# ayutaz/F5-TTS

Hardware: AMD Instinct MI355X
Metric: mel-frames/s (RTF alongside), F5TTS_v1_Base NFE=16 CFM.sample (higher is better)
Workload: dtype bf16; 1 GPU; C2: F5TTS_v1_Base CFM.sample, NFE 16 EPSS + sway -1, CFG 2.0, 1 utterance per GPU, 938 prompt + 938 generated frames (1876), 300 tokens; batch_per_gpu=1, frames=1876, gen_frames_per_gpu=938, nfe=16, parallelism=dp1

## Files before the change

f5-tts_amd/csrc/attention.hip:

```cpp
#include "common.h"
#include "kernels.h"

#include <cstdlib>
#include <cstring>

namespace f5h {

template <int OFF>
F5H_DEV u32x4 lds_b128(uint32_t addr) {
  u32x4 r;
  asm volatile("ds_read_b128 %0, %1 offset:%2" : "=v"(r) : "v"(addr), "i"(OFF));
  return r;
}
template <int OFF>
F5H_DEV uint2 lds_tr_b64(uint32_t addr) {
  uint2 r;
  asm volatile("ds_read_b64_tr_b16 %0, %1 offset:%2" : "=v"(r) : "v"(addr), "i"(OFF));
  return r;
}

F5H_DEV float xor32(float x) {
  const unsigned u = __float_as_uint(x);
  auto r = __builtin_amdgcn_permlane32_swap(u, u, false, false);
  const int hi = (__lane_id() >= 32);
  return __uint_as_float(hi ? r[0] : r[1]);
}

F5H_DEV void attn_block(int& qb, int& bh) {
  const int nqb = gridDim.x, nwg = gridDim.x * gridDim.y;
  const int w = blockIdx.x + nqb * blockIdx.y;
  const int xq = nwg >> 3, xr = nwg & 7, xcd = w & 7;
  const int id = (xcd < xr ? xcd * (xq + 1) : xr * (xq + 1) + (xcd - xr) * xq) + (w >> 3);
  qb = id % nqb;
  bh = id / nqb;
}

template <typename T, bool PRESCALED, int NW, bool RSM>
__global__ __launch_bounds__(64 * NW, 8 / NW) void attn16_kernel(AttnArgs a) {
  typedef Op16<T> OP;
  typedef typename OP::v8 v8;
  typedef typename OP::v4 v4;
  const ProbeT probe_t = probe_enter(a.probe);
  constexpr int TILE_B = 2 * 64 * 128;
  constexpr int NS = 4;
  constexpr int CPW = 512 / (64 * NW);
  constexpr float THR = 8.f;
  static_assert(CPW * 64 * NW == 512, "whole DMA rounds");
  __shared__ __attribute__((aligned(16))) uint4 lds[NS * TILE_B / 16];
  const int tid = threadIdx.x, lane = tid & 63, wid = tid >> 6;
  const int h = lane >> 5;
  int qb, bh;
  attn_block(qb, bh);
  if (a.q_len) bh = spread8(bh, gridDim.y);
  const int s_idx = bh / a.H, head = bh - s_idx * a.H;
  const int L = a.L;
  if (a.q_len && qb * (32 * NW) >= a.q_len[s_idx]) {
    probe_exit(a.probe, probe_t);
    return;
  }
  const int64_t base = (int64_t)bh * L * 64;
  const T* Q = reinterpret_cast<const T*>(a.q) + base;
  const T* K = reinterpret_cast<const T*>(a.k) + base;
  const T* V = reinterpret_cast<const T*>(a.v) + base;
  int klen = L;
  if (a.kv_len) klen = min(klen, a.kv_len[s_idx]);
  const int ntile = (klen + 63) / 64;

  const int qrow = qb * (32 * NW) + wid * 32 + (lane & 31);

  const int wid_s = __builtin_amdgcn_readfirstlane(wid);
  uint32_t dvoff[CPW];
#pragma unroll
  for (int r = 0; r < CPW; ++r) {
    const int p = (r * NW + wid) * 64 + lane, row = p >> 3, slot = p & 7;
    dvoff[r] = (uint32_t)(row * 128 + swz128(row, slot) * 16);
  }
  auto dma = [&](int buf, int kt, bool live = false) {
    uint4* Ks = lds + buf * (TILE_B / 16);
    uint4* Vs = Ks + 512;
    const int rows = live ? min(64, L - kt * 64) : max(0, min(64, L - kt * 64));
    const uint32_t ext = (uint32_t)__builtin_amdgcn_readfirstlane(rows * 128);
    const __amdgpu_buffer_rsrc_t krs = rsrc_of(K + (int64_t)kt * 4096, ext);
    const __amdgpu_buffer_rsrc_t vrs = rsrc_of(V + (int64_t)kt * 4096, ext);
#pragma unroll
    for (int r = 0; r < CPW; ++r) {
      dma16(krs, (LDS_PTR(void))(Ks + (r * NW + wid_s) * 64), dvoff[r], 0);
      dma16(vrs, (LDS_PTR(void))(Vs + (r * NW + wid_s) * 64), dvoff[r], 0);
    }
  };

  const uint32_t lds0 = (uint32_t)(uintptr_t)(LDS_PTR(void))lds;
  uint32_t kaddr[4];
#pragma unroll
  for (int ks = 0; ks < 4; ++ks) {
    const int row = lane & 31;
    kaddr[ks] = lds0 + row * 128 + swz128(row, ks * 2 + h) * 16;
  }
  const int G = lane >> 4, q4 = (lane & 15) >> 2, p4 = lane & 3;
  uint32_t vaddr[2][2];
#pragma unroll
  for (int u = 0; u < 2; ++u)
#pragma unroll
    for (int g8 = 0; g8 < 2; ++g8) {
      const int r1 = 4 * (G >> 1) + q4 + 8 * g8;
      const int dh = 32 * u + 16 * (G & 1) + 4 * p4;
      vaddr[u][g8] = lds0 + 64 * 128 + r1 * 128 + swz128(r1, dh >> 3) * 16 + ((dh >> 2) & 1) * 8;
    }

  typedef float f2 __attribute__((ext_vector_type(2)));
  float m_run = 0.f;
  f32x16 oacc[2], minit;
  f2 lrow = {0.f, 0.f};
  f32x16 lacc;
#pragma unroll
  for (int r = 0; r < 16; ++r) lacc[r] = 0.f;
  v8 ones;
#pragma unroll
  for (int j = 0; j < 8; ++j) ones[j] = from_f32<T>(1.f);
#pragma unroll
  for (int r = 0; r < 16; ++r) {
// ... 156 lines not shown
        for (int sx = 0; sx < 2; ++sx) {
          asm volatile("" : "+v"(vf[u][t][sx][0]));
          asm volatile("" : "+v"(vf[u][t][sx][1]));
        }
    __builtin_amdgcn_sched_barrier(0);
    static_for<0, 3>([&](auto C) {
      mma_chunk(C);
      exp_chunk(std::integral_constant<int, decltype(C)::value + 1>{});
      __builtin_amdgcn_sched_group_barrier(0x008, 1, 0);
      __builtin_amdgcn_sched_group_barrier(0x400, 4, 0);
      __builtin_amdgcn_sched_group_barrier(0x002, 4, 0);
      __builtin_amdgcn_sched_group_barrier(0x008, 1, 0);
      __builtin_amdgcn_sched_group_barrier(0x400, 4, 0);
      __builtin_amdgcn_sched_group_barrier(0x002, 4, 0);
      __builtin_amdgcn_sched_barrier(0);
    });
    mma_chunk(std::integral_constant<int, 3>{});
  };
  using IF = std::false_type;
  using IT = std::true_type;
  auto tile = [&](auto SLOT, auto FIRST_, auto SAFE_, const int kt) __attribute__((always_inline)) {
    tile_wait(kt);
    tile_qk(SLOT, FIRST_, SAFE_, kt);
    tile_pv(SLOT);
  };
  auto pass = [&](auto SAFE_) __attribute__((always_inline)) {
    if (wave_dead) {
      for (int kt = 0; kt < ntile; ++kt) {
        if (kt + 2 < ntile)
          asm volatile("s_waitcnt vmcnt(%0)" ::"i"(4 * CPW) : "memory");
        else if (kt + 1 < ntile)
          asm volatile("s_waitcnt vmcnt(%0)" ::"i"(2 * CPW) : "memory");
        else
          asm volatile("s_waitcnt vmcnt(0)" ::: "memory");
        __builtin_amdgcn_s_barrier();
        if (kt + 3 < ntile) dma((kt + 3) % NS, kt + 3, true);
      }
    } else {
      if (ntile > 0) tile(std::integral_constant<int, 0>{}, IT{}, SAFE_, 0);
      for (int kt0 = 0; kt0 < ntile; kt0 += NS) {
        static_for<0, NS>([&](auto S) {
          const int kt = kt0 + decltype(S)::value;
          if (kt >= 1 && kt < ntile) tile(S, IF{}, SAFE_, kt);
        });
      }
    }
    asm volatile("s_waitcnt vmcnt(0)" ::: "memory");
  };
  if (__builtin_amdgcn_readfirstlane(threadIdx.x) >= 256) __builtin_amdgcn_s_setprio(1);
  pass(IF{});
  auto row_sum = [&]() -> float {
    if constexpr (RSM) return lacc[0];
    float l = lrow.x + lrow.y;
    return l + xor32(l);
  };
  float l_tot = row_sum();
  {
    const bool bad = !(l_tot <= LMAX);
    const unsigned vote = __builtin_amdgcn_ballot_w64(bad) != 0ull ? 1u : 0u;
    __builtin_amdgcn_s_barrier();
    uint32_t* flags = reinterpret_cast<uint32_t*>(lds);
    if (lane == 0) flags[wid] = vote;
    __syncthreads();
    unsigned any = 0;
#pragma unroll
    for (int w = 0; w < NW; ++w) any |= flags[w];
    if (__builtin_amdgcn_readfirstlane(any) || a.force_safe) {
      __syncthreads();
      m_run = 0.f;
      lrow = f2{0.f, 0.f};
#pragma unroll
      for (int r = 0; r < 16; ++r) lacc[r] = 0.f;
#pragma unroll
      for (int r = 0; r < 16; ++r) {
        oacc[0][r] = 0.f;
        oacc[1][r] = 0.f;
        minit[r] = 0.f;
      }
      dma(0, 0);
      dma(1, 1);
      dma(2, 2);
      pass(IT{});
      l_tot = row_sum();
    }
  }
  probe_mark(a.probe, probe_t, 2);
  const float inv = l_tot > 0.f ? 1.f / l_tot : 0.f;
  if (!wave_dead) {
    T* O = reinterpret_cast<T*>(a.o) + (((int64_t)s_idx * L + min(qrow, L - 1)) * a.H + head) * 64;
#pragma unroll
    for (int u = 0; u < 2; ++u)
#pragma unroll
      for (int r4 = 0; r4 < 4; r4 += 2) {
        v4 w0 = {from_f32<T>(oacc[u][4 * r4 + 0] * inv), from_f32<T>(oacc[u][4 * r4 + 1] * inv),
                 from_f32<T>(oacc[u][4 * r4 + 2] * inv), from_f32<T>(oacc[u][4 * r4 + 3] * inv)};
        v4 w1 = {from_f32<T>(oacc[u][4 * r4 + 4] * inv), from_f32<T>(oacc[u][4 * r4 + 5] * inv),
                 from_f32<T>(oacc[u][4 * r4 + 6] * inv), from_f32<T>(oacc[u][4 * r4 + 7] * inv)};
        uint2 a2 = __builtin_bit_cast(uint2, w0), b2 = __builtin_bit_cast(uint2, w1);
        auto sx = __builtin_amdgcn_permlane32_swap(a2.x, b2.x, false, false);
        auto sy = __builtin_amdgcn_permlane32_swap(a2.y, b2.y, false, false);
        const uint4 out = make_uint4(sx[0], sy[0], sx[1], sy[1]);
        if (qrow < L) *reinterpret_cast<uint4*>(O + 32 * u + 8 * r4 + 8 * h) = out;
      }
  }
  probe_exit(a.probe, probe_t);
}

__global__ __launch_bounds__(64) void attn_f32_kernel(AttnArgs a) {
  const ProbeT probe_t = probe_enter(a.probe);
  __shared__ float Ks[32][65];
  __shared__ float Vs[32][64];
  const int lane = threadIdx.x;
  const int bh = blockIdx.y;
  const int s_idx = bh / a.H, head = bh - s_idx * a.H;
  const int L = a.L;
  const int64_t base = (int64_t)bh * L * 64;
  const float* Q = reinterpret_cast<const float*>(a.q) + base;
  const float* K = reinterpret_cast<const float*>(a.k) + base;
  const float* V = reinterpret_cast<const float*>(a.v) + base;
  int klen = L;
  if (a.kv_len) klen = min(klen, a.kv_len[s_idx]);
  if (a.q_len && (int)blockIdx.x * 64 >= a.q_len[s_idx]) {
    probe_exit(a.probe, probe_t);
    return;
  }
  const int qrow = blockIdx.x * 64 + lane;
  float q[64], o[64];
#pragma unroll
  for (int d = 0; d < 64; ++d) {
    q[d] = qrow < L ? Q[(int64_t)qrow * 64 + d] : 0.f;
    o[d] = 0.f;
  }
  float m_run = -INFINITY, l_run = 0.f;
  for (int k0 = 0; k0 < klen; k0 += 32) {
    __syncthreads();
    for (int i = lane; i < 32 * 64; i += 64) {
      int r = i >> 6, d = i & 63, key = k0 + r;
      Ks[r][d] = key < klen ? K[(int64_t)key * 64 + d] : 0.f;
      Vs[r][d] = key < klen ? V[(int64_t)key * 64 + d] : 0.f;
    }
    __syncthreads();
    float sc[32];
    float mx = m_run;
#pragma unroll
    for (int r = 0; r < 32; ++r) {
      float acc = 0.f;
#pragma unroll
      for (int d = 0; d < 64; ++d) acc = fmaf(q[d], Ks[r][d], acc);
      sc[r] = (k0 + r < klen) ? (a.prescaled ? acc : acc * a.scale) : -INFINITY;
      mx = fmaxf(mx, sc[r]);
    }
    const float alpha = a.prescaled ? exp2f(m_run - mx) : expf(m_run - mx);
    m_run = mx;
    l_run *= alpha;
#pragma unroll
    for (int d = 0; d < 64; ++d) o[d] *= alpha;
#pragma unroll
    for (int r = 0; r < 32; ++r) {
      float p = a.prescaled ? exp2f(sc[r] - mx) : expf(sc[r] - mx);
      l_run += p;
#pragma unroll
      for (int d = 0; d < 64; ++d) o[d] = fmaf(p, Vs[r][d], o[d]);
    }
  }
  if (qrow < L) {
    float* O = reinterpret_cast<float*>(a.o) + (((int64_t)s_idx * L + qrow) * a.H + head) * 64;
    const float inv = 1.f / l_run;
#pragma unroll
    for (int d = 0; d < 64; ++d) O[d] = o[d] * inv;
  }
  probe_exit(a.probe, probe_t);
}

template <typename T>
static void launch16(const AttnArgs& a, hipStream_t st) {
  constexpr int NW = 8;
  dim3 grid((a.L + 32 * NW - 1) / (32 * NW), a.S * a.H);
  static const bool rsm = [] {
    const char* v = getenv("F5H_ATTN_ROWSUM");
    return v && !strcmp(v, "mfma");
  }();
  if (a.prescaled) {
    if (rsm)
      hipLaunchKernelGGL((attn16_kernel<T, true, NW, true>), grid, dim3(64 * NW), 0, st, a);
    else
      hipLaunchKernelGGL((attn16_kernel<T, true, NW, false>), grid, dim3(64 * NW), 0, st, a);
  } else {
    hipLaunchKernelGGL((attn16_kernel<T, false, NW, false>), grid, dim3(64 * NW), 0, st, a);
  }
}

static int g_force_safe = 0;
void attention_force_safe(int on) { g_force_safe = on ? 1 : 0; }

hipError_t attention(int compute, const AttnArgs& a0, hipStream_t st) {
  if (a0.S <= 0 || a0.H <= 0 || a0.L <= 0) return hipErrorInvalidValue;
  AttnArgs a = a0;
  a.force_safe = g_force_safe;
  switch (compute) {
    case F5H_C_BF16: launch16<bf16>(a, st); break;
    case F5H_C_FP16: launch16<f16>(a, st); break;
    default: {
      dim3 grid((a.L + 63) / 64, a.S * a.H);
      hipLaunchKernelGGL(attn_f32_kernel, grid, dim3(64), 0, st, a);
    }
  }
  return hipGetLastError();
}

}
```

f5-tts_amd/csrc/chain.h:

```cpp
#pragma once
#include "common.h"
#include "kernels.h"

namespace f5h {

constexpr int kAuxWT = 16;
constexpr unsigned kChainSpinLimit = 1u << 18;
constexpr int kChainSleep = 2;

F5H_DEV void chain_wait(const ChainDep& d, int M, int r0, int nrows) {
  if (!d.wait) return;
  if (__builtin_amdgcn_readfirstlane(threadIdx.x >> 6) == 0) {
    const int g0 = r0 / kChainRows, g1 = (min(r0 + nrows, M) - 1) / kChainRows;
    for (int gi = g0; gi <= g1; ++gi) {
      const int rows = min(kChainRows, M - gi * kChainRows);
      const unsigned need = (unsigned)(d.wait_mult * ((rows + d.wait_unit - 1) / d.wait_unit));
      for (unsigned spins = 0;; ++spins) {
        const unsigned v =
            __builtin_amdgcn_readfirstlane(__hip_atomic_load(d.wait + gi, __ATOMIC_RELAXED, __HIP_MEMORY_SCOPE_AGENT));
        if (v >= need) break;
        if (spins >= d.spin_limit) {
          __hip_atomic_store(d.err, 1u, __ATOMIC_RELAXED, __HIP_MEMORY_SCOPE_AGENT);
          break;
        }
        __builtin_amdgcn_s_sleep(kChainSleep);
      }
    }
    __builtin_amdgcn_fence(__ATOMIC_ACQUIRE, "agent");
    asm volatile("s_waitcnt vmcnt(0)" ::: "memory");
    if (d.tl && threadIdx.x == 0) d.tl[1] = wall_clock64();
  }
  __syncthreads();
}

F5H_DEV void chain_publish(const ChainDep& d, int M, int r0, int nrows) {
  asm volatile("s_waitcnt vmcnt(0)" ::: "memory");
  __syncthreads();
  if (d.tl && threadIdx.x == 0) d.tl[2] = wall_clock64();
  if (threadIdx.x == 0) {
    const int g0 = r0 / kChainRows, g1 = (min(r0 + nrows, M) - 1) / kChainRows;
    for (int gi = g0; gi <= g1; ++gi) __hip_atomic_fetch_add(d.pub + gi, 1u, __ATOMIC_RELAXED, __HIP_MEMORY_SCOPE_AGENT);
  }
}

}
```

f5-tts_amd/csrc/common.h:

```cpp
#pragma once
#include <hip/hip_runtime.h>
#include <stdint.h>

#include <type_traits>

#include "kernels.h"

typedef __bf16 bf16;
typedef __bf16 bf16x8 __attribute__((ext_vector_type(8)));
typedef __bf16 bf16x4 __attribute__((ext_vector_type(4)));
typedef _Float16 f16;
typedef _Float16 f16x8 __attribute__((ext_vector_type(8)));
typedef _Float16 f16x4 __attribute__((ext_vector_type(4)));
typedef short s16x4 __attribute__((ext_vector_type(4)));
typedef float f32x4 __attribute__((ext_vector_type(4)));
typedef float f32x16 __attribute__((ext_vector_type(16)));
typedef unsigned int u32x4 __attribute__((ext_vector_type(4)));

#define F5H_DEV __device__ __forceinline__
#define LDS_PTR(T) __attribute__((address_space(3))) T*

F5H_DEV bf16 f2bf(float x) { return (bf16)x; }
F5H_DEV float bf2f(bf16 x) { return (float)x; }

// ... 122 lines not shown
F5H_DEV float wave_max(float v) {
#pragma unroll
  for (int o = 32; o > 0; o >>= 1) v = fmaxf(v, __shfl_xor(v, o, 64));
  return v;
}

F5H_DEV int swz128(int row, int chunk) {
  return chunk ^ ((((row >> 1) & 1) << 2) | ((row >> 2) & 3));
}
F5H_DEV int swz256(int row, int chunk) { return chunk ^ (row & 15); }

template <typename T> struct Slab;
template <> struct Slab<bf16> {
  typedef bf16x8 frag;
  static F5H_DEV f32x4 mma(const frag& a, const frag& b, f32x4 c) {
    return __builtin_amdgcn_mfma_f32_16x16x32_bf16(a, b, c, 0, 0, 0);
  }
};
template <> struct Slab<f16> {
  typedef f16x8 frag;
  static F5H_DEV f32x4 mma(const frag& a, const frag& b, f32x4 c) {
    return __builtin_amdgcn_mfma_f32_16x16x32_f16(a, b, c, 0, 0, 0);
  }
};
template <> struct Slab<float> {
  typedef f32x4 frag;
  static F5H_DEV f32x4 mma(const frag& a, const frag& b, f32x4 c) {
    c = __builtin_amdgcn_mfma_f32_16x16x4f32(a[0], b[0], c, 0, 0, 0);
    c = __builtin_amdgcn_mfma_f32_16x16x4f32(a[1], b[1], c, 0, 0, 0);
    c = __builtin_amdgcn_mfma_f32_16x16x4f32(a[2], b[2], c, 0, 0, 0);
    c = __builtin_amdgcn_mfma_f32_16x16x4f32(a[3], b[3], c, 0, 0, 0);
    return c;
  }
};

template <typename T, typename S> struct Load16;
template <> struct Load16<bf16, bf16> {
  static F5H_DEV uint4 ld(const bf16* p, bool ok) {
    return ok ? *reinterpret_cast<const uint4*>(p) : make_uint4(0, 0, 0, 0);
  }
};
template <> struct Load16<float, float> {
  static F5H_DEV uint4 ld(const float* p, bool ok) {
    return ok ? *reinterpret_cast<const uint4*>(p) : make_uint4(0, 0, 0, 0);
  }
};
template <> struct Load16<f16, f16> {
  static F5H_DEV uint4 ld(const f16* p, bool ok) {
    return ok ? *reinterpret_cast<const uint4*>(p) : make_uint4(0, 0, 0, 0);
  }
};
template <> struct Load16<f16, float> {
  static F5H_DEV uint4 ld(const float* p, bool ok) {
    if (!ok) return make_uint4(0, 0, 0, 0);
    float4 a = *reinterpret_cast<const float4*>(p);
    float4 b = *reinterpret_cast<const float4*>(p + 4);
    f16x8 v = {(f16)a.x, (f16)a.y, (f16)a.z, (f16)a.w, (f16)b.x, (f16)b.y, (f16)b.z, (f16)b.w};
    return __builtin_bit_cast(uint4, v);
  }
};
template <> struct Load16<bf16, float> {
  static F5H_DEV uint4 ld(const float* p, bool ok) {
    if (!ok) return make_uint4(0, 0, 0, 0);
    float4 a = *reinterpret_cast<const float4*>(p);
    float4 b = *reinterpret_cast<const float4*>(p + 4);
    bf16x8 v = {f2bf(a.x), f2bf(a.y), f2bf(a.z), f2bf(a.w), f2bf(b.x), f2bf(b.y), f2bf(b.z), f2bf(b.w)};
    return __builtin_bit_cast(uint4, v);
  }
};

template <typename T> F5H_DEV constexpr int elems16() { return 16 / (int)sizeof(T); }

F5H_DEV int spread8(int r, int n) {
  const int q = n >> 3, rem = n & 7;
  if (q == 0) return r;
  const int big = rem * (q + 1);
  const int c = r < big ? r / (q + 1) : rem + (r - big) / q;
  const int i = r < big ? r - c * (q + 1) : (r - big) - (c - rem) * q;
  return i * 8 + c;
}

F5H_DEV __amdgpu_buffer_rsrc_t rsrc_of(const void* p, uint64_t bytes) {
  return __builtin_amdgcn_make_buffer_rsrc(const_cast<void*>(p), 0, (int)(uint32_t)bytes, 0x00020000);
}
F5H_DEV void dma16(__amdgpu_buffer_rsrc_t r, LDS_PTR(void) dst, uint32_t voff, uint32_t soff) {
  __builtin_amdgcn_raw_ptr_buffer_load_lds(r, dst, 16, voff, soff, 0, 0);
}

template <int B, int E, typename F>
F5H_DEV void static_for(F&& f) {
  if constexpr (B < E) {
    f(std::integral_constant<int, B>{});
    static_for<B + 1, E>(f);
  }
}

#define F5H_OP_DISPATCH(compute, T, ...)  \
  do {                                     \
    switch (compute) {                     \
      case f5h::F5H_C_BF16: {              \
        typedef bf16 T;                    \
        __VA_ARGS__;                       \
      } break;                             \
      case f5h::F5H_C_FP16: {              \
        typedef f16 T;                     \
        __VA_ARGS__;                       \
      } break;                             \
      default: {                           \
        typedef float T;                   \
        __VA_ARGS__;                       \
      }                                    \
    }                                      \
  } while (0)
```

f5-tts_amd/csrc/engine.cpp:

```cpp
#include <hip/hip_runtime.h>

#include <cmath>
#include <cstring>
#include <algorithm>
#include <atomic>
#include <chrono>
#include <cstdio>
#include <memory>
#include <functional>
#include <mutex>
#include <string>
#include <unordered_map>
#include <vector>

#include "../../include/f5h.h"
#include "kernels.h"
#include "reaper.h"

using namespace f5h;

static thread_local std::string g_err;
static int fail(int code, const std::string& msg) {
  g_err = msg;
  return code;
}
int f5h_internal_fail(int code, const std::string& msg) { return fail(code, msg); }
#define HIPCK(x)                                                                               \
  do {                                                                                         \
    hipError_t _e = (x);                                                                       \
    if (_e != hipSuccess) return fail(F5H_EHIP, std::string(#x) + ": " + hipGetErrorString(_e)); \
  } while (0)

#define RC(x)              \
  do {                     \
    int _r = (x);          \
    if (_r) return _r;     \
  } while (0)

struct Lin {
  void* w = nullptr;
  float* b = nullptr;
  int N = 0, K = 0, Npad = 0;
};

struct CNX {
  float *dw_w = nullptr, *dw_b = nullptr, *ln_w = nullptr, *ln_b = nullptr, *gamma = nullptr, *beta = nullptr;
  Lin pw1, pw2;
};

struct Layer {
  Lin qkv, out, ff1, ff2, skip;
  float *g_attn = nullptr, *g_ff = nullptr;
  Lin qkv_g, ff1_g;
};

struct GraphKey {
  const void* ws;
  int kind;
  int B, N, nt, nfe, use_cfg, batch_mask, probe, split, pad_skip, chain, lnfold;
  int method;
  uint64_t kernel_epoch;
  uint32_t cfg_bits;
  bool operator==(const GraphKey& o) const {
    return ws == o.ws && kind == o.kind && B == o.B && N == o.N && nt == o.nt && nfe == o.nfe && kernel_epoch == o.kernel_epoch &&
           use_cfg == o.use_cfg && batch_mask == o.batch_mask && probe == o.probe && cfg_bits == o.cfg_bits &&
           split == o.split && pad_skip == o.pad_skip && chain == o.chain && lnfold == o.lnfold && method == o.method;
  }
};

struct f5h_engine {
  f5h_arch a{};
  int dev = 0;
  int bf = 0;
  size_t esz = 4;
  int tdp = 0;
  std::vector<void*> allocs;
  hipStream_t mstream = nullptr;
  Lin t1, t2, ada, in_x, in_ct, proj_out;
  float* text_table = nullptr;
  float* freqs = nullptr;
  std::vector<CNX> cnx;
  void* conv_w[2] = {nullptr, nullptr};
  float* conv_b[2] = {nullptr, nullptr};
  std::vector<Layer> layers;
  float* norm_out_g = nullptr;
  std::mutex gm;
  std::vector<std::shared_ptr<struct GraphEntry>> graphs;
  std::vector<std::shared_ptr<struct GraphEntry>> graveyard;
  std::vector<hipEvent_t> ev_pool;
  std::vector<struct GraphKey> pro_seen;
  int64_t n_evicted = 0, n_reaped = 0;
  std::mutex hm;
  double last_host[8] = {};
  hipStream_t cap = nullptr;
  hipStream_t cap2 = nullptr;
  hipEvent_t ev_fork = nullptr, ev_join = nullptr;
  int graph_mode = 1;
  int split_cfg = 2;
  int pad_skip = 1;
  int chain = 0;
  int lnfold = 1;
  bool lnf_ok = false, rmsf_ok = false;
  const void** lnf_w = nullptr;
  int64_t ada_row = 0;
  std::atomic<int64_t> n_lnfold{0};
  unsigned* chain_fault = nullptr;
  volatile unsigned* fault_host = nullptr;
  int fault_slot = -1;
  std::atomic<int64_t> n_chain{0};
  uint64_t use_ctr = 0;
  int64_t n_captures = 0, n_replays = 0;
  std::mutex pm;
  int probe_class = -1;
  unsigned long long* pstamp = nullptr;
  unsigned long long* pslots = nullptr;
  unsigned long long* ptl = nullptr;
  int* ptick = nullptr;
  double wall_khz = 0.0;
  UseLog uses;
};
static constexpr size_t kGraphCache = 16;
static constexpr size_t kProbeBytes = (64 + 2 * (size_t)kProbeEnd) * sizeof(unsigned long long);

static std::atomic<uint64_t> g_kernel_epoch{0};

struct GraphEntry {
  GraphKey key{};
  hipGraphExec_t exec = nullptr;
  uint64_t stamp = 0;
  std::vector<hipEvent_t> inflight;
  ~GraphEntry() {
    if (exec) (void)hipGraphExecDestroy(exec);
    for (hipEvent_t ev : inflight) (void)hipEventDestroy(ev);
  }
};

struct WView {
  const void* p;
  int dt;
  int64_t numel;
};
struct WMap {
  std::unordered_map<std::string, WView> m;
  const WView* get(const std::string& n, int64_t numel, std::string* err) const {
    auto it = m.find(n);
    if (it == m.end()) {
      *err = "missing weight " + n;
      return nullptr;
    }
    if (it->second.numel != numel) {
      *err = "weight " + n + " has " + std::to_string(it->second.numel) + " elements, expected " +
             std::to_string(numel);
      return nullptr;
    }
    return &it->second;
  }
};

static int ealloc(f5h_engine* e, size_t bytes, void** out) {
  void* p = dev_alloc(e->dev, bytes, e->mstream);
  if (!p) return fail(F5H_EHIP, "device allocation of " + std::to_string(bytes) + " bytes");
  e->allocs.push_back(p);
  *out = p;
  return 0;
}

template <typename T>
static int upload(f5h_engine* e, const std::vector<T>& h, T** out) {
  void* p = nullptr;
  RC(ealloc(e, h.size() * sizeof(T) + 16, &p));
  HIPCK(hipMemcpyAsync(p, h.data(), h.size() * sizeof(T), hipMemcpyHostToDevice, e->mstream));
  HIPCK(hipStreamSynchronize(e->mstream));
  *out = reinterpret_cast<T*>(p);
  return 0;
}

static int dalloc(f5h_engine* e, size_t bytes, void** out) {
  void* p = nullptr;
  RC(ealloc(e, bytes + 16, &p));
  HIPCK(hipMemsetAsync(p, 0, bytes + 16, e->mstream));
  *out = p;
  return 0;
}

static int op_dt(const f5h_engine* e) { return e->bf; }

static int pack_rows(const WView& v, int rows, int64_t ld_src, int col0, int ncols, void* dst, int ddt,
                     int64_t ld_dst, int dst_row0, int dst_col, hipStream_t st) {
// ... 233 lines not shown
  uint8_t* rowkeep;
  int32_t* kvlen;
  float* lnp;
  unsigned* chain;
  int chain_g4;
  float *ada_cur, *temb_cur, *tgrid;
  int* kstep;
  float* y;
  float** trajp;
  float *sgrid, *kbuf;
  std::vector<void*> xs;
  void* pp[2];
  float* in_cond;
  uint8_t* in_mask;
  int64_t* in_text;
  int32_t* in_dur;
};

static void layout(const f5h_engine* e, WS& ws, Bufs& b, int B, int N, int nfe, int use_cfg, int method = 0,
                   int steps = 0) {
  const f5h_arch& a = e->a;
  const int d = a.dim, td = a.text_dim, S = use_cfg ? 2 * B : B;
  const int L = a.backbone == F5H_DIT ? N : N + 1;
  const size_t rows = (size_t)S * L, es = e->esz;
  const int inner = a.heads * 64;
  b.tsin = ws.take<float>((size_t)nfe * 256);
  b.th = ws.take<float>((size_t)nfe * d);
  b.temb = ws.take<float>((size_t)nfe * d);
  b.tin_op = ws.take<char>((size_t)nfe * std::max(256, d) * es);
  b.ada = a.backbone == F5H_DIT ? ws.take<float>((size_t)nfe * e->ada_row) : nullptr;
  b.te = ws.take<float>((size_t)2 * B * N * td);
  b.keepfill = ws.take<uint8_t>((size_t)2 * B * N);
  if (a.conv_layers > 0) {
    b.dwln = ws.take<char>((size_t)2 * B * N * td * es);
    b.pw1o = ws.take<float>((size_t)2 * B * N * 2 * td);
    b.grno = ws.take<char>((size_t)2 * B * N * 2 * td * es);
    b.grn_scr = ws.take<float>((size_t)((N + 63) / 64 + 1) * 2 * B * 2 * td);
  } else {
    b.dwln = b.grno = nullptr;
    b.pw1o = b.grn_scr = nullptr;
  }
  b.act = ws.take<char>((size_t)S * N * (128 + e->tdp) * es);
  b.P = ws.take<float>((size_t)S * N * d);
  b.ypad = ws.take<char>((size_t)B * N * 128 * es);
  b.h0 = ws.take<float>((size_t)S * N * d);
  b.c1 = ws.take<char>((size_t)S * N * d * es);
  b.h = a.backbone == F5H_DIT ? ws.take<float>(rows * d) : nullptr;
  b.aop = ws.take<char>(rows * d * es);
  b.q = ws.take<char>(rows * inner * es);
  b.k = ws.take<char>(rows * inner * es);
  b.v = ws.take<char>(rows * inner * es);
  b.o = ws.take<char>(rows * inner * es);
  b.f = ws.take<char>(rows * a.ff_dim * es);
  b.p = ws.take<float>(rows * e->proj_out.Npad);
  b.rope = ws.take<float2>((size_t)L * 32);
  b.rowkeep = ws.take<uint8_t>(rows);
  b.kvlen = ws.take<int32_t>(S);
  b.chain_g4 = ((int)((rows + kChainRows - 1) / kChainRows) + 3) / 4 * 4;
  b.chain = a.backbone == F5H_DIT ? ws.take<unsigned>((size_t)a.depth * 5 * b.chain_g4) : nullptr;
  b.ada_cur = a.backbone == F5H_DIT ? ws.take<float>((size_t)e->ada_row) : nullptr;
  b.lnp = (e->lnf_ok || e->rmsf_ok) ? ws.take<float>(rows * (size_t)(d / 64) * 2) : nullptr;
  b.temb_cur = ws.take<float>((size_t)d);
  b.tgrid = ws.take<float>((size_t)nfe);
  b.kstep = ws.take<int>(64);
  b.y = ws.take<float>((size_t)B * N * e->a.mel_dim);
  b.trajp = ws.take<float*>(8);
  b.in_cond = ws.take<float>((size_t)B * N * a.mel_dim);
  b.in_mask = ws.take<uint8_t>((size_t)B * N);
  b.in_text = ws.take<int64_t>((size_t)B * N);
  b.in_dur = ws.take<int32_t>((size_t)B);
  b.xs.clear();
  b.pp[0] = b.pp[1] = nullptr;
  if (a.backbone == F5H_UNETT) {
    for (int i = 0; i <= a.depth / 2; ++i) b.xs.push_back(ws.take<char>(rows * d * es));
    b.pp[0] = ws.take<char>(rows * d * es);
    b.pp[1] = ws.take<char>(rows * d * es);
  }
  b.sgrid = method ? ws.take<float>((size_t)steps + 1) : nullptr;
  const int kept = ode_kept_slopes(method);
  b.kbuf = kept ? ws.take<float>((size_t)kept * B * N * a.mel_dim) : nullptr;
}

enum { KC_FFN1 = 0, KC_ATTN = 1, KC_QKV = 2, KC_FFN2 = 3, KC_CONV = 4, KC_OUT = 5, KC_NORM = 6, KC_CHAIN = 7 };
struct ProbeScope {
  f5h_engine* e;
  hipStream_t st;
  bool on;
  bool self = false;
  unsigned long long* slots = nullptr;
  ProbeScope(f5h_engine* e_, int kc, hipStream_t s, int* site, DevProbe* kp = nullptr)
      : e(e_), st(s), on(e_->probe_class == kc && e_->pslots && *site < kProbeSites) {
    if (!on) return;
    const int s0 = (*site)++;
    slots = e->pslots + (size_t)s0 * kProbeRow;
    if (kp) {
      self = true;
      kp->slots = slots;
      kp->tick = e->ptick;
      kp->tl = s0 == 0 ? e->ptl : nullptr;
    } else {
      (void)stamp_begin(slots, e->ptick, st);
    }
  }
  ~ProbeScope() {
    if (on && !self) (void)stamp_end(slots, e->ptick, st);
  }
};

struct Ctx {
  f5h_engine* e;
  hipStream_t st;
  Bufs b;
  int B, N, nt, S, L, nfe, use_cfg, batch_mask;
  int method, steps;
  int drop_audio, drop_text;
  hipStream_t st2;
  int site;
  int chain;
  int lnfold;
  double* hp;
};
enum { HP_TOTAL = 0, HP_PROLOGUE, HP_LOCK, HP_REAP, HP_CAPTURE, HP_INSTANTIATE, HP_LAUNCH, HP_FINAL, kHostPhases };
static double host_ms() {
  return std::chrono::duration<double, std::milli>(std::chrono::steady_clock::now().time_since_epoch()).count();
}

static GemmArgs gargs(const void* A, int64_t lda, const Lin& W, int M, void* C, int64_t ldc) {
  GemmArgs g{};
  g.A = A;
  g.lda = lda;
  g.W = W.w;
  g.ldw = W.K;
  g.M = M;
  g.N = W.N;
  g.K = W.K;
  g.bias = W.b;
  g.C = C;
  g.ldc = ldc;
  return g;
}

#define KCK(x)                                                                                  \
  do {                                                                                          \
    hipError_t _e = (x);                                                                        \
    if (_e != hipSuccess) return fail(F5H_EHIP, std::string(#x) + ": " + hipGetErrorString(_e)); \
  } while (0)

static int prologue(Ctx& c, const float* t_host, int nt_vals, const float* cond, const uint8_t* cond_mask,
                    const int64_t* text, const int32_t* duration, bool text_cached = false) {
  f5h_engine* e = c.e;
  const f5h_arch& a = e->a;
  const int d = a.dim, td = a.text_dim, bf = e->bf;
  Bufs& b = c.b;
  hipStream_t st = c.st;
  KCK(rope_table(c.L, b.rope, st));
  const int off = a.backbone == F5H_DIT ? 0 : 1;
  if (c.batch_mask) {
    KCK(build_rowkeep(duration, c.B, c.S, c.L, off, b.rowkeep, st));
    KCK(build_kvlen(duration, c.B, c.S, off, b.kvlen, st));
  }
  {
    if (t_host)
      KCK(time_sinus(t_host, nt_vals, b.tsin, st));
    else
      KCK(time_sinus_dev(b.tgrid, nt_vals, b.tsin, st));
    KCK(f32_to_op(bf, b.tsin, (int64_t)nt_vals * 256, b.tin_op, st));
    GemmArgs g = gargs(b.tin_op, 256, e->t1, nt_vals, b.th, d);
    KCK(gemm(bf, EPI_SILU, g, st));
    KCK(f32_to_op(bf, b.th, (int64_t)nt_vals * d, b.tin_op, st));
    g = gargs(b.tin_op, d, e->t2, nt_vals, b.temb, d);
    KCK(gemm(bf, EPI_STORE, g, st));
    if (a.backbone == F5H_DIT) {
      KCK(silu_to_op(bf, b.temb, b.tin_op, (int64_t)nt_vals * d, st));
      g = gargs(b.tin_op, d, e->ada, nt_vals, b.ada, e->ada_row);
      KCK(gemm(bf, EPI_STORE, g, st));
      if (c.lnfold) {
        LnFoldArgs la{};
        la.table = b.ada;
        la.stride = e->ada_row;
        la.out_off = e->ada.Npad;
        la.nfe = nt_vals;
        la.depth = a.depth;
        la.d = d;
        la.F = a.ff_dim;
        la.w1 = e->lnf_w;
        la.wqkv = e->lnf_w + a.depth;
        KCK(lnfold_uv(bf, la, st));
      }
    }
  }
  if (!text_cached) {
    TextEmbArgs t{};
    t.text = text;
    t.B = c.B;
    t.nt = c.nt;
    t.N = c.N;
    t.td = td;
    t.seq_len = (a.backbone == F5H_DIT && c.batch_mask) ? duration : nullptr;
    t.table = e->text_table;
    t.freqs = a.conv_layers > 0 ? e->freqs : nullptr;
    t.mask_padding = a.text_mask_padding;
    t.out_c = b.te;
// ... 79 lines not shown
    cv.x = b.h0 + no * d;
    cv.x_f32 = 1;
    cv.w = e->conv_w[0];
    cv.bias = e->conv_b[0];
    cv.mode = 0;
    cv.y = op(b.c1, no, d);
    {
      ProbeScope ps(e, KC_CONV, st, &c.site);
      KCK(conv_pos(bf, cv, st));
    }
    cv.x = op(b.c1, no, d);
    cv.x_f32 = bf ? 0 : 1;
    cv.w = e->conv_w[1];
    cv.bias = e->conv_b[1];
    cv.mode = r16 ? 2 : 1;
    cv.y = bh;
    cv.y_seq_stride = c.L;
    cv.y_row_off = dit ? 0 : 1;
    cv.resid = b.h0 + no * d;
    KCK(conv_pos(bf, cv, st));
  }
  if (!dit) KCK(write_time_token(bf, r16, b.temb_cur, ns, c.L, d, bh, st));

  const float* ada_k = dit ? b.ada_cur : nullptr;
  const int epi_resid = r16 ? EPI_RESID16 : EPI_RESID;
  void* h = bh;
  const void* h_in = nullptr;
  auto qkv_args = [&](const Layer& Lq) {
    GemmArgs g = gargs(aop, d, Lq.qkv, rows, nullptr, 0);
    g.rope = b.rope;
    g.seq_len = c.L;
    g.heads = H;
    g.rope_heads = a.pe_attn_head > 0 ? a.pe_attn_head : H;
    g.q = q;
    g.k = k;
    g.v = v;
    g.q_scale = 0.125f * 1.4426950408889634f;
    return g;
  };
  const bool chain_on = c.chain && dit && r16 && do_ln && !keep && d == 1024 && b.chain && s0 == 0 && ns == c.S &&
                        (e->probe_class < 0 || e->probe_class == KC_ATTN || e->probe_class == KC_CONV ||
                         e->probe_class == KC_CHAIN);
  static const bool zero_memset = [] {
    const char* v = getenv("F5H_CHAIN_ZERO");
    return v && !strcmp(v, "memset");
  }();
  if (chain_on) {
    if (zero_memset)
      KCK(hipMemsetAsync(b.chain, 0, (size_t)a.depth * 5 * b.chain_g4 * sizeof(unsigned), st));
    else
      KCK(zero_words(b.chain, (int64_t)a.depth * 5 * b.chain_g4, st));
  }
  bool qkv_done = false;
  bool final_done = false;
  const bool fold_on = c.lnfold && dit && r16 && do_ln && !keep && !chain_on && b.lnp && e->lnf_ok;
  const bool rms_on = c.lnfold && !dit && r16 && b.lnp && e->rmsf_ok;
  const int64_t lnf_lw = 2 * (int64_t)a.ff_dim + 6 * (int64_t)d;
  auto lnf = [&](int l) { return ada_k + e->ada.Npad + (int64_t)l * lnf_lw; };
  auto fold_consumer = [&](GemmArgs& g, const float* u, const float* v) {
    g.ln_part_in = b.lnp + ro * (size_t)(d / 64) * 2;
    g.ln_nparts = d / 64;
    g.ln_u = u;
    g.ln_v = v;
    g.ln_eps = 1e-6f;
  };
  auto rms_consumer = [&](GemmArgs& g) {
    g.ln_part_in = b.lnp + ro * (size_t)(d / 64) * 2;
    g.ln_nparts = d / 64;
    g.ln_rms = 1;
    g.ln_eps = 1e-30f;
  };
  auto rms_producer = [&](GemmArgs& g) {
    g.ln_part = b.lnp + ro * (size_t)(d / 64) * 2;
    g.ln_nparts = d / 64;
    g.ln_rms = 1;
  };
  auto fold_producer = [&](GemmArgs& g, const float* scale) {
    g.hs = aop;
    g.hs_scale = scale;
    g.ln_part = b.lnp + ro * (size_t)(d / 64) * 2;
    g.ln_nparts = d / 64;
  };
  if (fold_on || rms_on) e->n_lnfold.fetch_add(1, std::memory_order_relaxed);
  for (int l = 0; l < a.depth; ++l) {
    Layer& Ly = e->layers[l];
    const float* ad = ada_k ? ada_k + (size_t)l * 6 * d : nullptr;
    if (!dit) {
      const int half = a.depth / 2;
      if (l < half) {
        h_in = res(b.xs[l]);
        h = res(b.xs[l + 1]);
        if (!(rms_on && l > 0)) KCK(rms_norm_g(bf, h_in, r16, rows, d, Ly.g_attn, aop, st));
      } else {
        void* x_prev = h;
        h = res(b.pp[(l - half) & 1]);
        h_in = nullptr;
        GemmArgs g = gargs(x_prev, d, Ly.skip, rows, h, d);
        g.A2 = res(b.xs[a.depth - 1 - l]);
        g.k_split = d;
        KCK(gemm(bf, r16 ? EPI_STORE16 : EPI_STORE, g, st));
        KCK(rms_norm_g(bf, h, r16, rows, d, Ly.g_attn, aop, st));
      }
    } else {
      if (do_ln && !qkv_done && !(fold_on && l > 0))
        KCK(ln_modulate(bf, h, r16, rows, d, ad , ad + d , aop, st));
    }
    if (!qkv_done) {
      GemmArgs g = qkv_args(Ly);
      if (fold_on && l > 0) fold_consumer(g, lnf(l) + 2 * a.ff_dim, lnf(l) + 2 * a.ff_dim + 3 * d);
      if (rms_on && l > 0 && l < a.depth / 2) {
        g.A = h_in;
        g.W = Ly.qkv_g.w;
        rms_consumer(g);
      }
      ProbeScope ps(e, KC_QKV, st, &c.site, &g.probe);
      KCK(gemm(bf, EPI_QKV, g, st));
    }
    qkv_done = false;
    {
      AttnArgs at{};
      at.q = q;
      at.k = k;
      at.v = v;
      at.o = o;
      at.S = ns;
      at.H = H;
      at.L = c.L;
      at.kv_len = (a.attn_mask_enabled && c.batch_mask) ? b.kvlen + s0 : nullptr;
      at.q_len = (c.batch_mask && e->pad_skip) ? b.kvlen + s0 : nullptr;
      at.scale = 0.125f;
      at.prescaled = 1;
      ProbeScope ps(e, KC_ATTN, st, &c.site, &at.probe);
      KCK(attention(bf, at, st));
    }
    if (chain_on) {
      ChainArgs ca{};
      ca.out = gargs(o, inner, Ly.out, rows, h, d);
      ca.out.gate = ad + 2 * d;
      ca.ln1 = LnArgs{h, aop, ad + 3 * d , ad + 4 * d };
      ca.ff1 = gargs(aop, d, Ly.ff1, rows, f, a.ff_dim);
      ca.ff2 = gargs(f, a.ff_dim, Ly.ff2, rows, h, d);
      ca.ff2.gate = ad + 5 * d;
      if (l + 1 < a.depth) {
        const float* an = ada_k + (size_t)(l + 1) * 6 * d;
        ca.ln2 = LnArgs{h, aop, an , an + d };
        ca.qkv = qkv_args(e->layers[l + 1]);
      } else {
        const float* fin = ada_k + (size_t)a.depth * 6 * d;
        ca.ln2 = LnArgs{h, aop, fin + d, fin};
      }
      ca.cnt = b.chain + (size_t)l * 5 * b.chain_g4;
      ca.groups = (rows + kChainRows - 1) / kChainRows;
      ca.fault = e->chain_fault;
      ProbeScope ps(e, KC_CHAIN, st, &c.site, &ca.probe);
      const hipError_t ce = chain_launch(bf, ca, st);
      if (ce == hipSuccess) {
        e->n_chain.fetch_add(1, std::memory_order_relaxed);
        qkv_done = l + 1 < a.depth;
        final_done = l + 1 == a.depth;
        continue;
      }
      if (ce != hipErrorInvalidValue) KCK(ce);
    }
    {
      GemmArgs g = gargs(o, inner, Ly.out, rows, h, d);
      g.resid = h_in;
      g.gate = ad ? ad + 2 * d : nullptr;
      g.rowkeep = keep;
      if (keep && !h_in && e->pad_skip && !rms_on) {
        g.live_len = b.kvlen + s0;
        g.live_seq = c.L;
      }
      if (fold_on) fold_producer(g, ad + 4 * d );
      if (rms_on) rms_producer(g);
      ProbeScope ps(e, KC_OUT, st, &c.site, &g.probe);
      KCK(gemm(bf, epi_resid, g, st));
    }
    if (!fold_on && !rms_on) {
      ProbeScope ps(e, KC_NORM, st, &c.site);
      if (dit) {
        if (do_ln) KCK(ln_modulate(bf, h, r16, rows, d, ad + 3 * d , ad + 4 * d , aop, st));
      }
      else
        KCK(rms_norm_g(bf, h, r16, rows, d, Ly.g_ff, aop, st));
    }
    {
      GemmArgs g = gargs(aop, d, Ly.ff1, rows, f, a.ff_dim);
      if (fold_on) fold_consumer(g, lnf(l), lnf(l) + a.ff_dim);
      if (rms_on) {
        g.A = h;
        g.W = Ly.ff1_g.w;
        rms_consumer(g);
      }
      ProbeScope ps(e, KC_FFN1, st, &c.site, &g.probe);
      KCK(gemm(bf, EPI_GELU_TANH, g, st));
    }
    {
      GemmArgs g = gargs(f, a.ff_dim, Ly.ff2, rows, h, d);
      g.gate = ad ? ad + 5 * d : nullptr;
      if (fold_on && l + 1 < a.depth) fold_producer(g, ada_k + (size_t)(l + 1) * 6 * d + d);
      if (rms_on && l + 1 < a.depth / 2) rms_producer(g);
      ProbeScope ps(e, KC_FFN2, st, &c.site, &g.probe);
      KCK(gemm(bf, epi_resid, g, st));
    }
  }
  if (dit) {
    const float* fin = ada_k + (size_t)a.depth * 6 * d;
    if (!final_done) KCK(ln_modulate(bf, h, r16, rows, d, fin + d, fin, aop, st));
  } else {
    KCK(rms_norm_g(bf, h, r16, rows, d, e->norm_out_g, aop, st));
  }
  const int pld = e->proj_out.Npad;
  GemmArgs g = gargs(aop, d, e->proj_out, rows, b.p + ro * pld, pld);
  g.N = pld;
  KCK(gemm(bf, EPI_STORE, g, st));
  return 0;
}

static int backbone_step(Ctx& c) {
  if (!c.st2 || !c.use_cfg) return backbone_part(c, 0, c.S, c.st);
  f5h_engine* e = c.e;
  KCK(hipEventRecord(e->ev_fork, c.st));
  KCK(hipStreamWaitEvent(c.st2, e->ev_fork, 0));
  RC(backbone_part(c, 0, c.B, c.st));
  RC(backbone_part(c, c.B, c.B, c.st2));
  KCK(hipEventRecord(e->ev_join, c.st2));
  KCK(hipStreamWaitEvent(c.st, e->ev_join, 0));
  return 0;
}

static std::mutex g_slot_m;
static unsigned* g_slots = nullptr;
static std::vector<int> g_free_slots;
static constexpr int kFaultSlots = 4096;
static int fault_slot_take(volatile unsigned** host) {
  std::lock_guard<std::mutex> lk(g_slot_m);
  if (!g_slots) {
    void* p = nullptr;
    if (hipHostMalloc(&p, kFaultSlots * 64, hipHostMallocDefault) != hipSuccess) return -1;
    g_slots = static_cast<unsigned*>(p);
    for (int i = kFaultSlots - 1; i >= 0; --i) g_free_slots.push_back(i);
  }
  if (g_free_slots.empty()) return -1;
  const int i = g_free_slots.back();
  g_free_slots.pop_back();
  *host = g_slots + (size_t)i * 16;
  **host = 0u;
  return i;
}
static void fault_slot_give(int i) {
  if (i < 0) return;
  std::lock_guard<std::mutex> lk(g_slot_m);
  g_free_slots.push_back(i);
}

struct ChainGate {
  std::mutex m;
  hipStream_t owner = nullptr;
  bool owned = false;
  int enqueuing = 0;
  hipEvent_t done = nullptr;
  bool pending = false;
};
static ChainGate g_gate[64];
static std::atomic<int64_t> g_gate_refused{0};

static bool chain_admit(int dev, hipStream_t st) {
  ChainGate& g = g_gate[dev & 63];
  std::lock_guard<std::mutex> lk(g.m);
  if (g.owned && g.owner != st) {
    bool busy = g.enqueuing > 0;
    if (!busy && g.pending) {
      busy = hipEventQuery(g.done) == hipErrorNotReady;
      (void)hipGetLastError();
      if (!busy) g.pending = false;
    }
    if (busy) {
      g_gate_refused.fetch_add(1, std::memory_order_relaxed);
      return false;
    }
  }
  g.owner = st;
  g.owned = true;
  ++g.enqueuing;
// ... 207 lines not shown
  *out = e;
  return 0;
}

int f5h_engine_create(const f5h_arch* arch, const f5h_weight* weights, int32_t n_weights, int32_t device,
                      f5h_engine** out) {
  if (n_weights < 0 || (n_weights > 0 && !weights)) return fail(F5H_EINVAL, "null weights");
  std::vector<f5h_tensor_view> v((size_t)n_weights);
  for (int i = 0; i < n_weights; ++i)
    v[i] = f5h_tensor_view{weights[i].name, weights[i].data, F5H_DT_F32, 0, weights[i].numel};
  return f5h_engine_create_views(arch, v.data(), n_weights, device, out);
}

void f5h_engine_destroy(f5h_engine* e) {
  if (!e) return;
  retire(e->dev, [e] {
    for (hipEvent_t ev : e->uses.take()) {
      (void)hipEventSynchronize(ev);
      (void)hipEventDestroy(ev);
    }
    {
      std::lock_guard<std::mutex> g(e->gm);
      for (auto* v : {&e->graphs, &e->graveyard})
        for (auto& x : *v)
          for (hipEvent_t ev : x->inflight) (void)hipEventSynchronize(ev);
    }
    e->graphs.clear();
    e->graveyard.clear();
    for (hipEvent_t ev : e->ev_pool) (void)hipEventDestroy(ev);
    e->ev_pool.clear();
    if (e->cap) (void)hipStreamDestroy(e->cap);
    if (e->cap2) (void)hipStreamDestroy(e->cap2);
    if (e->ev_fork) (void)hipEventDestroy(e->ev_fork);
    if (e->ev_join) (void)hipEventDestroy(e->ev_join);
    for (void* p : e->allocs) dev_free(p, e->mstream);
    if (e->mstream) (void)hipStreamDestroy(e->mstream);
    fault_slot_give(e->fault_slot);
    delete e;
  });
}

size_t f5h_workspace_size_ode(const f5h_engine* e, int32_t B, int32_t N, int32_t nt, int32_t steps, int32_t use_cfg,
                             int32_t method) {
  (void)nt;
  if (!e || B <= 0 || N <= 0 || steps <= 0 || method < 0 || method >= kOdeMethods) return 0;
  WS ws;
  Bufs b;
  layout(e, ws, b, B, N, steps * ode_tableau(method).stages + 1, use_cfg, method, steps);
  return ws.off;
}
size_t f5h_workspace_size(const f5h_engine* e, int32_t B, int32_t N, int32_t nt, int32_t nfe, int32_t use_cfg) {
  return f5h_workspace_size_ode(e, B, N, nt, nfe, use_cfg, F5H_EULER);
}

static int check_ws(f5h_engine* e, int B, int N, int nfe, int use_cfg, void* w, size_t bytes, Ctx& c, int method = 0,
                    int steps = 0) {
  WS ws;
  layout(e, ws, c.b, B, N, nfe + 1, use_cfg, method, steps);
  if (bytes < ws.off)
    return fail(F5H_ENOMEM, "workspace too small: need " + std::to_string(ws.off) + " have " + std::to_string(bytes));
  ws.off = 0;
  ws.base = reinterpret_cast<char*>(w);
  layout(e, ws, c.b, B, N, nfe + 1, use_cfg, method, steps);
  return 0;
}

static int run_steps(Ctx& c, const f5h_sample_args* a, const void* ws);
static int graph_get(Ctx& c, const GraphKey& key, bool split, const std::function<int(Ctx&)>& body,
                     std::shared_ptr<GraphEntry>& hold, int64_t replays);
static int note_replays(f5h_engine* e, GraphEntry* g, hipStream_t st);
static bool prologue_repeats(f5h_engine* e, const GraphKey& key);

static GraphKey prologue_key(const Ctx& c, const void* ws) {
  GraphKey key{};
  key.ws = ws;
  key.kind = 1;
  key.B = c.B;
  key.N = c.N;
  key.nt = c.nt;
  key.nfe = c.nfe;
  key.use_cfg = c.use_cfg;
  key.batch_mask = c.batch_mask;
  key.lnfold = c.lnfold;
  key.method = c.method;
  key.kernel_epoch = g_kernel_epoch.load();
  return key;
}
static int prologue_graph(Ctx& c, const f5h_sample_args* a, const GraphKey& key) {
  f5h_engine* e = c.e;
  const size_t bn = (size_t)c.B * c.N;
  HIPCK(hipMemcpyAsync(c.b.in_cond, a->cond, bn * e->a.mel_dim * sizeof(float), hipMemcpyDeviceToDevice, c.st));
  HIPCK(hipMemcpyAsync(c.b.in_mask, a->cond_mask, bn, hipMemcpyDeviceToDevice, c.st));
  if (c.nt > 0)
    HIPCK(hipMemcpyAsync(c.b.in_text, a->text, (size_t)c.B * c.nt * sizeof(int64_t), hipMemcpyDeviceToDevice, c.st));
  HIPCK(hipMemcpyAsync(c.b.in_dur, a->duration, (size_t)c.B * sizeof(int32_t), hipMemcpyDeviceToDevice, c.st));
  const Bufs& b = c.b;
  std::shared_ptr<GraphEntry> hold;
  RC(graph_get(c, key, false,
               [&](Ctx& cc) { return prologue(cc, nullptr, cc.nfe, b.in_cond, b.in_mask, b.in_text, b.in_dur); },
               hold, 1));
  HIPCK(hipGraphLaunch(hold->exec, c.st));
  return note_replays(e, hold.get(), c.st);
}

static float round_to(int compute, float x) {
  if (compute == F5H_FP16) return (float)(_Float16)x;
  if (compute != F5H_BF16 || x != x) return x;
  uint32_t u;
  std::memcpy(&u, &x, 4);
  u = (u + 0x7fffu + ((u >> 16) & 1u)) & 0xffff0000u;
  std::memcpy(&x, &u, 4);
  return x;
}
static void ode_eval_times(int method, int compute, const float* t, int steps, float* out) {
#pragma clang fp contract(off)
  const OdeTableau T = ode_tableau(method);
  for (int i = 0; i <= steps; ++i)
    if (round_to(compute, t[i]) != t[i]) compute = F5H_FP32;
  for (int k = 0; k < steps; ++k) {
    const float t0 = t[k], t1 = t[k + 1];
    const float dt = round_to(compute, t1 - t0);
    for (int s = 0; s < T.stages; ++s) {
      float v = t0;
      if (s > 0) v = T.c[s] == 1.f ? t1 : round_to(compute, t0 + round_to(compute, dt * T.c[s]));
      out[k * T.stages + s] = v;
    }
  }
}

int f5h_debug_ode_tableau(int32_t method, int32_t* stages, float* c, float* a, float* b) {
  if (method < 0 || method >= kOdeMethods) return fail(F5H_EINVAL, "ode method must be 0 (euler), 1 (midpoint) or 2 (rk4)");
  const OdeTableau T = ode_tableau(method);
  if (stages) *stages = T.stages;
  if (c) std::memcpy(c, T.c, sizeof(T.c));
  if (a) std::memcpy(a, T.a, sizeof(T.a));
  if (b) std::memcpy(b, T.b, sizeof(T.b));
  return 0;
}
int f5h_debug_ode_eval_times(int32_t method, int32_t compute, const float* t_grid, int32_t steps, float* out) {
  if (method < 0 || method >= kOdeMethods || compute < F5H_FP32 || compute > F5H_FP16 || !t_grid || steps <= 0 || !out)
    return fail(F5H_EINVAL, "bad ode_eval_times argument");
  ode_eval_times(method, compute, t_grid, steps, out);
  return 0;
}

static int sample_impl(f5h_engine* e, void* stream, const f5h_sample_args* a, int method, void* workspace,
                       size_t workspace_bytes);
int f5h_sample(f5h_engine* e, void* stream, const f5h_sample_args* a, void* workspace, size_t workspace_bytes) {
  return sample_impl(e, stream, a, F5H_EULER, workspace, workspace_bytes);
}
int f5h_sample_ode(f5h_engine* e, void* stream, const f5h_sample_args* a, int32_t method, void* workspace,
                   size_t workspace_bytes) {
  if (method < 0 || method >= kOdeMethods) return fail(F5H_EINVAL, "ode method must be 0 (euler), 1 (midpoint) or 2 (rk4)");
  return sample_impl(e, stream, a, method, workspace, workspace_bytes);
}

static int sample_impl(f5h_engine* e, void* stream, const f5h_sample_args* a, int method, void* workspace,
                       size_t workspace_bytes) {
  if (!e || !a) return fail(F5H_EINVAL, "null engine/args");
  if (a->B <= 0 || a->N <= 0 || a->nt < 0 || a->nfe <= 0 || a->nfe > 512)
    return fail(F5H_EINVAL, "bad B/N/nt/nfe");
  const int stages = ode_tableau(method).stages;
  if (a->nfe * stages > 512)
    return fail(F5H_EINVAL, std::to_string(a->nfe) + " steps x " + std::to_string(stages) + " stages = " +
                                std::to_string(a->nfe * stages) +
                                " backbone evaluations exceed the 512 rows of the per-call time tables");
  if (!a->cond || !a->cond_mask || !a->duration || !a->y0 || !a->t_grid || !a->out || (a->nt > 0 && !a->text))
    return fail(F5H_EINVAL, "null tensor argument");
  if (e->a.backbone == F5H_DIT && a->N > 8192) return fail(F5H_EINVAL, "N exceeds the text position table (8192)");
  HIPCK(hipSetDevice(e->dev));
  UseNote used{e->uses, reinterpret_cast<hipStream_t>(stream)};
  Ctx c{};
  c.e = e;
  c.st = reinterpret_cast<hipStream_t>(stream);
  c.B = a->B;
  c.N = a->N;
  c.nt = a->nt;
  c.method = method;
  c.steps = a->nfe;
  c.nfe = a->nfe * stages;
  c.use_cfg = a->cfg_strength >= 1e-5f;
  c.S = c.use_cfg ? 2 * c.B : c.B;
  c.L = e->a.backbone == F5H_DIT ? c.N : c.N + 1;
  c.batch_mask = a->use_batch_mask ? 1 : 0;
  RC(check_ws(e, c.B, c.N, c.nfe, c.use_cfg, workspace, workspace_bytes, c, method, c.steps));
  RC(chain_fault_check(e, c.st));
  ChainTicket ticket;
  c.chain = chain_for_call(e, c, ticket);
  c.lnfold = e->lnfold && !c.chain && ((e->lnf_ok && !c.batch_mask) || e->rmsf_ok);
  double hp[kHostPhases] = {};
  c.hp = hp;
  const double h0 = host_ms();
  static const bool pro_graph = [] {
    const char* v = getenv("F5H_PROLOGUE_GRAPH");
    return !(v && *v == '0');
  }();
  std::vector<float> evt;
  const float* t_rows = a->t_grid;
  if (method == F5H_EULER) {
    HIPCK(grid_upload(a->t_grid, c.nfe + 1, c.b.tgrid, c.st));
  } else {
    evt.resize(c.nfe);
    ode_eval_times(method, e->bf, a->t_grid, c.steps, evt.data());
    t_rows = evt.data();
    HIPCK(grid_upload(t_rows, c.nfe, c.b.tgrid, c.st));
    HIPCK(grid_upload(a->t_grid, c.steps + 1, c.b.sgrid, c.st));
  }
  const GraphKey pkey = prologue_key(c, workspace);
  if (pro_graph && e->graph_mode && c.nt <= c.N && prologue_repeats(e, pkey))
    RC(prologue_graph(c, a, pkey));
  else
    RC(prologue(c, t_rows, c.nfe, a->cond, a->cond_mask, a->text, a->duration));
  const double h1 = host_ms();
  const size_t ysz = (size_t)c.B * c.N * e->a.mel_dim;
  HIPCK(hipMemcpyAsync(c.b.y, a->y0, ysz * sizeof(float), hipMemcpyDeviceToDevice, c.st));
  if (a->trajectory)
    HIPCK(hipMemcpyAsync(a->trajectory, a->y0, ysz * sizeof(float), hipMemcpyDeviceToDevice, c.st));
  HIPCK(pack_y(e->bf, c.b.y, c.B * c.N, e->a.mel_dim, c.b.ypad, c.st));
  HIPCK(ptr_upload(a->trajectory, c.b.trajp, c.st));
  HIPCK(hipMemsetAsync(c.b.kstep, 0, 64 * sizeof(int), c.st));
  RC(step_prep(c));
  const double h2 = host_ms();
  const double g2 = hp[HP_LOCK] + hp[HP_REAP] + hp[HP_CAPTURE] + hp[HP_INSTANTIATE];
  RC(run_steps(c, a, workspace));
  const double h3 = host_ms();
  HIPCK(final_where_out(a->cond, a->cond_mask, c.b.y, a->out, c.B, c.N, e->a.mel_dim,
                        c.chain ? e->chain_fault : nullptr, c.st));
  if (c.chain) RC(chain_fault_note(e, c.st));
  const double h4 = host_ms();
  hp[HP_TOTAL] = h4 - h0;
  hp[HP_PROLOGUE] = h1 - h0;
  hp[HP_LAUNCH] = (h3 - h2) - (hp[HP_LOCK] + hp[HP_REAP] + hp[HP_CAPTURE] + hp[HP_INSTANTIATE] - g2);
  hp[HP_FINAL] = h4 - h3;
  {
    std::lock_guard<std::mutex> g(e->hm);
    std::memcpy(e->last_host, hp, sizeof(hp));
  }
  return 0;
}

static int enqueue_step(Ctx& c, const f5h_sample_args* a) {
  f5h_engine* e = c.e;
  {
    c.site = 0;
    RC(backbone_step(c));
    const bool dit = e->a.backbone == F5H_DIT;
    if (c.method != F5H_EULER) {
      RkArgs r{};
      r.y = c.b.y;
      r.B = c.B;
      r.N = c.N;
      r.mel = e->a.mel_dim;
      r.p = c.b.p;
      r.p_seq_stride = (int64_t)c.L * e->proj_out.Npad;
      r.p_row_off = dit ? 0 : 1;
      r.p_ld = e->proj_out.Npad;
      r.use_cfg = c.use_cfg;
      r.cfg = a->cfg_strength;
      r.ypad = c.b.ypad;
      r.compute = e->bf;
      r.method = c.method;
      r.kbuf = c.b.kbuf;
      r.keval = c.b.kstep;
      r.sgrid = c.b.sgrid;
      r.trajp = c.b.trajp;
      r.next_src = dit ? c.b.ada : c.b.temb;
      r.next_stride = dit ? e->ada_row : e->a.dim;
      r.next_n = dit ? (int)e->ada_row : e->a.dim;
      r.next_dst = dit ? c.b.ada_cur : c.b.temb_cur;
      r.neval = c.nfe;
      r.arrive = reinterpret_cast<unsigned*>(c.b.kstep + kArrive);
      r.tick = e->ptick;
      KCK(cfg_rk(r, c.st));
      return 0;
    }
    EulerArgs u{};
    u.y = c.b.y;
    u.B = c.B;
    u.N = c.N;
    u.mel = e->a.mel_dim;
    u.p = c.b.p;
    u.p_seq_stride = (int64_t)c.L * e->proj_out.Npad;
    u.p_row_off = e->a.backbone == F5H_DIT ? 0 : 1;
    u.p_ld = e->proj_out.Npad;
    u.use_cfg = c.use_cfg;
    u.cfg = a->cfg_strength;
    u.dt = 0.f;
    u.kstep = c.b.kstep;
    u.tgrid = c.b.tgrid;
    u.ypad = c.b.ypad;
    u.compute = e->bf;
    u.traj = nullptr;
    u.trajp = c.b.trajp;
    u.next_src = dit ? c.b.ada : c.b.temb;
    u.next_stride = dit ? e->ada_row : e->a.dim;
    u.next_n = dit ? (int)e->ada_row : e->a.dim;
    u.next_dst = dit ? c.b.ada_cur : c.b.temb_cur;
    u.nfe = c.nfe;
    u.arrive = reinterpret_cast<unsigned*>(c.b.kstep + kArrive);
    u.tick = e->ptick;
    KCK(cfg_euler(u, c.st));
  }
  return 0;
}

static int run_steps(Ctx& c, const f5h_sample_args* a, const void* ws) {
  f5h_engine* e = c.e;
  if (!e->graph_mode) {
    for (int k = 0; k < c.nfe; ++k) RC(enqueue_step(c, a));
    return 0;
  }
  GraphKey key{};
  key.ws = ws;
  key.B = c.B;
  key.N = c.N;
  key.nfe = c.nfe;
  key.use_cfg = c.use_cfg;
  key.batch_mask = c.batch_mask;
  key.probe = e->probe_class;
  const bool split = e->split_cfg == 1;
  key.split = split;
  key.pad_skip = e->pad_skip;
  key.chain = c.chain;
  key.lnfold = c.lnfold;
  key.method = c.method;
  key.kernel_epoch = g_kernel_epoch.load();
  std::memcpy(&key.cfg_bits, &a->cfg_strength, 4);
  std::shared_ptr<GraphEntry> hold;
  RC(graph_get(c, key, split, [&](Ctx& cc) { return enqueue_step(cc, a); }, hold, c.nfe));
  int rc = 0, k = 0;
  for (; k < c.nfe; ++k) {
    const hipError_t le = hipGraphLaunch(hold->exec, c.st);
    if (le != hipSuccess) {
      rc = fail(F5H_EHIP, std::string("hipGraphLaunch: ") + hipGetErrorString(le));
      break;
    }
  }
  if (k > 0) {
    const int r2 = note_replays(e, hold.get(), c.st);
    if (!rc) rc = r2;
  }
  return rc;
}

static bool host_trace() {
  static const bool on = [] {
    const char* v = getenv("F5H_HOST_TRACE");
    return v && *v == '1';
  }();
  return on;
}
static void reap_graphs(f5h_engine* e) {
  auto done = [e](GraphEntry& g) {
    size_t k = 0;
    for (hipEvent_t ev : g.inflight) {
      if (hipEventQuery(ev) == hipSuccess)
        e->ev_pool.push_back(ev);
      else
        g.inflight[k++] = ev;
    }
    (void)hipGetLastError();
    g.inflight.resize(k);
    return k == 0;
  };
  for (auto& g : e->graphs)
    if (g->inflight.size() > 4) done(*g);
  size_t k = 0;
  for (size_t i = 0; i < e->graveyard.size(); ++i) {
    auto& g = e->graveyard[i];
    if (done(*g) && g.use_count() == 1) {
      ++e->n_reaped;
      continue;
    }
    if (k != i) std::swap(e->graveyard[k], e->graveyard[i]);
    ++k;
  }
  e->graveyard.resize(k);
}

static int note_replays(f5h_engine* e, GraphEntry* g, hipStream_t st) {
  hipEvent_t ev = nullptr;
  {
    std::lock_guard<std::mutex> lk(e->gm);
    if (!e->ev_pool.empty()) {
      ev = e->ev_pool.back();
      e->ev_pool.pop_back();
    }
  }
  if (!ev) HIPCK(hipEventCreateWithFlags(&ev, hipEventDisableTiming));
  HIPCK(hipEventRecord(ev, st));
  std::lock_guard<std::mutex> lk(e->gm);
  g->inflight.push_back(ev);
  return 0;
}

static int graph_get(Ctx& c, const GraphKey& key, bool split, const std::function<int(Ctx&)>& body,
                     std::shared_ptr<GraphEntry>& hold, int64_t replays) {
  f5h_engine* e = c.e;
  const double t0 = host_ms();
  std::lock_guard<std::mutex> g(e->gm);
  const double t1 = host_ms();
  const int64_t reaped0 = e->n_reaped;
  reap_graphs(e);
  const double t2 = host_ms();
  if (c.hp) {
    c.hp[HP_LOCK] += t1 - t0;
    c.hp[HP_REAP] += t2 - t1;
// ... 14 lines not shown
    ne->key = key;
    Ctx cc = c;
    cc.st = e->cap;
    cc.st2 = split ? e->cap2 : nullptr;
    const double c0 = host_ms();
    hipError_t be = hipStreamBeginCapture(e->cap, hipStreamCaptureModeThreadLocal);
    if (be != hipSuccess) return fail(F5H_EHIP, std::string("hipStreamBeginCapture: ") + hipGetErrorString(be));
    const int rc = body(cc);
    hipGraph_t graph = nullptr;
    const hipError_t ce = hipStreamEndCapture(e->cap, &graph);
    if (rc || ce != hipSuccess) {
      if (graph) (void)hipGraphDestroy(graph);
      if (rc) return rc;
      return fail(F5H_EHIP, std::string("hipStreamEndCapture: ") + hipGetErrorString(ce));
    }
    const double c1 = host_ms();
    const hipError_t ie = hipGraphInstantiate(&ne->exec, graph, nullptr, nullptr, 0);
    (void)hipGraphDestroy(graph);
    if (c.hp) {
      c.hp[HP_CAPTURE] += c1 - c0;
      c.hp[HP_INSTANTIATE] += host_ms() - c1;
    }
    if (host_trace())
      std::fprintf(stderr, "[f5h host] capture %.3f ms, instantiate %.3f ms\n", c1 - c0, host_ms() - c1);
    if (ie != hipSuccess) {
      ne->exec = nullptr;
      return fail(F5H_EHIP, std::string("hipGraphInstantiate: ") + hipGetErrorString(ie));
    }
    if (e->graphs.size() >= kGraphCache) {
      size_t lru = 0;
      for (size_t i = 1; i < e->graphs.size(); ++i)
        if (e->graphs[i]->stamp < e->graphs[lru]->stamp) lru = i;
      e->graveyard.push_back(std::move(e->graphs[lru]));
      e->graphs.erase(e->graphs.begin() + lru);
      ++e->n_evicted;
    }
    e->graphs.push_back(ne);
    e->n_captures++;
    hold = ne;
  }
  hold->stamp = ++e->use_ctr;
  e->n_replays += replays;
  return 0;
}

static bool prologue_repeats(f5h_engine* e, const GraphKey& key) {
  std::lock_guard<std::mutex> g(e->gm);
  for (const auto& x : e->graphs)
    if (x->key == key) return true;
  for (const auto& k : e->pro_seen)
    if (k == key) return true;
  if (e->pro_seen.size() >= 64) e->pro_seen.erase(e->pro_seen.begin());
  e->pro_seen.push_back(key);
  return false;
}

int f5h_forward(f5h_engine* e, void* stream, const f5h_forward_args* a, void* workspace, size_t workspace_bytes) {
  if (!e || !a) return fail(F5H_EINVAL, "null engine/args");
  if (a->B <= 0 || a->N <= 0 || a->nt < 0) return fail(F5H_EINVAL, "bad B/N/nt");
  if (!a->x || !a->cond || !a->cond_mask || !a->duration || !a->pred || (a->nt > 0 && !a->text))
    return fail(F5H_EINVAL, "null tensor argument");
  HIPCK(hipSetDevice(e->dev));
  UseNote used{e->uses, reinterpret_cast<hipStream_t>(stream)};
  Ctx c{};
  c.e = e;
  c.st = reinterpret_cast<hipStream_t>(stream);
  c.B = a->B;
  c.N = a->N;
  c.nt = a->nt;
  c.nfe = 1;
  c.use_cfg = a->cfg_infer ? 1 : 0;
  c.S = c.use_cfg ? 2 * c.B : c.B;
  c.drop_audio = (!c.use_cfg && a->drop_audio_cond) ? 1 : 0;
  c.drop_text = (!c.use_cfg && a->drop_text) ? 1 : 0;
  c.L = e->a.backbone == F5H_DIT ? c.N : c.N + 1;
  c.batch_mask = a->use_batch_mask ? 1 : 0;
  if (e->a.backbone == F5H_DIT && a->N > 8192) return fail(F5H_EINVAL, "N exceeds the text position table (8192)");
  if (a->text_cache < 0 || a->text_cache > 2) return fail(F5H_EINVAL, "text_cache must be 0, 1 or 2");
  RC(check_ws(e, c.B, c.N, 1, c.use_cfg, workspace, workspace_bytes, c));
  RC(chain_fault_check(e, c.st));
  ChainTicket ticket;
  c.chain = chain_for_call(e, c, ticket);
  c.lnfold = e->lnfold && !c.chain && ((e->lnf_ok && !c.batch_mask) || e->rmsf_ok);
  const bool cached = a->text_cache == 2;
  if (a->t_dev) {
    HIPCK(hipMemcpyAsync(c.b.tgrid, a->t_dev, sizeof(float), hipMemcpyDeviceToDevice, c.st));
    RC(prologue(c, nullptr, 1, a->cond, a->cond_mask, a->text, a->duration, cached));
  } else {
    float tg[2] = {a->t, a->t};
    RC(prologue(c, tg, 1, a->cond, a->cond_mask, a->text, a->duration, cached));
  }
  HIPCK(pack_y(e->bf, a->x, c.B * c.N, e->a.mel_dim, c.b.ypad, c.st));
  HIPCK(hipMemsetAsync(c.b.kstep, 0, sizeof(int), c.st));
  auto body = [](Ctx& cc) -> int {
    cc.site = 0;
    RC(step_prep(cc));
    RC(backbone_step(cc));
    KCK(step_advance(cc.b.kstep, cc.e->ptick, cc.st));
    return 0;
  };
  if (e->graph_mode && a->text_cache != 0) {
    GraphKey key{};
    key.ws = workspace;
    key.kind = 2;
    key.B = c.B;
    key.N = c.N;
    key.nt = c.nt;
    key.nfe = 1;
    key.use_cfg = c.use_cfg;
    key.batch_mask = c.batch_mask;
    key.probe = e->probe_class;
    key.pad_skip = e->pad_skip;
    key.chain = c.chain;
    key.lnfold = c.lnfold;
    key.kernel_epoch = g_kernel_epoch.load();
    std::shared_ptr<GraphEntry> hold;
    RC(graph_get(c, key, false, body, hold, 1));
    HIPCK(hipGraphLaunch(hold->exec, c.st));
    RC(note_replays(e, hold.get(), c.st));
  } else {
    RC(body(c));
  }
  HIPCK(copy_pred(c.b.p, c.S, c.L, e->a.backbone == F5H_DIT ? 0 : 1, e->a.mel_dim, e->proj_out.Npad, a->pred,
                  c.chain ? e->chain_fault : nullptr, c.st));
  if (c.chain) RC(chain_fault_note(e, c.st));
  return 0;
}

int f5h_probe_enable(f5h_engine* e, int32_t kclass, int32_t enable) {
  if (!e) return fail(F5H_EINVAL, "null engine");
  std::lock_guard<std::mutex> g(e->pm);
  e->probe_class = enable ? kclass : -1;
  if (e->pstamp) {
    HIPCK(hipSetDevice(e->dev));
    HIPCK(hipDeviceSynchronize());
    HIPCK(hipMemset(e->pstamp, 0, 64 * sizeof(unsigned long long)));
    HIPCK(hipMemset(e->pslots, 0xff, (size_t)kProbeEnd * sizeof(unsigned long long)));
    HIPCK(hipMemset(e->pslots + kProbeEnd, 0, (size_t)kProbeEnd * sizeof(unsigned long long)));
    HIPCK(hipMemset(e->ptl, 0, (size_t)kTimelineWG * 4 * sizeof(unsigned long long)));
    HIPCK(hipDeviceSynchronize());
  }
  return 0;
}

int f5h_probe_timeline(f5h_engine* e, uint64_t* stamps, int32_t max_wg, int32_t* n_wg, double* tick_khz) {
  if (!e || !stamps || max_wg <= 0) return fail(F5H_EINVAL, "null engine / buffer");
  std::lock_guard<std::mutex> g(e->pm);
  HIPCK(hipSetDevice(e->dev));
  HIPCK(hipDeviceSynchronize());
  const int n = std::min<int>(max_wg, kTimelineWG);
  HIPCK(hipMemcpy(stamps, e->ptl, (size_t)n * 4 * sizeof(unsigned long long), hipMemcpyDeviceToHost));
  int last = 0;
  for (int i = 0; i < n; ++i)
    if (stamps[4 * i]) last = i + 1;
  if (n_wg) *n_wg = last;
  if (tick_khz) *tick_khz = e->wall_khz;
  return 0;
}

int f5h_probe_read(f5h_engine* e, int64_t* launches, double* total_ms) {
  if (!e) return fail(F5H_EINVAL, "null engine");
  std::lock_guard<std::mutex> g(e->pm);
  double ms = 0.0;
  int64_t n = 0;
  if (e->pstamp && e->wall_khz > 0.0) {
    HIPCK(hipSetDevice(e->dev));
    HIPCK(hipDeviceSynchronize());
    std::vector<unsigned long long> h(2 * (size_t)kProbeEnd);
    HIPCK(hipMemcpy(h.data(), e->pslots, h.size() * sizeof(unsigned long long), hipMemcpyDeviceToHost));
    unsigned long long ticks = 0;
    for (int64_t i = 0; i < kProbeEnd; i += (int64_t)kProbeLanes * kProbeStride) {
      unsigned long long t0 = ~0ull, t1 = 0;
      for (int l = 0; l < kProbeLanes; ++l) {
        t0 = std::min(t0, h[i + l * kProbeStride]);
        t1 = std::max(t1, h[kProbeEnd + i + l * kProbeStride]);
      }
      if (t1 == 0 || t0 == ~0ull || t1 < t0) continue;
      ticks += t1 - t0;
      ++n;
    }
    ms = (double)ticks / e->wall_khz;
  }
  if (launches) *launches = n;
  if (total_ms) *total_ms = ms;
  return 0;
}

int f5h_set_graph_mode(f5h_engine* e, int32_t mode) {
  if (!e) return fail(F5H_EINVAL, "null engine");
  if (mode != 0 && mode != 1) return fail(F5H_EINVAL, "graph mode must be 0 (eager) or 1 (step graph)");
  std::lock_guard<std::mutex> g(e->gm);
  e->graph_mode = mode;
  return 0;
}

int f5h_set_cfg_streams(f5h_engine* e, int32_t n) {
  if (!e) return fail(F5H_EINVAL, "null engine");
  if (n < 0 || n > 2) return fail(F5H_EINVAL, "cfg streams must be 0 (auto), 1 or 2");
  std::lock_guard<std::mutex> g(e->gm);
  e->split_cfg = n == 0 ? 2 : (n == 2 ? 1 : 0);
  return 0;
}

int f5h_set_pad_skip(f5h_engine* e, int32_t enable) {
  if (!e) return fail(F5H_EINVAL, "null engine");
  if (enable != 0 && enable != 1) return fail(F5H_EINVAL, "pad skip must be 0 or 1");
  std::lock_guard<std::mutex> g(e->gm);
  e->pad_skip = enable;
  return 0;
}

int f5h_set_chain(f5h_engine* e, int32_t enable) {
  if (!e) return fail(F5H_EINVAL, "null engine");
  if (enable != 0 && enable != 1) return fail(F5H_EINVAL, "chain must be 0 or 1");
  std::lock_guard<std::mutex> g(e->gm);
  e->chain = enable;
  return 0;
}

int f5h_chain_stats(f5h_engine* e, int64_t* launches, int32_t* fault, int64_t* refused) {
  if (!e) return fail(F5H_EINVAL, "null engine");
  if (launches) *launches = e->n_chain.load(std::memory_order_relaxed);
  if (refused) *refused = g_gate_refused.load(std::memory_order_relaxed);
  if (fault) {
    *fault = 0;
    if (e->chain_fault) {
      unsigned v = 0;
      HIPCK(hipSetDevice(e->dev));
      HIPCK(hipMemcpyAsync(&v, e->chain_fault, sizeof(v), hipMemcpyDeviceToHost, e->mstream));
      HIPCK(hipStreamSynchronize(e->mstream));
      *fault = v ? 1 : 0;
    }
  }
  return 0;
}

int f5h_set_ln_fold(f5h_engine* e, int32_t enable) {
  if (!e) return fail(F5H_EINVAL, "null engine");
  if (enable != 0 && enable != 1) return fail(F5H_EINVAL, "ln fold must be 0 or 1");
  std::lock_guard<std::mutex> g(e->gm);
  e->lnfold = enable;
  return 0;
}

int f5h_ln_fold_stats(f5h_engine* e, int32_t* supported, int64_t* passes) {
  if (!e) return fail(F5H_EINVAL, "null engine");
  if (supported) *supported = (e->lnf_ok || e->rmsf_ok) ? 1 : 0;
  if (passes) *passes = e->n_lnfold.load(std::memory_order_relaxed);
  return 0;
}

int f5h_last_call_host_ms(f5h_engine* e, double* ms, int32_t n) {
  if (!e || !ms || n <= 0) return fail(F5H_EINVAL, "null engine / buffer");
  std::lock_guard<std::mutex> g(e->hm);
  for (int i = 0; i < n; ++i) ms[i] = i < kHostPhases ? e->last_host[i] : 0.0;
  return 0;
}

int f5h_chain_debug_spin_limit(int64_t limit) {
  chain_set_spin_limit(limit);
  g_kernel_epoch.fetch_add(1);
  return 0;
}

int f5h_graph_stats(f5h_engine* e, int64_t* captures, int64_t* replays, int32_t* cached) {
  if (!e) return fail(F5H_EINVAL, "null engine");
  std::lock_guard<std::mutex> g(e->gm);
  if (captures) *captures = e->n_captures;
  if (replays) *replays = e->n_replays;
  if (cached) *cached = (int32_t)e->graphs.size();
  return 0;
}

int f5h_op_linear(void* stream, int32_t compute, int32_t M, int32_t N, int32_t K, const float* A, const float* W,
                  const float* bias, float* C, void* workspace, size_t workspace_bytes) {
  if (M <= 0 || N <= 0 || K <= 0 || K % 64) return fail(F5H_EINVAL, "op_linear needs K % 64 == 0");
  if (compute < F5H_FP32 || compute > F5H_FP16) return fail(F5H_EINVAL, "bad compute mode");
  const int Npad = (N + 127) / 128 * 128;
  const size_t es = compute ? 2 : 4;
  const size_t need = (size_t)Npad * K * es;
  if (workspace_bytes < (need + 255) / 256 * 256 + (size_t)M * K * es)
    return fail(F5H_ENOMEM, "workspace too small for op_linear");
  hipStream_t st = reinterpret_cast<hipStream_t>(stream);
  HIPCK(hipMemsetAsync(workspace, 0, need, st));
  HIPCK(f32_to_op(compute, W, (int64_t)N * K, workspace, st));
  const void* Aop = A;
  if (compute) {
    char* ab = reinterpret_cast<char*>(workspace) + (need + 255) / 256 * 256;
    HIPCK(f32_to_op(compute, A, (int64_t)M * K, ab, st));
    Aop = ab;
  }
  GemmArgs g{};
  g.A = Aop;
  g.lda = K;
  g.W = workspace;
  g.ldw = K;
  g.M = M;
  g.N = N;
  g.K = K;
  g.bias = bias;
  g.C = C;
  g.ldc = N;
  HIPCK(gemm(compute, EPI_STORE, g, st));
  return 0;
}

int f5h_gemm_force_config(int32_t cfg) {
  if (cfg != -1 && cfg != 0 && cfg != 1 && cfg != 5 && cfg != 11 && cfg != 12 && cfg != 13)
    return fail(F5H_EINVAL, "gemm config must be -1, 0, 1, 5, 11, 12 or 13");
  gemm_force_config(cfg);
  g_kernel_epoch.fetch_add(1);
  return 0;
}

int f5h_attn_force_safe(int32_t on) {
  attention_force_safe(on);
  g_kernel_epoch.fetch_add(1);
  return 0;
}

int f5h_debug_tile_live(const int32_t* live_len, int32_t live_seq, int32_t M, int32_t m0, int32_t BM) {
  if (live_seq <= 0 || M <= 0 || BM <= 0 || m0 < 0 || m0 >= M) return fail(F5H_EINVAL, "bad tile");
  return tile_live_rows(live_len, live_seq, M, m0, BM) ? 1 : 0;
}

static int op_attention_impl(void* stream, int32_t compute, int32_t S, int32_t H, int32_t N, const float* Q,
                             const float* K, const float* V, const int32_t* kv_len, const int32_t* q_len,
                             int32_t q_prescaled, float* O, void* workspace, size_t workspace_bytes) {
  if (S <= 0 || H <= 0 || N <= 0) return fail(F5H_EINVAL, "bad attention shape");
  if (compute < F5H_FP32 || compute > F5H_FP16) return fail(F5H_EINVAL, "bad compute mode");
  hipStream_t st = reinterpret_cast<hipStream_t>(stream);
// ... 414 lines not shown
```

f5-tts_amd/csrc/gemm.hip:

```cpp
#include "gemm_impl.h"

namespace f5h {

static int g_force_cfg = -1;
static int gemm_env_cfg() {
  static int v = [] {
    const char* e = getenv("F5H_GEMM_CFG");
    return e ? atoi(e) : -1;
  }();
  return v;
}


static int large_cfg() {
  static const int v = [] {
    const char* e = getenv("F5H_LARGE_CFG");
    const int c = e ? atoi(e) : 11;
    return (c == 12 || c == 13) ? c : 11;
  }();
  return v;
}

int gemm_group_m() {
  static const int v = [] {
    const char* e = getenv("F5H_GEMM_GROUP_M");
    const int g = e ? atoi(e) : 1;
    return g > 1 && g <= 64 ? g : 1;
  }();
  return v;
}

int gemm_num_cus() {
  static int cus[64] = {0};
  int dev = 0;
  if (hipGetDevice(&dev) != hipSuccess || dev < 0 || dev >= 64) return 256;
  if (!cus[dev]) {
    int n = 0;
    if (hipDeviceGetAttribute(&n, hipDeviceAttributeMultiprocessorCount, dev) != hipSuccess || n <= 0) n = 256;
    cus[dev] = n;
  }
  return cus[dev];
}

static int pick_cfg(const GemmArgs& a) {
  if (a.K % 64 == 0 && (int64_t)((a.M + 255) / 256) * ((a.N + 255) / 256) >= 1024) return large_cfg();
  struct Opt { int cfg, bm, bn; float eff; };
  constexpr Opt opts[3] = {{5, 192, 128, 0.86f}, {1, 128, 128, 0.74f}, {0, 64, 128, 0.57f}};
  int best = 0;
  double tbest = 1e300;
  for (const Opt& o : opts) {
    const int64_t tiles = (int64_t)((a.M + o.bm - 1) / o.bm) * ((a.N + o.bn - 1) / o.bn);
    const double t = (double)((tiles + 511) / 512) * o.bm * o.bn / o.eff;
    if (t < tbest * 0.999) tbest = t, best = o.cfg;
  }
  return best;
}

static int gemm_map_cfg(int N, int K) {
  struct E { int n, k, c; };
  static std::vector<E> m = [] {
    std::vector<E> v;
    const char* e = getenv("F5H_GEMM_MAP");
    while (e && *e) {
      int n, k, c, used = 0;
      if (sscanf(e, "%d:%d:%d%n", &n, &k, &c, &used) != 3) break;
      v.push_back({n, k, c});
      e += used;
      if (*e == ',') ++e;
    }
    return v;
  }();
  for (const E& x : m)
    if (x.n == N && x.k == K) return x.c;
  return -1;
}


int gemm_select_cfg(const GemmArgs& a) {
  int cfg = g_force_cfg >= 0 ? g_force_cfg : gemm_env_cfg();
  if (cfg < 0) cfg = gemm_map_cfg(a.N, a.K);
  if (cfg < 0) cfg = pick_cfg(a);
  return cfg;
}

hipError_t gemm_launch_bf16_a(int epi, const GemmArgs& a, hipStream_t st);
hipError_t gemm_launch_bf16_b(int epi, const GemmArgs& a, hipStream_t st);
hipError_t gemm_launch_f16_a(int epi, const GemmArgs& a, hipStream_t st);
hipError_t gemm_launch_f16_b(int epi, const GemmArgs& a, hipStream_t st);
hipError_t gemm_launch_f32(int epi, const GemmArgs& a, hipStream_t st);

static bool hot_epi(int epi) {
  return epi == EPI_QKV || epi == EPI_RESID || epi == EPI_RESID16 || epi == EPI_GELU_TANH || epi == EPI_GELU_ERF_OP;
}

void gemm_force_config(int cfg) { g_force_cfg = cfg; }

hipError_t gemm(int compute, int epi, const GemmArgs& a, hipStream_t st) {
  const int bke = compute ? 64 : 32;
  if (a.K % bke != 0 || a.M < 0 || a.N <= 0 || a.lda % 8 || a.ldw % 8) return hipErrorInvalidValue;
  if (epi == EPI_INPROJ && (a.ldc % 8 || a.ld_add % 8 || a.N % 8)) return hipErrorInvalidValue;
  if (epi == EPI_QKV && (a.N % 64)) return hipErrorInvalidValue;
  if (a.A2 && (a.k_split <= 0 || a.k_split % 64 || a.k_split >= a.K)) return hipErrorInvalidValue;
  if (a.resid && epi != EPI_RESID && epi != EPI_RESID16) return hipErrorInvalidValue;
  switch (compute) {
    case F5H_C_BF16: return hot_epi(epi) ? gemm_launch_bf16_a(epi, a, st) : gemm_launch_bf16_b(epi, a, st);
    case F5H_C_FP16: return hot_epi(epi) ? gemm_launch_f16_a(epi, a, st) : gemm_launch_f16_b(epi, a, st);
    default: return gemm_launch_f32(epi, a, st);
  }
}

}
```

f5-tts_amd/csrc/gemm_impl.h:

```cpp
#pragma once
#include "common.h"
#include "kernels.h"
#include "chain.h"

#include <cstdio>
#include <cstdlib>
#include <vector>

namespace f5h {

int gemm_select_cfg(const GemmArgs& a);


template <int BM, int BN, int WGM, int WGN, int NS, int KB = 128>
struct GemmCfg {
  static constexpr int NW = WGM * WGN, THREADS = 64 * NW;
  static constexpr int WM = BM / WGM, WN = BN / WGN, MT = WM / 16, NT = WN / 16;
  static constexpr int CPR = KB / 16;
  static constexpr int stage_bytes = (BM + BN) * KB;
  static constexpr int main_bytes = NS * stage_bytes;
  static constexpr int EPAD = WN + 4;
  static constexpr int epi_bytes = NW * 16 * EPAD * 4;
  static constexpr int bytes = main_bytes > epi_bytes ? main_bytes : epi_bytes;
  static_assert(KB == 128 || KB == 64, "stage row bytes");
// ... 420 lines not shown
      const float* src = Cs + rr * EPAD + cc * 8;
      const float4 a0 = *reinterpret_cast<const float4*>(src), a1 = *reinterpret_cast<const float4*>(src + 4);
      V8 x{{a0.x, a0.y, a0.z, a0.w, a1.x, a1.y, a1.z, a1.w}};
      const RowIn& ri = rbuf[i % RB][t];
      if constexpr (LNCONS) {
        float m, rstd;
        if constexpr (LNF == 3) {
          const float2 ms = *reinterpret_cast<const float2*>(ln_rows + 2 * (i * 16 + rr));
          m = ms.x;
          rstd = ms.y;
        } else {
        const float m0 = __uint_as_float(ri.s0.x), m1 = __uint_as_float(ri.s1.x);
        m = mul_nc(sum8(add_nc(ln_w0 * m0, ln_w1 * m1)), ln_inv_np);
        const float e0 = ln_m2_term(__uint_as_float(ri.s0.y), m0, m), e1 = ln_m2_term(__uint_as_float(ri.s1.y), m1, m);
        rstd = ln_rstd(sum8(add_nc(ln_w0 * e0, ln_w1 * e1)), ln_inv_np, g.ln_eps);
        }
#pragma unroll
        for (int e = 0; e < 8; e += 2) {
          const f32x2 t = f32x2{x.v[e], x.v[e + 1]} - f32x2{m, m} * f32x2{lnA.v[e], lnA.v[e + 1]};
          const f32x2 y = f32x2{rstd, rstd} * t + f32x2{lnB.v[e], lnB.v[e + 1]};
          x.v[e] = y.x;
          x.v[e + 1] = y.y;
        }
      }
      if constexpr (BIAS && !LNCONS) {
#pragma unroll
        for (int e = 0; e < 8; ++e) x.v[e] = add_nc(x.v[e], bias8.v[e]);
      }
      if constexpr (EPI == EPI_QKV) {
        const V8 cs = as_v8(ri);
#pragma unroll
        for (int p = 0; p < 4; ++p) {
          const float c = cs.v[2 * p], sn = cs.v[2 * p + 1];
          const f32x2 ab = {x.v[2 * p], x.v[2 * p + 1]};
          f32x2 r;
          {
#pragma clang fp contract(off)
            const f32x2 pc = ab * c, ps = f32x2{ab.y, ab.x} * sn;
            r = pc + f32x2{-ps.x, ps.y};
            r = (rope_on ? r : ab) * qsc;
          }
          x.v[2 * p] = r.x;
          x.v[2 * p + 1] = r.y;
        }
        (void)row;
        store8_rs<TC, AUX>(dst, (uint32_t)(((ps_sq[t] * g.heads + head) * g.seq_len + ps_pos[t]) * 64 + dh), x);
        advance(ps_sq[t], ps_pos[t]);
      } else if constexpr (EPI == EPI_RESID || EPI == EPI_RESID16) {
        V8 c;
        if constexpr (PREF)
          c = pre[PREF ? i : 0][PREF ? t : 0];
        else
          c = as_v8(ri);
        const bool keep = !masked || ri.kb;
        V8 o;
#pragma unroll
        for (int e = 0; e < 8; ++e) o.v[e] = resid_add(c.v[e], gate8.v[e], x.v[e], keep);
        store8_rs<ResT<TC, EPI>, AUX>(dst, (uint32_t)((int64_t)row * g.ldc + col), o);
        if constexpr (LNF == 1 || LNF == 4) {
          V8 hr, hv;
          f32x2 s2 = {0.f, 0.f};
#pragma unroll
          for (int e = 0; e < 8; e += 2) {
            const f32x2 h2 = {to_f32(from_f32<TC>(o.v[e])), to_f32(from_f32<TC>(o.v[e + 1]))};
            hr.v[e] = h2.x;
            hr.v[e + 1] = h2.y;
            if constexpr (LNF == 1) {
              const f32x2 v2 = h2 * f32x2{lnA.v[e], lnA.v[e + 1]};
              hv.v[e] = v2.x;
              hv.v[e + 1] = v2.y;
              s2 += h2;
            }
          }
          if constexpr (LNF == 1) store8_rs<TC, AUX>(ln_dst, (uint32_t)((int64_t)row * g.ldc + col), hv);
          const float mean = LNF == 4 ? 0.f : sum8(s2.x + s2.y) * (1.f / 64.f);
          f32x2 q2 = {0.f, 0.f};
#pragma unroll
          for (int e = 0; e < 8; e += 2) {
            const f32x2 dv = f32x2{hr.v[e], hr.v[e + 1]} - f32x2{mean, mean};
            q2 += dv * dv;
          }
          const float m2 = sum8(q2.x + q2.y);
          __builtin_amdgcn_raw_buffer_store_b64(u32x2_t{__float_as_uint(mean), __float_as_uint(m2)}, ln_st,
                                                (uint32_t)((row * ln_np + ln_p) * 8), 0, AUX);
        }
      } else if constexpr (EPI == EPI_GELU_TANH || EPI == EPI_GELU_ERF_OP) {
        if constexpr (EPI == EPI_GELU_TANH && is16<TC>()) {
#pragma unroll
          for (int e = 0; e < 8; e += 2) {
            const f32x2 gv = gelu_tanh_fast2(f32x2{x.v[e], x.v[e + 1]});
            x.v[e] = gv.x;
            x.v[e + 1] = gv.y;
          }
        } else {
#pragma unroll
          for (int e = 0; e < 8; ++e) x.v[e] = EPI == EPI_GELU_ERF_OP ? gelu_erf(x.v[e]) : gelu_tanh(x.v[e]);
        }
        store8_rs<TC, AUX>(dst, (uint32_t)((int64_t)row * g.ldc + col), x);
      } else if constexpr (EPI == EPI_STORE16) {
        store8_rs<TC, AUX>(dst, (uint32_t)((int64_t)row * g.ldc + col), x);
      } else if constexpr (EPI == EPI_INPROJ) {
        V8 o0, o1;
#pragma unroll
        for (int e = 0; e < 4; ++e) {
          o0.v[e] = x.v[e] + __uint_as_float(ri.d0[e]);
          o0.v[e + 4] = x.v[e + 4] + __uint_as_float(ri.d1[e]);
          o1.v[e] = x.v[e] + __uint_as_float(ri.e0[e]);
          o1.v[e + 4] = x.v[e + 4] + __uint_as_float(ri.e1[e]);
        }
        constexpr uint32_t kPast = 0xF0000000u / 4;
        store8_rs<float, AUX>(dst, row < g.M ? (uint32_t)((int64_t)row * g.ldc + col) : kPast, o0);
        if (g.dual_rows)
          store8_rs<float, AUX>(dst, row < g.M ? (uint32_t)((int64_t)(row + g.dual_rows) * g.ldc + col) : kPast, o1);
      } else {
        store8_rs<float, AUX>(dst, (uint32_t)((int64_t)row * g.ldc + col), x);
      }
    }
    __builtin_amdgcn_fence(__ATOMIC_RELEASE, "wavefront");
    __builtin_amdgcn_wave_barrier();
    __builtin_amdgcn_fence(__ATOMIC_ACQUIRE, "wavefront");
  });
}
template <typename TC, int EPI, int MT, int NT, int WN, int EPAD, bool PREF, int AUX = 0, int PD = 1, int PM, int PT>
F5H_DEV void epilogue_fast(const GemmArgs& g, const f32x4 (&acc)[MT][NT], float* Cs, int rbase, int cbase,
                           int lane, const V8 (&pre)[PM][PT], const float* ln_rows = nullptr) {
  if constexpr (WN == 64 && is16<TC>() && AUX == 0) {
    if constexpr (EPI == EPI_RESID16) {
      if (g.ln_part && g.ln_rms) {
        if (g.bias)
          epilogue_fast_t<TC, EPI, MT, NT, WN, EPAD, PREF, true, PM, PT, AUX, PD, 4>(g, acc, Cs, rbase, cbase, lane, pre);
        else
          epilogue_fast_t<TC, EPI, MT, NT, WN, EPAD, PREF, false, PM, PT, AUX, PD, 4>(g, acc, Cs, rbase, cbase, lane, pre);
        return;
      }
      if (g.ln_part) {
        if (g.bias)
          epilogue_fast_t<TC, EPI, MT, NT, WN, EPAD, PREF, true, PM, PT, AUX, PD, 1>(g, acc, Cs, rbase, cbase, lane, pre);
        else
          epilogue_fast_t<TC, EPI, MT, NT, WN, EPAD, PREF, false, PM, PT, AUX, PD, 1>(g, acc, Cs, rbase, cbase, lane, pre);
        return;
      }
    } else if constexpr (EPI == EPI_GELU_TANH || EPI == EPI_QKV) {
      if (g.ln_part_in && ln_rows) {
        if (g.bias)
          epilogue_fast_t<TC, EPI, MT, NT, WN, EPAD, PREF, true, PM, PT, AUX, PD, 3>(g, acc, Cs, rbase, cbase, lane, pre,
                                                                                   ln_rows);
        else
          epilogue_fast_t<TC, EPI, MT, NT, WN, EPAD, PREF, false, PM, PT, AUX, PD, 3>(g, acc, Cs, rbase, cbase, lane, pre,
                                                                                    ln_rows);
        return;
      }
      if (g.ln_part_in) {
        if (g.bias)
          epilogue_fast_t<TC, EPI, MT, NT, WN, EPAD, PREF, true, PM, PT, AUX, PD, 2>(g, acc, Cs, rbase, cbase, lane, pre);
        else
          epilogue_fast_t<TC, EPI, MT, NT, WN, EPAD, PREF, false, PM, PT, AUX, PD, 2>(g, acc, Cs, rbase, cbase, lane, pre);
        return;
      }
    }
  }
  if (g.bias)
    epilogue_fast_t<TC, EPI, MT, NT, WN, EPAD, PREF, true, PM, PT, AUX, PD>(g, acc, Cs, rbase, cbase, lane, pre);
  else
    epilogue_fast_t<TC, EPI, MT, NT, WN, EPAD, PREF, false, PM, PT, AUX, PD>(g, acc, Cs, rbase, cbase, lane, pre);
}

template <typename TC, int EPI, int MT, int NT, bool PREF, bool BIAS, int PM, int PT, int AUX = 0>
F5H_DEV void epilogue_direct_t(const GemmArgs& g, const f32x4 (&acc)[MT][NT], int rbase, int cbase, int lane,
                               const V8 (&pre)[PM][PT]) {
  static_assert(NT % 2 == 0, "column blocks in pairs");
  constexpr int NP = NT / 2;
  const int fr = lane & 15, q = lane >> 4;
  const int coff = 16 * (q & 1) + 8 * (q >> 1);
  V8 bias8[NP], gate8[NP];
  int colp[NP];
#pragma unroll
  for (int jp = 0; jp < NP; ++jp) {
    colp[jp] = cbase + 32 * jp + coff;
    bias8[jp] = V8{};
    if constexpr (BIAS) bias8[jp] = load8(g.bias + colp[jp]);
    gate8[jp] = V8{{1.f, 1.f, 1.f, 1.f, 1.f, 1.f, 1.f, 1.f}};
    if constexpr (EPI == EPI_RESID || EPI == EPI_RESID16)
      if (g.gate) gate8[jp] = load8(g.gate + colp[jp]);
  }
  int which = 0, head = 0, dh[NP];
  bool rope_on = false;
  float qsc = 1.f;
  __amdgpu_buffer_rsrc_t dst;
  if constexpr (EPI == EPI_QKV) {
    const int inner = g.heads * 64;
    which = __builtin_amdgcn_readfirstlane(fdiv(cbase, inner));
    head = __builtin_amdgcn_readfirstlane((cbase - which * inner) >> 6);
#pragma unroll
    for (int jp = 0; jp < NP; ++jp) dh[jp] = (colp[jp] - which * inner) & 63;
    rope_on = which < 2 && head < g.rope_heads;
    qsc = (which == 0 && g.q_scale != 0.f) ? g.q_scale : 1.f;
    dst = rsrc_of(which == 0 ? g.q : (which == 1 ? g.k : g.v), (uint64_t)g.M * inner * sizeof(TC));
  } else {
    constexpr int OES = (EPI == EPI_STORE || EPI == EPI_RESID || EPI == EPI_INPROJ) ? 4 : (int)sizeof(TC);
    dst = rsrc_of(g.C, (uint64_t)(g.M + (EPI == EPI_INPROJ ? g.dual_rows : 0)) * g.ldc * OES);
  }
  struct RowIn {
    u32x4 d0, d1;
    u32x4 e0, e1;
  };
  const __amdgpu_buffer_rsrc_t rk = rsrc_of(g.rowkeep, g.rowkeep ? (uint64_t)g.M : 0);
  const bool masked = g.rowkeep != nullptr;
  int pf_sq = 0, pf_pos = 0, ps_sq = 0, ps_pos = 0;
  if constexpr (EPI == EPI_QKV) {
// ... 65 lines not shown
        x.v[r + 4] = __uint_as_float(sw[1]);
      }
      const int col = colp[jp];
      if constexpr (BIAS) {
#pragma unroll
        for (int e = 0; e < 8; ++e) x.v[e] = add_nc(x.v[e], bias8[jp].v[e]);
      }
      const RowIn& ri = rbuf[i & 1][jp];
      if constexpr (EPI == EPI_QKV) {
        const V8 cs = as_v8(ri);
#pragma unroll
        for (int p = 0; p < 4; ++p) {
          const float c = cs.v[2 * p], sn = cs.v[2 * p + 1];
          const f32x2 ab = {x.v[2 * p], x.v[2 * p + 1]};
          f32x2 rr;
          {
#pragma clang fp contract(off)
            const f32x2 pc = ab * c, ps = f32x2{ab.y, ab.x} * sn;
            rr = pc + f32x2{-ps.x, ps.y};
            rr = (rope_on ? rr : ab) * qsc;
          }
          x.v[2 * p] = rr.x;
          x.v[2 * p + 1] = rr.y;
        }
        (void)row;
        store8_rs<TC, AUX>(dst, (uint32_t)(((ps_sq * g.heads + head) * g.seq_len + ps_pos) * 64 + dh[jp]), x);
      } else if constexpr (EPI == EPI_RESID || EPI == EPI_RESID16) {
        V8 c;
        if constexpr (PREF)
          c = pre[PREF ? i : 0][PREF ? jp : 0];
        else
          c = as_v8(ri);
        const bool keep = !masked || kb[i & 1];
        V8 o;
#pragma unroll
        for (int e = 0; e < 8; ++e) o.v[e] = resid_add(c.v[e], gate8[jp].v[e], x.v[e], keep);
        store8_rs<ResT<TC, EPI>, AUX>(dst, (uint32_t)((int64_t)row * g.ldc + col), o);
      } else if constexpr (EPI == EPI_GELU_TANH || EPI == EPI_GELU_ERF_OP) {
        if constexpr (EPI == EPI_GELU_TANH && is16<TC>()) {
#pragma unroll
          for (int e = 0; e < 8; e += 2) {
            const f32x2 gv = gelu_tanh_fast2(f32x2{x.v[e], x.v[e + 1]});
            x.v[e] = gv.x;
            x.v[e + 1] = gv.y;
          }
        } else {
#pragma unroll
          for (int e = 0; e < 8; ++e) x.v[e] = EPI == EPI_GELU_ERF_OP ? gelu_erf(x.v[e]) : gelu_tanh(x.v[e]);
        }
        store8_rs<TC, AUX>(dst, (uint32_t)((int64_t)row * g.ldc + col), x);
      } else if constexpr (EPI == EPI_STORE16) {
        store8_rs<TC, AUX>(dst, (uint32_t)((int64_t)row * g.ldc + col), x);
      } else if constexpr (EPI == EPI_INPROJ) {
        V8 o0, o1;
#pragma unroll
        for (int e = 0; e < 4; ++e) {
          o0.v[e] = x.v[e] + __uint_as_float(ri.d0[e]);
          o0.v[e + 4] = x.v[e + 4] + __uint_as_float(ri.d1[e]);
          o1.v[e] = x.v[e] + __uint_as_float(ri.e0[e]);
          o1.v[e + 4] = x.v[e + 4] + __uint_as_float(ri.e1[e]);
        }
        constexpr uint32_t kPast = 0xF0000000u / 4;
        store8_rs<float, AUX>(dst, row < g.M ? (uint32_t)((int64_t)row * g.ldc + col) : kPast, o0);
        if (g.dual_rows)
          store8_rs<float, AUX>(dst, row < g.M ? (uint32_t)((int64_t)(row + g.dual_rows) * g.ldc + col) : kPast, o1);
      } else {
        store8_rs<float, AUX>(dst, (uint32_t)((int64_t)row * g.ldc + col), x);
      }
    }
    if constexpr (EPI == EPI_QKV) advance(ps_sq, ps_pos);
  });
}
template <typename TC, int EPI, int MT, int NT, bool PREF, int AUX = 0, int PM, int PT>
F5H_DEV void epilogue_direct(const GemmArgs& g, const f32x4 (&acc)[MT][NT], int rbase, int cbase, int lane,
                             const V8 (&pre)[PM][PT]) {
  if (g.bias)
    epilogue_direct_t<TC, EPI, MT, NT, PREF, true, PM, PT, AUX>(g, acc, rbase, cbase, lane, pre);
  else
    epilogue_direct_t<TC, EPI, MT, NT, PREF, false, PM, PT, AUX>(g, acc, rbase, cbase, lane, pre);
}


template <typename TC, int EPI, int BM, int BN, int WGM, int WGN, int NS, bool FAST, int KB, bool PUB = false,
          bool CHAIN = false>
F5H_DEV void gemm_body(const GemmArgs& g, const int b, const int nwg, uint4* lds, const ChainDep& dep) {
  const ProbeT probe_t = probe_enter(g.probe);
  typedef GemmCfg<BM, BN, WGM, WGN, NS, KB> C;
  constexpr int E = elems16<TC>();
  constexpr int CPR = C::CPR, SLABS = KB / 64;
  constexpr int BKE = CPR * E;
  constexpr int NW = C::NW, WM = C::WM, WN = C::WN, MT = C::MT, NT = C::NT;
  constexpr int AR = BM * CPR / C::THREADS, BR = BN * CPR / C::THREADS;
  constexpr int DPS = AR + BR;
  static_assert(NS >= 2 && NS <= 6 && (NS - 1) * DPS <= 63, "LDS stages");
  typedef typename Slab<TC>::frag frag;
  auto swz = [](int row, int chunk) { return KB == 128 ? swz128g(row, chunk) : swz64(row, chunk); };

  constexpr int stage_u4 = C::stage_bytes / 16;
  const int tid = threadIdx.x, lane = tid & 63, wid = tid >> 6;
  const int wm = wid / WGN, wn = wid % WGN;
  const int ntn = (g.N + BN - 1) / BN;
  const int xq = nwg >> 3, xr = nwg & 7, xcd = b & 7;
  const int bid = (xcd < xr ? xcd * (xq + 1) : xr * (xq + 1) + (xcd - xr) * xq) + (b >> 3);
  if constexpr (CHAIN) {
    if (bid >= ((g.M + BM - 1) / BM) * ntn) return;
  }
  const int mrow = g.live_len ? spread8(bid / ntn, (g.M + BM - 1) / BM) : bid / ntn;
  const int m0 = mrow * BM, n0 = (bid % ntn) * BN;
  if constexpr (EPI == EPI_RESID || EPI == EPI_RESID16) {
    if (!tile_live(g, m0, BM)) {
      probe_exit(g.probe, probe_t);
      return;
    }
  }
  const TC* A = reinterpret_cast<const TC*>(g.A);
  const TC* W = reinterpret_cast<const TC*>(g.W);

  const int wid_s = __builtin_amdgcn_readfirstlane(wid);
  constexpr int ESZ = (int)sizeof(TC);
  const uint32_t abytes = (uint32_t)(min(BM, g.M - m0) * g.lda * ESZ);
  const uint32_t wbytes = (uint32_t)(min(BN, g.N - n0) * g.ldw * ESZ);
  uint32_t aoff[AR], boff[BR];
  static_for<0, AR>([&](auto I) {
    constexpr int i = decltype(I)::value;
    const int p = (i * NW + wid) * 64 + lane, row = p / CPR, slot = p % CPR;
    aoff[i] = (uint32_t)((row * g.lda + swz(row, slot) * E) * ESZ);
  });
  static_for<0, BR>([&](auto I) {
    constexpr int i = decltype(I)::value;
    const int p = (i * NW + wid) * 64 + lane, row = p / CPR, slot = p % CPR;
    boff[i] = (uint32_t)((row * g.ldw + swz(row, slot) * E) * ESZ);
  });
  const TC* A2 = reinterpret_cast<const TC*>(g.A2);
  const __amdgpu_buffer_rsrc_t wrs =
      rsrc_of(W + (int64_t)n0 * g.ldw, wbytes);
  auto stage_a = [&](int buf, int k0) {
    uint4* As = lds + buf * stage_u4;
    const bool second = A2 && k0 >= g.k_split;
    const TC* Ab = second ? A2 : A;
    const int ka = second ? k0 - g.k_split : k0;
    const __amdgpu_buffer_rsrc_t ars =
        rsrc_of(Ab + (int64_t)m0 * g.lda, abytes);
    static_for<0, AR>([&](auto I) {
      constexpr int i = decltype(I)::value;
      dma16(ars, (LDS_PTR(void))(As + (i * NW + wid_s) * 64), aoff[i], ka * ESZ);
    });
  };
  auto stage_w = [&](int buf, int k0) {
    uint4* Bs = lds + buf * stage_u4 + BM * CPR;
    static_for<0, BR>([&](auto I) {
      constexpr int i = decltype(I)::value;
      dma16(wrs, (LDS_PTR(void))(Bs + (i * NW + wid_s) * 64), boff[i], k0 * ESZ);
    });
  };
  auto stage = [&](int buf, int k0) {
    stage_a(buf, k0);
    stage_w(buf, k0);
  };

  const uint32_t lds0 = (uint32_t)(uintptr_t)(LDS_PTR(void))lds;
  const int fr = lane & 15, q = lane >> 4;
  uint32_t abase[SLABS], bbase[SLABS];
#pragma unroll
  for (int s = 0; s < SLABS; ++s) {
    abase[s] = lds0 + (wm * WM + fr) * KB + swz(fr, s * 4 + q) * 16;
    bbase[s] = lds0 + BM * KB + (wn * WN + fr) * KB + swz(fr, s * 4 + q) * 16;
  }
// ... 38 lines not shown
  for (int kt = 0; kt < nk; ++kt) {
    if (kt == 0) {
      if constexpr (CHAIN)
        wait_stages<AR, NPRE>(min(NS - 2, nk - 1));
      else
        wait_stages<DPS, NPRE>(min(NS - 2, nk - 1));
    } else {
      wait_stages<DPS>(min(NS - 2, nk - 1 - kt));
    }
    __builtin_amdgcn_s_barrier();
    if (kt == 0) probe_mark(g.probe, probe_t, 1);
    const uint32_t soff = (uint32_t)((kt % NS) * C::stage_bytes);
    u32x4 ar[SLABS][MT], br[SLABS][NT];
#pragma unroll
    for (int s = 0; s < SLABS; ++s) {
      static_for<0, MT>([&](auto I) {
        constexpr int i = decltype(I)::value;
        ar[s][i] = lds_read_b128<i * 16 * KB>(abase[s] + soff);
      });
      static_for<0, NT>([&](auto J) {
        constexpr int j = decltype(J)::value;
        br[s][j] = lds_read_b128<j * 16 * KB>(bbase[s] + soff);
      });
    }
    if (kt + NS - 1 < nk) stage((kt + NS - 1) % NS, (kt + NS - 1) * BKE);
    if constexpr (SLABS == 1) {
      asm volatile("s_waitcnt lgkmcnt(0)" ::: "memory");
#pragma unroll
      for (int i = 0; i < MT; ++i) asm volatile("" : "+v"(ar[0][i]));
#pragma unroll
      for (int j = 0; j < NT; ++j) asm volatile("" : "+v"(br[0][j]));
      __builtin_amdgcn_sched_barrier(0);
#pragma unroll
      for (int i = 0; i < MT; ++i)
#pragma unroll
        for (int j = 0; j < NT; ++j)
          acc[i][j] = Slab<TC>::mma(__builtin_bit_cast(frag, br[0][j]), __builtin_bit_cast(frag, ar[0][i]), acc[i][j]);
      continue;
    } else {
    asm volatile("s_waitcnt lgkmcnt(%0)" ::"i"(MT + NT) : "memory");
#pragma unroll
    for (int i = 0; i < MT; ++i) asm volatile("" : "+v"(ar[0][i]));
#pragma unroll
    for (int j = 0; j < NT; ++j) asm volatile("" : "+v"(br[0][j]));
    __builtin_amdgcn_sched_barrier(0);
#pragma unroll
    for (int i = 0; i < MT; ++i)
#pragma unroll
      for (int j = 0; j < NT; ++j)
        acc[i][j] = Slab<TC>::mma(__builtin_bit_cast(frag, br[0][j]), __builtin_bit_cast(frag, ar[0][i]), acc[i][j]);
    __builtin_amdgcn_sched_barrier(0);
    asm volatile("s_waitcnt lgkmcnt(0)" ::: "memory");
#pragma unroll
    for (int i = 0; i < MT; ++i) asm volatile("" : "+v"(ar[1][i]));
#pragma unroll
    for (int j = 0; j < NT; ++j) asm volatile("" : "+v"(br[1][j]));
    __builtin_amdgcn_sched_barrier(0);
#pragma unroll
    for (int i = 0; i < MT; ++i)
#pragma unroll
      for (int j = 0; j < NT; ++j)
        acc[i][j] = Slab<TC>::mma(__builtin_bit_cast(frag, br[SLABS - 1][j]), __builtin_bit_cast(frag, ar[SLABS - 1][i]),
                                  acc[i][j]);
    }
  }
  __builtin_amdgcn_s_waitcnt(0x0F70);
  __syncthreads();
  probe_mark(g.probe, probe_t, 2);
  float* const ln_rows = reinterpret_cast<float*>(lds) + NW * 16 * C::EPAD;
  if constexpr (LNC) {
    static_assert(C::bytes >= (NW * 16 * C::EPAD + 2 * BM) * 4, "LDS for the fold's row statistics");
    if (g.ln_part_in) {
      if (tid < BM) ln_row_stats(g, lnraw, ln_rows + 2 * tid);
      __syncthreads();
    }
  }

  float* Cs = reinterpret_cast<float*>(lds) + wid * 16 * C::EPAD;
  constexpr int CH = WN / 8;
  constexpr int TPC = 16 * CH / 64;
  constexpr bool FAST_EPI = FAST && NT % 2 == 0;
  static_assert(FAST_EPI || !PUB, "the chain publishes after the fast (LDS-strip) epilogue");
  if constexpr (FAST_EPI) {
    epilogue_fast<TC, EPI, MT, NT, WN, C::EPAD, PREF, PUB ? kAuxWT : 0>(g, acc, Cs, m0 + wm * WM, n0 + wn * WN, lane,
                                                                         pre, LNC ? ln_rows + 2 * wm * WM : nullptr);
    if constexpr (PUB) chain_publish(dep, g.M, m0, BM);
  }
  if constexpr (!FAST_EPI) {
#pragma unroll
    for (int i = 0; i < MT; ++i) {
#pragma unroll
      for (int j = 0; j < NT; ++j) *reinterpret_cast<f32x4*>(Cs + fr * C::EPAD + j * 16 + 4 * q) = acc[i][j];
      __builtin_amdgcn_fence(__ATOMIC_RELEASE, "wavefront");
      __builtin_amdgcn_wave_barrier();
      __builtin_amdgcn_fence(__ATOMIC_ACQUIRE, "wavefront");
#pragma unroll
      for (int t = 0; t < TPC; ++t) {
        const int idx = t * 64 + lane, rr = idx / CH, cc = idx % CH;
        const int row = m0 + wm * WM + i * 16 + rr, col = n0 + wn * WN + cc * 8;
        const float* src = Cs + rr * C::EPAD + cc * 8;
        float4 a = *reinterpret_cast<const float4*>(src), b = *reinterpret_cast<const float4*>(src + 4);
        if (row < g.M && col < g.N)
          epi8<TC, EPI>(g, row, col, V8{{a.x, a.y, a.z, a.w, b.x, b.y, b.z, b.w}}, PREF ? &pre[PREF ? i : 0][PREF ? t : 0] : nullptr);
      }
      __builtin_amdgcn_fence(__ATOMIC_RELEASE, "wavefront");
      __builtin_amdgcn_wave_barrier();
      __builtin_amdgcn_fence(__ATOMIC_ACQUIRE, "wavefront");
    }
  }
  probe_exit(g.probe, probe_t);
}

template <typename TC, int EPI, int BM, int BN, int WGM, int WGN, int NS, bool FAST = false, int KB = 128>
__global__ __launch_bounds__(64 * WGM * WGN, 2) void gemm_kernel(GemmArgs g) {
  __shared__ __attribute__((aligned(16))) uint4 lds[GemmCfg<BM, BN, WGM, WGN, NS, KB>::bytes / 16];
  gemm_body<TC, EPI, BM, BN, WGM, WGN, NS, FAST, KB>(g, blockIdx.x, gridDim.x, lds, ChainDep{});
}

template <int BM, int BN, int WGM2, int WGN2, int KS, int D>
struct PPCfg {
  static constexpr int WM = BM / 2 / WGM2, WN = BN / WGN2, MT = WM / 16, NT = WN / 16;
  static constexpr int stage_bytes = (BM + BN) * 64;
  static constexpr int R = D + 1;
  static constexpr int ring_bytes = R * KS * stage_bytes;
  static constexpr int EPAD = WN + 4;
  static constexpr int epi_bytes = 8 * 16 * EPAD * 4;
  static constexpr int bytes = ring_bytes > epi_bytes ? ring_bytes : epi_bytes;
  static constexpr int NA = BM / 64, NB = BN / 64;
  static_assert(WGM2 * WGN2 == 4, "4 waves per group");
  static_assert(MT * 16 == WM && NT * 16 == WN, "16x16 fragments");
  static_assert(NA * 64 == BM && NB * 64 == BN, "whole DMA rounds");
  static_assert(bytes <= 160 * 1024, "LDS");
};

template <typename TC, int EPI, int BM, int BN, int WGM2, int WGN2, int KS, int D, bool FAST = false>
__global__ __launch_bounds__(512, 1) void gemm_pp_kernel(GemmArgs g) {
  const ProbeT probe_t = probe_enter(g.probe);
  typedef PPCfg<BM, BN, WGM2, WGN2, KS, D> C;
  constexpr int WM = C::WM, WN = C::WN, MT = C::MT, NT = C::NT, NA = C::NA, NB = C::NB;
  constexpr int SB = C::stage_bytes, PB = KS * SB;
  __shared__ __attribute__((aligned(16))) uint4 lds[C::bytes / 16];

  const int tid = threadIdx.x, lane = tid & 63;
  const int wid = __builtin_amdgcn_readfirstlane(tid >> 6);
  const int grp = wid >> 2, w4 = wid & 3;
  const int wm = w4 / WGN2, wn = w4 % WGN2;
  const int ntn = (g.N + BN - 1) / BN;
  const int nwg = gridDim.x, b = blockIdx.x, xq = nwg >> 3, xr = nwg & 7, xcd = b & 7;
  const int bid = (xcd < xr ? xcd * (xq + 1) : xr * (xq + 1) + (xcd - xr) * xq) + (b >> 3);
  const int mrow = g.live_len ? spread8(bid / ntn, (g.M + BM - 1) / BM) : bid / ntn;
  const int m0 = mrow * BM, n0 = (bid % ntn) * BN;
  if constexpr (EPI == EPI_RESID || EPI == EPI_RESID16) {
    if (!tile_live(g, m0, BM)) {
      probe_exit(g.probe, probe_t);
      return;
    }
  }
  const TC* A = reinterpret_cast<const TC*>(g.A);
  const TC* W = reinterpret_cast<const TC*>(g.W);

  constexpr int NI = NA > NB ? NA : NB;
  const int nI = grp == 0 ? NA : NB;
  const int ld = grp == 0 ? g.lda : g.ldw;
  const TC* pan = grp == 0 ? A + (int64_t)m0 * g.lda : W + (int64_t)n0 * g.ldw;
  const TC* pan2 = (grp == 0 && g.A2) ? reinterpret_cast<const TC*>(g.A2) + (int64_t)m0 * g.lda : pan;
  const uint32_t pbytes = (uint32_t)((grp == 0 ? min(BM, g.M - m0) : min(BN, g.N - n0)) * ld * 2);
  uint32_t voff[NI], dst_off[NI];
#pragma unroll
  for (int i = 0; i < NI; ++i) {
    const int row = (i * 4 + w4) * 16 + (lane >> 2);
    const int lc = swz64(row, lane & 3);
    voff[i] = (uint32_t)((row * ld + lc * 8) * 2);
    dst_off[i] = (uint32_t)((grp == 0 ? 0 : BM * 64) + (i * 4 + w4) * 16 * 64);
  }
  char* lds_c = reinterpret_cast<char*>(lds);
  auto dma_phase = [&](int p) {
    const int slot = p % C::R;
#pragma unroll
    for (int s = 0; s < KS; ++s) {
      const int k0 = (p * KS + s) * 32;
      const bool second = grp == 0 && g.A2 && k0 >= g.k_split;
      const __amdgpu_buffer_rsrc_t rs =
          rsrc_of(second ? pan2 : pan, pbytes);
      const int ks = second ? k0 - g.k_split : k0;
#pragma unroll
      for (int i = 0; i < NI; ++i)
        if (i < nI)
          dma16(rs, (LDS_PTR(void))(lds_c + slot * PB + s * SB + dst_off[i]), voff[i], ks * 2);
    }
  };
  auto wait_dma = [&](int need, int issued) {
    const int younger = min(max(issued - need, 0), D - 1);
    static_for<0, D>([&](auto Y) {
      constexpr int y = decltype(Y)::value;
      if (younger == y) {
        if (grp == 0)
          asm volatile("s_waitcnt vmcnt(%0)" ::"i"(y * KS * NA) : "memory");
        else
          asm volatile("s_waitcnt vmcnt(%0)" ::"i"(y * KS * NB) : "memory");
// ... 419 lines not shown
    __builtin_amdgcn_s_barrier();
    __builtin_amdgcn_sched_barrier(0);
  };
  using I0 = std::integral_constant<int, 0>;
  using I1 = std::integral_constant<int, 1>;

  const int T = g.K / KT;
  dma_half(0, 0);
  dma_half(0, 2);
  dma_half(0, 3);
  dma_half(0, 1);
  if (T > 1) {
    dma_half(1, 0);
    dma_half(1, 2);
    dma_half(1, 3);
    asm volatile("s_waitcnt vmcnt(6)" ::: "memory");
  } else {
    asm volatile("s_waitcnt vmcnt(0)" ::: "memory");
  }
  __builtin_amdgcn_s_barrier();
  probe_mark(g.probe, probe_t, 1);
  for (int t = 0; t < T; ++t) {
    const uint32_t so = (uint32_t)((t & 1) * BUF);
    const bool more1 = t + 1 < T, more2 = t + 2 < T;
    read_b(so, I0{}, bl);
    read_a(so, I0{});
    if (more1) dma_half(t + 1, 1);
    compute(I0{}, I0{}, bl);
    read_b(so, I1{}, br);
    if (more2) dma_half(t + 2, 0);
    compute(I0{}, I1{}, br);
    read_a(so, I1{});
    if (more2) dma_half(t + 2, 2);
    compute(I1{}, I1{}, br);
    if (more2) {
      dma_half(t + 2, 3);
      asm volatile("s_waitcnt vmcnt(6)" ::: "memory");
    } else {
      asm volatile("s_waitcnt vmcnt(0)" ::: "memory");
    }
    compute(I1{}, I0{}, bl);
  }
  __builtin_amdgcn_s_waitcnt(0x0F70);
  __syncthreads();
  probe_mark(g.probe, probe_t, 2);

  float* Cs = reinterpret_cast<float*>(lds) + wid * 16 * EPAD;
  static_for<0, 4>([&](auto QB) {
    constexpr int ha = decltype(QB)::value >> 1, hb = decltype(QB)::value & 1;
    const int rbase = m0 + ha * 128 + wr * 64, cbase = n0 + hb * 128 + wc * QW;
    if constexpr (FAST) {
      const V8 none[1][1] = {};
      epilogue_fast<TC, EPI, 4, 2, QW, EPAD, false>(g, acc[ha][hb], Cs, rbase, cbase, lane, none);
    } else {
      constexpr int CH = QW / 8;
#pragma unroll
      for (int i = 0; i < 4; ++i) {
#pragma unroll
        for (int j = 0; j < 2; ++j)
          *reinterpret_cast<f32x4*>(Cs + fr * EPAD + j * 16 + 4 * q) = acc[ha][hb][i][j];
        __builtin_amdgcn_fence(__ATOMIC_RELEASE, "wavefront");
        __builtin_amdgcn_wave_barrier();
        __builtin_amdgcn_fence(__ATOMIC_ACQUIRE, "wavefront");
        for (int idx = lane; idx < 16 * CH; idx += 64) {
          const int rr = idx / CH, cc = idx % CH;
          const int row = rbase + i * 16 + rr, col = cbase + cc * 8;
          const float* sp = Cs + rr * EPAD + cc * 8;
          float4 x0 = *reinterpret_cast<const float4*>(sp), x1 = *reinterpret_cast<const float4*>(sp + 4);
          if (row < g.M && col < g.N)
            epi8<TC, EPI>(g, row, col, V8{{x0.x, x0.y, x0.z, x0.w, x1.x, x1.y, x1.z, x1.w}});
        }
        __builtin_amdgcn_fence(__ATOMIC_RELEASE, "wavefront");
        __builtin_amdgcn_wave_barrier();
        __builtin_amdgcn_fence(__ATOMIC_ACQUIRE, "wavefront");
      }
    }
  });
  probe_exit(g.probe, probe_t);
}

template <typename TC, int EPI>
static void launch_8p(const GemmArgs& a, hipStream_t st);

template <int EPI>
static bool fast_epi_ok(const GemmArgs& a, int BN) {
  const uint64_t span = (uint64_t)(a.M + a.dual_rows) * (uint64_t)std::max<int64_t>(a.ldc, a.N) * 4;
  return a.N % BN == 0 && (EPI == EPI_QKV || a.ldc % 8 == 0) && (EPI != EPI_INPROJ || a.ld_add % 8 == 0) &&
         span < 0xF0000000ull;
}

template <typename TC, int EPI, int BM, int BN, int WGM2, int WGN2, int KS, int D>
static void launch_pp(const GemmArgs& a, hipStream_t st) {
  const int tiles = ((a.M + BM - 1) / BM) * ((a.N + BN - 1) / BN);
  constexpr bool HOT = EPI == EPI_QKV || EPI == EPI_RESID || EPI == EPI_RESID16 || EPI == EPI_GELU_TANH ||
                       EPI == EPI_GELU_ERF_OP || EPI == EPI_STORE || EPI == EPI_STORE16 || EPI == EPI_INPROJ;
  if constexpr (HOT) {
    if (fast_epi_ok<EPI>(a, BN)) {
      hipLaunchKernelGGL((gemm_pp_kernel<TC, EPI, BM, BN, WGM2, WGN2, KS, D, true>), dim3(tiles), dim3(512), 0, st, a);
      return;
    }
  }
  hipLaunchKernelGGL((gemm_pp_kernel<TC, EPI, BM, BN, WGM2, WGN2, KS, D>), dim3(tiles), dim3(512), 0, st, a);
}

int gemm_num_cus();
int gemm_group_m();
template <typename TC, int EPI, int BM, int BN, int WGM2, int WGN2, int KS, int D>
static void launch_ppp(const GemmArgs& a, hipStream_t st) {
  const int tiles = ((a.M + BM - 1) / BM) * ((a.N + BN - 1) / BN);
  constexpr bool HOT = EPI == EPI_QKV || EPI == EPI_RESID || EPI == EPI_RESID16 || EPI == EPI_GELU_TANH ||
                       EPI == EPI_GELU_ERF_OP || EPI == EPI_STORE || EPI == EPI_STORE16 || EPI == EPI_INPROJ;
  if constexpr (HOT) {
    if (fast_epi_ok<EPI>(a, BN) && a.K >= 32 * KS * D) {
      const int grid = std::min(tiles, gemm_num_cus());
      GemmArgs b = a;
      b.group_m = gemm_group_m();
      hipLaunchKernelGGL((gemm_ppp_kernel<TC, EPI, BM, BN, WGM2, WGN2, KS, D>), dim3(grid), dim3(512), 0, st, b);
      return;
    }
  }
  launch_pp<TC, EPI, BM, BN, WGM2, WGN2, KS, D>(a, st);
}

template <typename TC, int EPI>
static void launch_8p(const GemmArgs& a, hipStream_t st) {
  const int tiles = ((a.M + 255) / 256) * ((a.N + 255) / 256);
  constexpr bool HOT = EPI == EPI_QKV || EPI == EPI_RESID || EPI == EPI_RESID16 || EPI == EPI_GELU_TANH ||
                       EPI == EPI_GELU_ERF_OP || EPI == EPI_STORE || EPI == EPI_STORE16 || EPI == EPI_INPROJ;
  if constexpr (HOT) {
    if (fast_epi_ok<EPI>(a, 256)) {
      hipLaunchKernelGGL((gemm_8p_kernel<TC, EPI, true>), dim3(tiles), dim3(512), 0, st, a);
      return;
    }
  }
  hipLaunchKernelGGL((gemm_8p_kernel<TC, EPI>), dim3(tiles), dim3(512), 0, st, a);
}

template <typename TC, int EPI, int BM, int BN, int WGM, int WGN, int NS, int KB = 128>
static void launch_cfg(const GemmArgs& a, hipStream_t st) {
  const int tiles = ((a.M + BM - 1) / BM) * ((a.N + BN - 1) / BN);
  constexpr bool HOT = EPI == EPI_QKV || EPI == EPI_RESID || EPI == EPI_RESID16 || EPI == EPI_GELU_TANH ||
                       EPI == EPI_GELU_ERF_OP || EPI == EPI_STORE || EPI == EPI_STORE16 || EPI == EPI_INPROJ;
  if constexpr (HOT) {
    if (fast_epi_ok<EPI>(a, BN)) {
      hipLaunchKernelGGL((gemm_kernel<TC, EPI, BM, BN, WGM, WGN, NS, true, KB>), dim3(tiles), dim3(64 * WGM * WGN), 0,
                         st, a);
      return;
    }
  }
  hipLaunchKernelGGL((gemm_kernel<TC, EPI, BM, BN, WGM, WGN, NS, false, KB>), dim3(tiles), dim3(64 * WGM * WGN), 0, st,
                     a);
}

template <typename TC, int EPI>
static hipError_t launch_t(const GemmArgs& a, hipStream_t st) {
  if (a.M == 0) return hipSuccess;
  int cfg = 0;
  if constexpr (is16<TC>()) cfg = gemm_select_cfg(a);
  if ((a.ln_part || a.ln_part_in) && (cfg == 12 || cfg == 13)) cfg = 11;
  if ((a.ln_part || a.ln_part_in) && cfg == 11 && !fast_epi_ok<EPI>(a, 256)) cfg = 1;
  if (a.hs || a.ln_part || a.ln_part_in) {
    const bool prod = a.ln_part && EPI == EPI_RESID16 && (a.ln_rms ? !a.hs && !a.hs_scale : a.hs && a.hs_scale);
    const bool cons = a.ln_part_in && (EPI == EPI_GELU_TANH || EPI == EPI_QKV) &&
                      (a.ln_rms ? !a.ln_u && !a.ln_v : a.ln_u && a.ln_v);
    const int bn = cfg == 11 ? 256 : 128;
    if (!is16<TC>() || (a.ln_part && a.ln_part_in) || !(prod || cons) || a.ln_nparts <= 0 || a.ln_nparts > 16 ||
        (cfg != 0 && cfg != 1 && cfg != 5 && cfg != 11) || !fast_epi_ok<EPI>(a, bn) || (a.rowkeep && !a.ln_rms) ||
        a.live_len)
      return hipErrorInvalidValue;
  }
  switch (cfg) {
    case 0: launch_cfg<TC, EPI, 64, 128, 2, 2, 3>(a, st); break;
    case 1: launch_cfg<TC, EPI, 128, 128, 2, 2, 2>(a, st); break;
    case 5: launch_cfg<TC, EPI, 192, 128, 2, 2, 2>(a, st); break;
    default:
      if constexpr (is16<TC>()) {
        if (a.K % 64) return hipErrorInvalidValue;
        if (cfg != 11 && cfg != 12 && cfg != 13) return hipErrorInvalidValue;
        if (cfg == 11)
          launch_pp<TC, EPI, 256, 256, 1, 4, 1, 3>(a, st);
        else if (cfg == 13)
          launch_ppp<TC, EPI, 256, 256, 1, 4, 1, 3>(a, st);
        else
          launch_8p<TC, EPI>(a, st);
        break;
      }
      return hipErrorInvalidValue;
  }
  return hipGetLastError();
}

template <typename TC>
static hipError_t launch_epi(int epi, const GemmArgs& a, hipStream_t st) {
  switch (epi) {
    case EPI_STORE: return launch_t<TC, EPI_STORE>(a, st);
    case EPI_SILU: return launch_t<TC, EPI_SILU>(a, st);
    case EPI_GELU_TANH: return launch_t<TC, EPI_GELU_TANH>(a, st);
    case EPI_GELU_ERF: return launch_t<TC, EPI_GELU_ERF>(a, st);
    case EPI_RESID: return launch_t<TC, EPI_RESID>(a, st);
    case EPI_RESID16: return launch_t<TC, EPI_RESID16>(a, st);
    case EPI_RESID_FILL: return launch_t<TC, EPI_RESID_FILL>(a, st);
    case EPI_INPROJ: return launch_t<TC, EPI_INPROJ>(a, st);
    case EPI_QKV: return launch_t<TC, EPI_QKV>(a, st);
    case EPI_GELU_ERF_OP: return launch_t<TC, EPI_GELU_ERF_OP>(a, st);
    case EPI_STORE16: return launch_t<TC, EPI_STORE16>(a, st);
  }
  return hipErrorInvalidValue;
}


}
```

f5-tts_amd/csrc/kernels.h:

```cpp
#pragma once
#include <hip/hip_runtime.h>
#include <stdint.h>

namespace f5h {

enum ComputeMode { F5H_C_FP32 = 0, F5H_C_BF16 = 1, F5H_C_FP16 = 2 };

enum Epi {
  EPI_STORE = 0,
  EPI_SILU = 1,
  EPI_GELU_TANH = 2,
  EPI_GELU_ERF = 3,
  EPI_RESID = 4,
  EPI_RESID_FILL = 5,
  EPI_INPROJ = 6,
  EPI_QKV = 7,
  EPI_GELU_ERF_OP = 8,
  EPI_RESID16 = 9,
  EPI_STORE16 = 10,
};

constexpr int kProbeTicks = 512, kProbeSites = 64, kProbeLanes = 16, kProbeStride = 16, kProbeEvery = 4;
constexpr int64_t kProbeRow = (int64_t)kProbeTicks * kProbeLanes * kProbeStride;
constexpr int64_t kProbeEnd = kProbeRow * kProbeSites;
struct DevProbe {
  unsigned long long* slots;
  const int* tick;
  unsigned long long* tl;
};
constexpr int kTimelineWG = 8192;

struct GemmArgs {
  const void* A; int64_t lda;
  const void* W; int64_t ldw;
  int M, N, K;
  const float* bias;
  void* C; int64_t ldc;
  const float* gate;
  const uint8_t* rowkeep;
  const float* add; int64_t ld_add;
  int64_t dual_rows;
  const float2* rope;
  int seq_len;
  int heads, rope_heads;
  void* q; void* k; void* v;
  float q_scale;
  DevProbe probe;
  const void* resid;
  const void* A2; int k_split;
  const int32_t* live_len; int live_seq;
  int group_m;
  void* hs; const float* hs_scale; float* ln_part;
  const float* ln_part_in; int ln_nparts; const float* ln_u; const float* ln_v;
  int ln_rms; float ln_eps;
};

__host__ __device__ inline bool tile_live_rows(const int32_t* live_len, int live_seq, int M, int m0, int BM) {
  if (!live_len) return true;
  const int last = (m0 + BM < M ? m0 + BM : M) - 1;
  for (int s = m0 / live_seq; s <= last / live_seq; ++s) {
    const int r0 = s * live_seq;
    const int lo = m0 > r0 ? m0 : r0;
    const int hi_tile = last + 1, hi_live = r0 + live_len[s];
    if (lo < (hi_tile < hi_live ? hi_tile : hi_live)) return true;
  }
  return false;
}

hipError_t gemm(int compute, int epi, const GemmArgs& a, hipStream_t st);
void gemm_force_config(int cfg);

struct AttnArgs {
  const void* q; const void* k; const void* v; void* o;
  int S, H, L;
  const int32_t* kv_len;
  const int32_t* q_len;
  float scale;
  int prescaled;
  DevProbe probe;
  int force_safe;
};
hipError_t attention(int compute, const AttnArgs& a, hipStream_t st);
void attention_force_safe(int on);

struct ConvArgs {
  const void* x; int x_f32;
  const void* w;
  const float* bias;
  const uint8_t* rowkeep;
  int S, L, d;
  int mode;
  void* y; int64_t y_seq_stride; int64_t y_row_off;
  const float* resid;
};
hipError_t conv_pos(int compute, const ConvArgs& a, hipStream_t st);

hipError_t time_sinus(const float* t_host, int n, float* out, hipStream_t st);
hipError_t time_sinus_dev(const float* tg, int n, float* out, hipStream_t st);
hipError_t silu_to_op(int compute, const float* x, void* y, int64_t n, hipStream_t st);
hipError_t ln_modulate(int compute, const void* h, int h16, int M, int d, const float* shift, const float* scale,
                       void* out, hipStream_t st);
hipError_t rms_norm_g(int compute, const void* h, int h16, int M, int d, const float* g, void* out, hipStream_t st);
hipError_t scale_cols(int compute, const void* W, int64_t rows, int K, const float* g, void* out, hipStream_t st);
hipError_t rope_table(int L, float2* out, hipStream_t st);
struct TextEmbArgs {
  const int64_t* text; int B, nt, N, td;
  const int32_t* seq_len;
  const float* table;
  const float* freqs;
  int mask_padding;
  float* out_c; float* out_u;
  uint8_t* keep;
};
hipError_t text_embed(const TextEmbArgs& a, hipStream_t st);
hipError_t dwconv_ln(int compute, const float* x, int S, int L, int C, const float* dw_w, const float* dw_b,
                     const float* ln_w, const float* ln_b, void* out, hipStream_t st);
hipError_t grn(int compute, const float* x, int S, int L, int C, const float* gamma, const float* beta,
               float* scratch , void* out, hipStream_t st);
hipError_t build_ct(int compute, const float* cond, const uint8_t* cond_mask, const float* text_c,
                    const float* text_u, int B, int N, int td, int S, int drop_audio, int drop_text, void* out,
                    hipStream_t st);
hipError_t pack_y(int compute, const float* y, int rows, int mel, void* ypad, hipStream_t st);
struct EulerArgs {
  float* y; int B, N, mel;
  const float* p; int64_t p_seq_stride; int p_row_off; int64_t p_ld;
  int use_cfg; float cfg; float dt;
  void* ypad; int compute;
  float* traj;
  const int* kstep; const float* tgrid; float* const* trajp;
  const float* next_src; int64_t next_stride; int next_n; float* next_dst; int nfe;
  unsigned* arrive; int* tick;
};
hipError_t cfg_euler(const EulerArgs& a, hipStream_t st);
constexpr int kOdeMethods = 3;
struct OdeTableau {
  int stages;
  float c[4], a[16], b[4];
};
constexpr float kOneThird = (float)(1.0 / 3.0), kTwoThirds = (float)(2.0 / 3.0);
constexpr OdeTableau ode_tableau(int method) {
  return method == 1   ? OdeTableau{2, {0.f, 0.5f}, {0.f, 0.f, 0.f, 0.f, 0.5f}, {0.f, 1.f}}
         : method == 2 ? OdeTableau{4,
                                    {0.f, kOneThird, kTwoThirds, 1.f},
                                    {0.f, 0.f, 0.f, 0.f, kOneThird, 0.f, 0.f, 0.f, -kOneThird, 1.f, 0.f, 0.f, 1.f, -1.f, 1.f, 0.f},
                                    {0.125f, 0.375f, 0.375f, 0.125f}}
                       : OdeTableau{1, {0.f}, {0.f}, {1.f}};
}
constexpr int ode_kept_slopes(int method) { return method == 2 ? 3 : 0; }
struct RkArgs {
  float* y; int B, N, mel;
  const float* p; int64_t p_seq_stride; int p_row_off; int64_t p_ld;
  int use_cfg; float cfg;
  void* ypad; int compute;
  int method;
  float* kbuf;
  int* keval; const float* sgrid; float* const* trajp;
  const float* next_src; int64_t next_stride; int next_n; float* next_dst; int neval;
  unsigned* arrive; int* tick;
};
hipError_t cfg_rk(const RkArgs& a, hipStream_t st);
hipError_t grid_upload(const float* t_host, int n, float* out, hipStream_t st);
hipError_t step_begin(const int* kstep, const float* src, int64_t stride, int n, float* dst, hipStream_t st);
hipError_t stamp_begin(unsigned long long* slots, const int* tick, hipStream_t st);
hipError_t stamp_end(unsigned long long* slots, const int* tick, hipStream_t st);
hipError_t step_advance(int* kstep, int* tick, hipStream_t st);
// ... 66 lines not shown
```

f5-tts_amd/f5_tts_amd/_lib.py:

```python

from __future__ import annotations

import ctypes
import os

import torch

_HERE = os.path.dirname(os.path.abspath(__file__))
LIB_PATH = os.environ.get("F5H_LIB", os.path.join(_HERE, "lib", "libf5h.so"))

F5H_DIT, F5H_UNETT = 0, 1
F5H_FP32, F5H_BF16, F5H_FP16 = 0, 1, 2
COMPUTE = {"fp32": F5H_FP32, "bf16": F5H_BF16, "fp16": F5H_FP16}
F5H_DT_F32, F5H_DT_BF16, F5H_DT_F16 = 0, 1, 2
F5H_EULER, F5H_MIDPOINT, F5H_RK4 = 0, 1, 2
ODE_METHOD = {"euler": F5H_EULER, "midpoint": F5H_MIDPOINT, "rk4": F5H_RK4}

EXPORTS = (
    "f5h_engine_create_views",
    "f5h_engine_create",
    "f5h_engine_destroy",
    "f5h_release_pending",
    "f5h_workspace_size",
    "f5h_sample",
    "f5h_workspace_size_ode",
    "f5h_sample_ode",
    "f5h_debug_ode_tableau",
    "f5h_debug_ode_eval_times",
    "f5h_forward",
    "f5h_probe_enable",
    "f5h_probe_read",
    "f5h_probe_timeline",
    "f5h_set_graph_mode",
    "f5h_set_cfg_streams",
    "f5h_graph_stats",
    "f5h_last_call_host_ms",
    "f5h_set_pad_skip",
    "f5h_set_chain",
    "f5h_chain_stats",
    "f5h_chain_debug_spin_limit",
    "f5h_set_ln_fold",
    "f5h_ln_fold_stats",
    "f5h_op_linear",
    "f5h_op_attention",
    "f5h_op_attention_qlen",
    "f5h_op_conv_pos",
    "f5h_op_norm",
    "f5h_op_dwconv_ln",
    "f5h_op_grn",
    "f5h_op_gemm_epi",
    "f5h_op_lnfold_uv",
    "f5h_op_scale_cols",
    "f5h_gemm_force_config",
    "f5h_attn_force_safe",
    "f5h_debug_tile_live",
    "f5h_vocos_create",
    "f5h_vocos_destroy",
    "f5h_vocos_workspace_size",
    "f5h_vocos_decode",
    "f5h_mel_create",
    "f5h_mel_destroy",
    "f5h_mel_workspace_size",
    "f5h_mel_forward",
    "f5h_last_error",
    "f5h_version",
)

KCLASS = {"ffn1": 0, "attention": 1, "qkv": 2, "ffn2": 3, "conv": 4, "out": 5, "norm": 6, "chain": 7}


class Arch(ctypes.Structure):
    _fields_ = [(n, ctypes.c_int32) for n in (
        "backbone", "dim", "depth", "heads", "dim_head", "ff_dim", "text_dim", "text_num_embeds", "mel_dim",
        "conv_layers", "text_mask_padding", "pe_attn_head", "attn_mask_enabled", "compute")]


class VocosArch(ctypes.Structure):
    _fields_ = [(n, ctypes.c_int32) for n in (
        "input_channels", "dim", "intermediate_dim", "num_layers", "n_fft", "hop_length", "compute")]


class MelArch(ctypes.Structure):
    _fields_ = [(n, ctypes.c_int32) for n in ("n_fft", "hop_length", "n_mels", "sample_rate")]


class Weight(ctypes.Structure):
    _fields_ = [("name", ctypes.c_char_p), ("data", ctypes.c_void_p), ("numel", ctypes.c_int64)]


class TensorView(ctypes.Structure):
    _fields_ = [("name", ctypes.c_char_p), ("data", ctypes.c_void_p), ("dtype", ctypes.c_int32),
                ("on_device", ctypes.c_int32), ("numel", ctypes.c_int64)]


class SampleArgs(ctypes.Structure):
    _fields_ = [
        ("B", ctypes.c_int32), ("N", ctypes.c_int32), ("nt", ctypes.c_int32), ("nfe", ctypes.c_int32),
        ("cond", ctypes.c_void_p), ("cond_mask", ctypes.c_void_p), ("text", ctypes.c_void_p),
        ("duration", ctypes.c_void_p), ("y0", ctypes.c_void_p), ("t_grid", ctypes.c_void_p),
        ("cfg_strength", ctypes.c_float), ("use_batch_mask", ctypes.c_int32),
        ("out", ctypes.c_void_p), ("trajectory", ctypes.c_void_p),
    ]


class ForwardArgs(ctypes.Structure):
    _fields_ = [
        ("B", ctypes.c_int32), ("N", ctypes.c_int32), ("nt", ctypes.c_int32),
        ("x", ctypes.c_void_p), ("cond", ctypes.c_void_p), ("cond_mask", ctypes.c_void_p),
        ("text", ctypes.c_void_p), ("duration", ctypes.c_void_p), ("t", ctypes.c_float),
        ("use_batch_mask", ctypes.c_int32), ("pred", ctypes.c_void_p),
        ("cfg_infer", ctypes.c_int32), ("drop_audio_cond", ctypes.c_int32), ("drop_text", ctypes.c_int32),
        ("t_dev", ctypes.c_void_p), ("text_cache", ctypes.c_int32),
    ]


class OpGemmArgs(ctypes.Structure):
    _fields_ = [
        ("compute", ctypes.c_int32), ("epi", ctypes.c_int32), ("M", ctypes.c_int32), ("N", ctypes.c_int32),
        ("K", ctypes.c_int32), ("k_split", ctypes.c_int32),
        ("A", ctypes.c_void_p), ("A2", ctypes.c_void_p), ("W", ctypes.c_void_p), ("bias", ctypes.c_void_p),
        ("C", ctypes.c_void_p), ("resid", ctypes.c_void_p), ("gate", ctypes.c_void_p), ("rowkeep", ctypes.c_void_p),
        ("live_len", ctypes.c_void_p), ("live_seq", ctypes.c_int32),
        ("seq_len", ctypes.c_int32), ("heads", ctypes.c_int32), ("rope_heads", ctypes.c_int32),
        ("q_scale", ctypes.c_float),
        ("add", ctypes.c_void_p), ("ld_add", ctypes.c_int64), ("dual_rows", ctypes.c_int64),
# ... 24 lines not shown
        raise RuntimeError(_load_error)
    L = ctypes.CDLL(LIB_PATH)
    vp, i32, i64, sz = ctypes.c_void_p, ctypes.c_int32, ctypes.c_int64, ctypes.c_size_t
    L.f5h_engine_create.argtypes = [ctypes.POINTER(Arch), ctypes.POINTER(Weight), i32, i32, ctypes.POINTER(vp)]
    L.f5h_engine_create.restype = ctypes.c_int
    L.f5h_engine_create_views.argtypes = [ctypes.POINTER(Arch), ctypes.POINTER(TensorView), i32, i32,
                                          ctypes.POINTER(vp)]
    L.f5h_engine_create_views.restype = ctypes.c_int
    L.f5h_engine_destroy.argtypes = [vp]
    L.f5h_engine_destroy.restype = None
    L.f5h_release_pending.argtypes = [i32]
    L.f5h_release_pending.restype = ctypes.c_int
    L.f5h_workspace_size.argtypes = [vp, i32, i32, i32, i32, i32]
    L.f5h_workspace_size.restype = sz
    L.f5h_sample.argtypes = [vp, vp, ctypes.POINTER(SampleArgs), vp, sz]
    L.f5h_sample.restype = ctypes.c_int
    if hasattr(L, "f5h_sample_ode"):
        L.f5h_workspace_size_ode.argtypes = [vp, i32, i32, i32, i32, i32, i32]
        L.f5h_workspace_size_ode.restype = sz
        L.f5h_sample_ode.argtypes = [vp, vp, ctypes.POINTER(SampleArgs), i32, vp, sz]
        L.f5h_sample_ode.restype = ctypes.c_int
        fp = ctypes.POINTER(ctypes.c_float)
        L.f5h_debug_ode_tableau.argtypes = [i32, ctypes.POINTER(i32), fp, fp, fp]
        L.f5h_debug_ode_tableau.restype = ctypes.c_int
        L.f5h_debug_ode_eval_times.argtypes = [i32, i32, fp, i32, fp]
        L.f5h_debug_ode_eval_times.restype = ctypes.c_int
    L.f5h_forward.argtypes = [vp, vp, ctypes.POINTER(ForwardArgs), vp, sz]
    L.f5h_forward.restype = ctypes.c_int
    L.f5h_probe_enable.argtypes = [vp, i32, i32]
    L.f5h_probe_enable.restype = ctypes.c_int
    L.f5h_probe_read.argtypes = [vp, ctypes.POINTER(i64), ctypes.POINTER(ctypes.c_double)]
    L.f5h_probe_read.restype = ctypes.c_int
    L.f5h_probe_timeline.argtypes = [vp, ctypes.POINTER(ctypes.c_uint64), i32, ctypes.POINTER(i32),
                                     ctypes.POINTER(ctypes.c_double)]
    L.f5h_probe_timeline.restype = ctypes.c_int
    L.f5h_set_graph_mode.argtypes = [vp, i32]
    L.f5h_set_graph_mode.restype = ctypes.c_int
    L.f5h_set_cfg_streams.argtypes = [vp, i32]
    L.f5h_set_cfg_streams.restype = ctypes.c_int
    L.f5h_graph_stats.argtypes = [vp, ctypes.POINTER(i64), ctypes.POINTER(i64), ctypes.POINTER(i32)]
    L.f5h_graph_stats.restype = ctypes.c_int
    if hasattr(L, "f5h_last_call_host_ms"):
        L.f5h_last_call_host_ms.argtypes = [vp, ctypes.POINTER(ctypes.c_double), i32]
        L.f5h_last_call_host_ms.restype = ctypes.c_int
    L.f5h_set_pad_skip.argtypes = [vp, i32]
    L.f5h_set_pad_skip.restype = ctypes.c_int
    L.f5h_op_linear.argtypes = [vp, i32, i32, i32, i32, vp, vp, vp, vp, vp, sz]
    L.f5h_op_linear.restype = ctypes.c_int
    L.f5h_op_attention.argtypes = [vp, i32, i32, i32, i32, vp, vp, vp, vp, i32, vp, vp, sz]
    L.f5h_op_attention.restype = ctypes.c_int
    if hasattr(L, "f5h_op_gemm_epi"):
        L.f5h_op_attention_qlen.argtypes = [vp, i32, i32, i32, i32, vp, vp, vp, vp, vp, i32, vp, vp, sz]
        L.f5h_op_attention_qlen.restype = ctypes.c_int
        L.f5h_op_conv_pos.argtypes = [vp, i32, i32, i32, i32, vp, vp, vp, vp, i32, vp, i32, i64, i64, vp, vp, sz]
        L.f5h_op_conv_pos.restype = ctypes.c_int
        L.f5h_op_norm.argtypes = [vp, i32, i32, i32, i32, i32, vp, vp, vp, vp, vp, sz]
        L.f5h_op_norm.restype = ctypes.c_int
        L.f5h_op_dwconv_ln.argtypes = [vp, i32, i32, i32, i32, vp, vp, vp, vp, vp, vp, vp, sz]
        L.f5h_op_dwconv_ln.restype = ctypes.c_int
        L.f5h_op_grn.argtypes = [vp, i32, i32, i32, i32, vp, vp, vp, vp, vp, sz]
        L.f5h_op_grn.restype = ctypes.c_int
        L.f5h_op_gemm_epi.argtypes = [vp, ctypes.POINTER(OpGemmArgs), vp, sz]
        L.f5h_op_gemm_epi.restype = ctypes.c_int
        if hasattr(L, "f5h_op_lnfold_uv"):
            L.f5h_op_lnfold_uv.argtypes = [vp, i32, i32, i32, i32, i32, vp, i64, i64, vp, vp, vp, sz]
            L.f5h_op_lnfold_uv.restype = ctypes.c_int
            L.f5h_op_scale_cols.argtypes = [vp, i32, i64, i32, vp, vp, vp, vp, sz]
            L.f5h_op_scale_cols.restype = ctypes.c_int
    L.f5h_gemm_force_config.argtypes = [i32]
    L.f5h_gemm_force_config.restype = ctypes.c_int
    if hasattr(L, "f5h_attn_force_safe"):
        L.f5h_attn_force_safe.argtypes = [i32]
        L.f5h_attn_force_safe.restype = ctypes.c_int
    if hasattr(L, "f5h_set_chain"):
        L.f5h_set_chain.argtypes = [vp, i32]
        L.f5h_set_chain.restype = ctypes.c_int
        L.f5h_chain_stats.argtypes = [vp, ctypes.POINTER(i64), ctypes.POINTER(i32), ctypes.POINTER(i64)]
        L.f5h_chain_stats.restype = ctypes.c_int
    if hasattr(L, "f5h_set_ln_fold"):
        L.f5h_set_ln_fold.argtypes = [vp, i32]
        L.f5h_set_ln_fold.restype = ctypes.c_int
        L.f5h_ln_fold_stats.argtypes = [vp, ctypes.POINTER(i32), ctypes.POINTER(i64)]
        L.f5h_ln_fold_stats.restype = ctypes.c_int
    if hasattr(L, "f5h_chain_debug_spin_limit"):
        L.f5h_chain_debug_spin_limit.argtypes = [i64]
        L.f5h_chain_debug_spin_limit.restype = ctypes.c_int
    if hasattr(L, "f5h_debug_tile_live"):
        L.f5h_debug_tile_live.argtypes = [vp, i32, i32, i32, i32]
        L.f5h_debug_tile_live.restype = ctypes.c_int
    L.f5h_vocos_create.argtypes = [ctypes.POINTER(VocosArch), ctypes.POINTER(Weight), i32, i32, ctypes.POINTER(vp)]
    L.f5h_vocos_create.restype = ctypes.c_int
    L.f5h_vocos_destroy.argtypes = [vp]
    L.f5h_vocos_destroy.restype = None
    L.f5h_vocos_workspace_size.argtypes = [vp, i32, i32]
    L.f5h_vocos_workspace_size.restype = sz
    L.f5h_vocos_decode.argtypes = [vp, vp, i32, i32, vp, vp, vp, sz]
    L.f5h_vocos_decode.restype = ctypes.c_int
    L.f5h_mel_create.argtypes = [ctypes.POINTER(MelArch), i32, ctypes.POINTER(vp)]
    L.f5h_mel_create.restype = ctypes.c_int
    L.f5h_mel_destroy.argtypes = [vp]
    L.f5h_mel_destroy.restype = None
    L.f5h_mel_workspace_size.argtypes = [vp, i32, i32]
    L.f5h_mel_workspace_size.restype = sz
    L.f5h_mel_forward.argtypes = [vp, vp, i32, i32, vp, vp, vp, sz]
    L.f5h_mel_forward.restype = ctypes.c_int
    L.f5h_last_error.argtypes = []
    L.f5h_last_error.restype = ctypes.c_char_p
    L.f5h_version.argtypes = []
    L.f5h_version.restype = ctypes.c_char_p
    _lib = L
    return L


def has_ode() -> bool:
    return hasattr(lib(), "f5h_sample_ode")


def check(rc: int, what: str = "f5h"):
    if rc != 0:
        msg = lib().f5h_last_error().decode(errors="replace")
        raise RuntimeError(f"{what} failed (status {rc}): {msg}")


def ptr(t) -> int | None:
    return None if t is None else t.data_ptr()


def stream_handle(device=None) -> int:
    return torch.cuda.current_stream(device).cuda_stream
```

f5-tts_amd/f5_tts_amd/engine.py:

```python

from __future__ import annotations

import ctypes
import threading

import numpy as np
import torch

from . import _lib


_VIEW_DT = {torch.float32: _lib.F5H_DT_F32, torch.bfloat16: _lib.F5H_DT_BF16, torch.float16: _lib.F5H_DT_F16}


def _arch_struct(arch: dict, compute: str) -> _lib.Arch:
    a = _lib.Arch()
    a.backbone = _lib.F5H_DIT if arch["backbone"] == "DiT" else _lib.F5H_UNETT
    a.dim = arch["dim"]
    a.depth = arch["depth"]
    a.heads = arch["heads"]
    a.dim_head = arch.get("dim_head", 64)
    a.ff_dim = int(arch["dim"] * arch["ff_mult"])
    a.text_dim = arch["text_dim"] if arch.get("text_dim") is not None else arch["mel_dim"]
    a.text_num_embeds = arch["text_num_embeds"]
# ... 23 lines not shown
    def __init__(self, arch: dict, weights: dict, compute: str = "bf16", device=None):
        L = _lib.lib()
        self.arch = dict(arch)
        self.compute = compute
        self.device = torch.device("cuda", torch.cuda.current_device() if device is None else
                                   torch.device(device).index or 0)
        keep, views = [], []
        for k, v in weights.items():
            k = k[len("transformer."):] if k.startswith("transformer.") else k
            t = v.detach() if isinstance(v, torch.Tensor) else torch.from_numpy(np.ascontiguousarray(v))
            if t.dtype not in _VIEW_DT:
                t = t.to(torch.float32)
            if t.is_cuda and t.device != self.device:
                t = t.to(self.device)
            t = t.contiguous()
            keep.append(t)
            views.append((k.encode(), t))
        arr = (_lib.TensorView * len(views))()
        for i, (name, t) in enumerate(views):
            arr[i].name = name
            arr[i].data = t.data_ptr()
            arr[i].dtype = _VIEW_DT[t.dtype]
            arr[i].on_device = int(t.is_cuda)
            arr[i].numel = t.numel()
        a = _arch_struct(self.arch, compute)
        h = ctypes.c_void_p()
        with torch.cuda.device(self.device):
            if any(t.is_cuda for t in keep):
                torch.cuda.current_stream(self.device).synchronize()
            _lib.check(L.f5h_engine_create_views(ctypes.byref(a), arr, len(views), self.device.index,
                                                 ctypes.byref(h)), "f5h_engine_create_views")
        del keep
        self._h = h
        self._lock = threading.Lock()
        self._ws_cache: dict = {}

    def __del__(self):
        h = getattr(self, "_h", None)
        if h is not None and h.value:
            try:
                _lib.lib().f5h_engine_destroy(h)
            except Exception:
                pass
            self._h = None

    def workspace_bytes(self, B, N, nt, nfe, use_cfg=True, method="euler") -> int:
        m = _ode_method(method)
        if not _lib.has_ode():
            return int(_lib.lib().f5h_workspace_size(self._h, B, N, nt, nfe, int(use_cfg)))
        return int(_lib.lib().f5h_workspace_size_ode(self._h, B, N, nt, nfe, int(use_cfg), m))

    def _workspace(self, nbytes):
        return torch.empty(max(nbytes, 256), dtype=torch.uint8, device=self.device)

    def _cached_workspace(self, nbytes, stream):
        with self._lock:
            ent = self._ws_cache.get((stream, nbytes))
            if ent is None:
                if len(self._ws_cache) >= 4:
                    self._ws_cache.pop(next(iter(self._ws_cache)))
                ent = (self._workspace(nbytes), threading.Lock())
                self._ws_cache[(stream, nbytes)] = ent
            return ent

    def set_graph_mode(self, on: bool):
        _lib.check(_lib.lib().f5h_set_graph_mode(self._h, int(bool(on))), "set_graph_mode")

    def set_cfg_streams(self, n: int):
        _lib.check(_lib.lib().f5h_set_cfg_streams(self._h, int(n)), "set_cfg_streams")

    def set_pad_skip(self, on: bool):
        _lib.check(_lib.lib().f5h_set_pad_skip(self._h, int(bool(on))), "set_pad_skip")

    def set_chain(self, on: bool):
        _lib.check(_lib.lib().f5h_set_chain(self._h, int(bool(on))), "set_chain")

    def set_ln_fold(self, on: bool):
        _lib.check(_lib.lib().f5h_set_ln_fold(self._h, int(bool(on))), "set_ln_fold")

    def ln_fold_stats(self):
        sup, n = ctypes.c_int32(), ctypes.c_int64()
        _lib.check(_lib.lib().f5h_ln_fold_stats(self._h, ctypes.byref(sup), ctypes.byref(n)), "ln_fold_stats")
        return bool(sup.value), int(n.value)

    def chain_stats(self):
        n, f, r = ctypes.c_int64(), ctypes.c_int32(), ctypes.c_int64()
        _lib.check(_lib.lib().f5h_chain_stats(self._h, ctypes.byref(n), ctypes.byref(f), ctypes.byref(r)),
                   "chain_stats")
        return int(n.value), int(f.value), int(r.value)

    HOST_PHASES = ("total", "prologue", "cache_lock", "reap", "capture", "instantiate", "launch", "final")

    def last_call_host_ms(self):
        buf = (ctypes.c_double * 8)()
        _lib.check(_lib.lib().f5h_last_call_host_ms(self._h, buf, 8), "last_call_host_ms")
        return {k: round(buf[i], 4) for i, k in enumerate(self.HOST_PHASES)}

    def graph_stats(self):
        cap, rep, n = ctypes.c_int64(), ctypes.c_int64(), ctypes.c_int32()
        _lib.check(_lib.lib().f5h_graph_stats(self._h, ctypes.byref(cap), ctypes.byref(rep), ctypes.byref(n)),
                   "graph_stats")
        return {"captures": cap.value, "replays": rep.value, "cached": n.value}

    def sample(self, cond, cond_mask, text, duration, y0, t_grid, cfg_strength, use_batch_mask,
               out=None, keep_trajectory=True, workspace=None, method="euler"):
        B, N, mel = cond.shape
        nt = text.shape[1]
        tg = np.ascontiguousarray(np.asarray(t_grid, dtype=np.float32))
        nfe = tg.shape[0] - 1
        cond = cond.to(self.device, torch.float32).contiguous()
        cmask = cond_mask.to(self.device, torch.uint8).contiguous()
        text = text.to(self.device, torch.int64).contiguous()
        dur = duration.to(self.device, torch.int32).contiguous()
        y0 = y0.to(self.device, torch.float32).contiguous()
        if out is None:
            out = torch.empty(B, N, mel, dtype=torch.float32, device=self.device)
        traj = (torch.empty(nfe + 1, B, N, mel, dtype=torch.float32, device=self.device)
                if keep_trajectory else None)
        use_cfg = cfg_strength >= 1e-5
        m = _ode_method(method)
        need = self.workspace_bytes(B, N, nt, nfe, use_cfg, method)
        stream = _lib.stream_handle(self.device)
        if workspace is not None and workspace.numel() >= need:
            ws, wlock = workspace, threading.Lock()
        else:
            ws, wlock = self._cached_workspace(need, stream)
        a = _lib.SampleArgs()
        a.B, a.N, a.nt, a.nfe = B, N, nt, nfe
        a.cond, a.cond_mask, a.text, a.duration, a.y0 = (cond.data_ptr(), cmask.data_ptr(), text.data_ptr(),
                                                         dur.data_ptr(), y0.data_ptr())
        a.t_grid = tg.ctypes.data
        a.cfg_strength = float(cfg_strength)
        a.use_batch_mask = int(bool(use_batch_mask))
        a.out = out.data_ptr()
        a.trajectory = traj.data_ptr() if traj is not None else None
        with torch.cuda.device(self.device), wlock:
            if _lib.has_ode():
                _lib.check(_lib.lib().f5h_sample_ode(self._h, stream, ctypes.byref(a), m, ws.data_ptr(), ws.numel()),
                           "f5h_sample_ode")
            else:
                _lib.check(_lib.lib().f5h_sample(self._h, stream, ctypes.byref(a), ws.data_ptr(), ws.numel()),
                           "f5h_sample")
        return out, traj

    def forward_workspace(self, B, N, nt, cfg_infer=True):
        return self._workspace(self.workspace_bytes(B, N, nt, 1, cfg_infer))

    def forward(self, x, cond, cond_mask, text, duration, t, use_batch_mask, cfg_infer=True,
                drop_audio_cond=False, drop_text=False, text_cache=0, workspace=None):
        B, N, mel = x.shape
        nt = text.shape[1]
        x = x.to(self.device, torch.float32).contiguous()
        cond = cond.to(self.device, torch.float32).contiguous()
        cmask = cond_mask.to(self.device, torch.uint8).contiguous()
        text = text.to(self.device, torch.int64).contiguous()
        dur = duration.to(self.device, torch.int32).contiguous()
        S = 2 * B if cfg_infer else B
        pred = torch.empty(S, N, mel, dtype=torch.float32, device=self.device)
        need = self.workspace_bytes(B, N, nt, 1, cfg_infer)
        if text_cache and (workspace is None or workspace.numel() < need):
            raise ValueError("text_cache needs a kept workspace of workspace_bytes(B, N, nt, 1, cfg_infer) bytes")
        ws = workspace if workspace is not None and workspace.numel() >= need else self._workspace(need)
        t_dev = None
        if torch.is_tensor(t):
            t_dev = t.reshape(-1)[:1].to(self.device, torch.float32).contiguous()
        a = _lib.ForwardArgs()
        a.B, a.N, a.nt = B, N, nt
        a.x, a.cond, a.cond_mask, a.text, a.duration = (x.data_ptr(), cond.data_ptr(), cmask.data_ptr(),
                                                        text.data_ptr(), dur.data_ptr())
        a.t = 0.0 if t_dev is not None else float(t)
        a.t_dev = t_dev.data_ptr() if t_dev is not None else None
        a.text_cache = int(text_cache)
        a.use_batch_mask = int(bool(use_batch_mask))
        a.pred = pred.data_ptr()
        a.cfg_infer = int(bool(cfg_infer))
        a.drop_audio_cond = int(bool(drop_audio_cond))
        a.drop_text = int(bool(drop_text))
        with torch.cuda.device(self.device):
            _lib.check(_lib.lib().f5h_forward(self._h, _lib.stream_handle(self.device), ctypes.byref(a),
                                              ws.data_ptr(), ws.numel()), "f5h_forward")
        return pred

    def probe(self, kclass: str | None):
        L = _lib.lib()
        if kclass is None:
            _lib.check(L.f5h_probe_enable(self._h, 0, 0), "probe")
        else:
            _lib.check(L.f5h_probe_enable(self._h, _lib.KCLASS[kclass], 1), "probe")

    def probe_timeline(self, max_wg: int = 8192):
        buf = (ctypes.c_uint64 * (4 * max_wg))()
        n, khz = ctypes.c_int32(), ctypes.c_double()
        _lib.check(_lib.lib().f5h_probe_timeline(self._h, buf, max_wg, ctypes.byref(n), ctypes.byref(khz)),
                   "probe_timeline")
        a = np.frombuffer(buf, dtype=np.uint64, count=4 * n.value).reshape(n.value, 4).astype(np.float64)
        if n.value == 0 or khz.value <= 0:
            return a
        t0 = a[:, 0][a[:, 0] > 0].min()
        return np.where(a > 0, (a - t0) * 1e3 / khz.value, np.nan)

    def probe_read(self):
        n = ctypes.c_int64()
        ms = ctypes.c_double()
        _lib.check(_lib.lib().f5h_probe_read(self._h, ctypes.byref(n), ctypes.byref(ms)), "probe_read")
        return n.value, ms.value


def op_linear(A, W, bias=None, compute="bf16"):
    M, K = A.shape
    N = W.shape[0]
    C = torch.empty(M, N, dtype=torch.float32, device=A.device)
    ws = torch.empty(((N + 127) // 128 * 128) * K * 4 + 512 + M * K * 4, dtype=torch.uint8, device=A.device)
    _lib.check(_lib.lib().f5h_op_linear(_lib.stream_handle(A.device), _lib.COMPUTE[compute], M, N, K,
                                        A.contiguous().data_ptr(), W.contiguous().data_ptr(), _lib.ptr(bias),
                                        C.data_ptr(), ws.data_ptr(), ws.numel()), "f5h_op_linear")
    return C


def op_attention(Q, K, V, kv_len=None, compute="bf16", q_prescaled=False, poison=False, q_len=None):
    S, H, N, D = Q.shape
    assert D == 64
    O = torch.empty(S, N, H * 64, dtype=torch.float32, device=Q.device)
    ws = torch.empty(Q.numel() * 8 + 1024, dtype=torch.uint8, device=Q.device)
    if poison:
        ws.fill_(0xFF)
    kv = None if kv_len is None else kv_len.to(Q.device, torch.int32).contiguous()
    if q_len is None:
        _lib.check(_lib.lib().f5h_op_attention(_lib.stream_handle(Q.device), _lib.COMPUTE[compute], S, H, N,
                                               Q.contiguous().data_ptr(), K.contiguous().data_ptr(),
                                               V.contiguous().data_ptr(), _lib.ptr(kv), int(bool(q_prescaled)),
                                               O.data_ptr(), ws.data_ptr(), ws.numel()), "f5h_op_attention")
        return O
    if poison:
        O.fill_(float("nan"))
    ql = q_len.to(Q.device, torch.int32).contiguous()
    _lib.check(_lib.lib().f5h_op_attention_qlen(_lib.stream_handle(Q.device), _lib.COMPUTE[compute], S, H, N,
                                                Q.contiguous().data_ptr(), K.contiguous().data_ptr(),
                                                V.contiguous().data_ptr(), _lib.ptr(kv), ql.data_ptr(),
                                                int(bool(q_prescaled)), O.data_ptr(), ws.data_ptr(), ws.numel()),
               "f5h_op_attention_qlen")
    return O


def _f32(t, dev=None):
    return None if t is None else t.to(device=dev or t.device, dtype=torch.float32).contiguous()


def _u8(t, dev):
    return None if t is None else t.to(device=dev, dtype=torch.uint8).contiguous()


def op_conv_pos(x, w, bias, rowkeep=None, mode=0, resid=None, x_as_f32=True, y=None, y_row_off=0, compute="bf16"):
    S, L, d = x.shape
    dev = x.device
    x, w, bias, resid = _f32(x), _f32(w, dev), _f32(bias, dev), _f32(resid, dev)
    if y is None:
        y = torch.full((S, L + (y_row_off if mode else 0), d), float("nan"), dtype=torch.float32, device=dev)
    assert y.is_contiguous() and y.dtype == torch.float32
    keep = _u8(rowkeep, dev)
    ws = torch.empty(16 * 31 * 64 * 64 * 4 + x.numel() * 2 + y.numel() * 2 + 1024, dtype=torch.uint8, device=dev)
    _lib.check(_lib.lib().f5h_op_conv_pos(_lib.stream_handle(dev), _lib.COMPUTE[compute], S, L, d, x.data_ptr(),
                                          w.data_ptr(), bias.data_ptr(), _lib.ptr(keep), int(mode),
                                          _lib.ptr(resid), int(bool(x_as_f32)), y.shape[1], int(y_row_off),
                                          y.data_ptr(), ws.data_ptr(), ws.numel()), "f5h_op_conv_pos")
    return y


def op_norm(kind, h, p0, p1=None, h16=False, compute="bf16"):
    M, d = h.shape
    dev = h.device
    h, p0, p1 = _f32(h), _f32(p0, dev), _f32(p1, dev)
    out = torch.empty(M, d, dtype=torch.float32, device=dev)
    ws = torch.empty(h.numel() * 4 + 1024, dtype=torch.uint8, device=dev)
    _lib.check(_lib.lib().f5h_op_norm(_lib.stream_handle(dev), _lib.COMPUTE[compute], {"ln": 0, "rms": 1}[kind],
                                      int(bool(h16)), M, d, h.data_ptr(), p0.data_ptr(), _lib.ptr(p1),
                                      out.data_ptr(), ws.data_ptr(), ws.numel()), "f5h_op_norm")
    return out


def op_dwconv_ln(x, dw_w, dw_b, ln_w, ln_b, compute="bf16"):
    S, L, C = x.shape
    dev = x.device
    x, dw_w, dw_b, ln_w, ln_b = (_f32(t, dev) for t in (x, dw_w, dw_b, ln_w, ln_b))
    out = torch.empty(S, L, C, dtype=torch.float32, device=dev)
    ws = torch.empty(x.numel() * 2 + 1024, dtype=torch.uint8, device=dev)
    _lib.check(_lib.lib().f5h_op_dwconv_ln(_lib.stream_handle(dev), _lib.COMPUTE[compute], S, L, C, x.data_ptr(),
                                           dw_w.data_ptr(), dw_b.data_ptr(), ln_w.data_ptr(), ln_b.data_ptr(),
                                           out.data_ptr(), ws.data_ptr(), ws.numel()), "f5h_op_dwconv_ln")
    return out


def op_grn(x, gamma, beta, compute="bf16"):
    S, L, C = x.shape
    dev = x.device
    x, gamma, beta = (_f32(t, dev) for t in (x, gamma, beta))
    out = torch.empty(S, L, C, dtype=torch.float32, device=dev)
    ws = torch.empty(((L + 63) // 64 + 1) * S * C * 4 + x.numel() * 2 + 1024, dtype=torch.uint8, device=dev)
    _lib.check(_lib.lib().f5h_op_grn(_lib.stream_handle(dev), _lib.COMPUTE[compute], S, L, C, x.data_ptr(),
                                     gamma.data_ptr(), beta.data_ptr(), out.data_ptr(), ws.data_ptr(), ws.numel()),
               "f5h_op_grn")
    return out


EPI = {"store": 0, "silu": 1, "gelu_tanh": 2, "gelu_erf": 3, "resid": 4, "resid_fill": 5, "inproj": 6, "qkv": 7,
       "gelu_erf_op": 8, "resid16": 9, "store16": 10}


def op_gemm_epi(epi, A, W, bias=None, C=None, compute="bf16", A2=None, k_split=0, resid=None, gate=None, rowkeep=None,
                live_len=None, live_seq=0, add=None, dual_rows=0, seq_len=0, heads=0, rope_heads=0, q_scale=0.0,
                hs_scale=None, ln_producer=False, ln_part_in=None, ln_u=None, ln_v=None, ln_rms=False, ln_eps=0.0,
                ln_nparts=None, poison=False):
    M, K = A.shape
    N = W.shape[0]
    dev = A.device
    A, A2, W, bias, resid, gate, add = (_f32(t, dev) for t in (A, A2, W, bias, resid, gate, add))
    keep = _u8(rowkeep, dev)
    ll = None if live_len is None else live_len.to(dev, torch.int32).contiguous()
    a = _lib.OpGemmArgs()
    a.compute, a.epi, a.M, a.N, a.K, a.k_split = _lib.COMPUTE[compute], EPI[epi], M, N, K, int(k_split)
    a.A, a.A2, a.W, a.bias = A.data_ptr(), _lib.ptr(A2), W.data_ptr(), _lib.ptr(bias)
    a.resid, a.gate, a.rowkeep, a.live_len, a.live_seq = _lib.ptr(resid), _lib.ptr(gate), _lib.ptr(keep), \
        _lib.ptr(ll), int(live_seq)
    a.add, a.ld_add, a.dual_rows = _lib.ptr(add), (0 if add is None else add.shape[1]), int(dual_rows)
    ws_bytes = ((N + 127) // 128 * 128) * K * 4 + 3 * M * K * 4 + 3 * (M + int(dual_rows)) * N * 4 + 4096
    hs_scale, ln_part_in, ln_u, ln_v = (_f32(t, dev) for t in (hs_scale, ln_part_in, ln_u, ln_v))
    hs = parts = None
    if ln_producer:
        G = _lib.OP_GUARD_ROWS
        a.ln_nparts = N // 64 if ln_nparts is None else int(ln_nparts)
        parts = torch.empty(M + G, max(a.ln_nparts, 1), 2, dtype=torch.float32, device=dev)
        a.ln_part_out = parts.data_ptr()
        if hs_scale is not None:
            hs = torch.empty(M + G, N, dtype=torch.float32, device=dev)
            a.hs_scale, a.hs_out = hs_scale.data_ptr(), hs.data_ptr()
            ws_bytes += (M + G) * N * 2 + 256
    elif ln_part_in is not None:
        a.ln_nparts = K // 64 if ln_nparts is None else int(ln_nparts)
        a.ln_part_in, a.ln_u, a.ln_v = ln_part_in.data_ptr(), _lib.ptr(ln_u), _lib.ptr(ln_v)
    a.ln_rms, a.ln_eps, a.poison = int(bool(ln_rms)), float(ln_eps), int(bool(poison))
    out = None
    if epi == "qkv":
        S = M // seq_len if seq_len > 0 else 0
        q, k, v = (torch.full((S, heads, seq_len, 64), float("nan"), dtype=torch.float32, device=dev)
                   for _ in range(3))
        rope = torch.empty(max(seq_len, 0), 32, 2, dtype=torch.float32, device=dev)
        a.seq_len, a.heads, a.rope_heads, a.q_scale = int(seq_len), int(heads), int(rope_heads), float(q_scale)
        a.q, a.k, a.v, a.rope_out = q.data_ptr(), k.data_ptr(), v.data_ptr(), rope.data_ptr()
        ws_bytes += max(seq_len, 0) * 256 + 1024
        out = (q, k, v, rope)
    else:
        if C is None:
            C = torch.full((M + int(dual_rows), N), float("nan"), dtype=torch.float32, device=dev)
        else:
            C = _f32(C, dev).clone()
        a.C = C.data_ptr()
        out = C
    ws = torch.empty(ws_bytes, dtype=torch.uint8, device=dev)
    _lib.check(_lib.lib().f5h_op_gemm_epi(_lib.stream_handle(dev), ctypes.byref(a), ws.data_ptr(), ws.numel()),
               "f5h_op_gemm_epi")
    return (out, hs, parts) if ln_producer else out


def op_lnfold_uv(table, W1, Wqkv, nfe, out_off, compute="bf16"):
    depth, F, d = W1.shape
    dev = table.device
    table = _f32(table).clone()
    W1, Wqkv = _f32(W1, dev), _f32(Wqkv, dev)
    ws = torch.empty((W1.numel() + Wqkv.numel()) * 2 + 16 * depth + 2048, dtype=torch.uint8, device=dev)
    _lib.check(_lib.lib().f5h_op_lnfold_uv(_lib.stream_handle(dev), _lib.COMPUTE[compute], int(nfe), depth, d, F,
                                           table.data_ptr(), table.shape[1], int(out_off), W1.data_ptr(),
                                           Wqkv.data_ptr(), ws.data_ptr(), ws.numel()), "f5h_op_lnfold_uv")
    return table


def op_scale_cols(W, g, compute="bf16"):
    rows, K = W.shape
    dev = W.device
    W, g = _f32(W), _f32(g, dev)
    out = torch.empty(rows, K, dtype=torch.float32, device=dev)
    ws = torch.empty(W.numel() * 4 + 1024, dtype=torch.uint8, device=dev)
    _lib.check(_lib.lib().f5h_op_scale_cols(_lib.stream_handle(dev), _lib.COMPUTE[compute], rows, K, W.data_ptr(),
                                            g.data_ptr(), out.data_ptr(), ws.data_ptr(), ws.numel()),
               "f5h_op_scale_cols")
    return out


def attn_force_safe(on: bool):
    _lib.check(_lib.lib().f5h_attn_force_safe(int(bool(on))), "attn_force_safe")


def gemm_force_config(cfg: int = -1):
    _lib.check(_lib.lib().f5h_gemm_force_config(int(cfg)), "gemm_force_config")


def chain_debug_spin_limit(limit: int = -1):
    _lib.check(_lib.lib().f5h_chain_debug_spin_limit(int(limit)), "chain_debug_spin_limit")
```

include/f5h.h:

```cpp
#ifndef F5H_H
#define F5H_H

#include <stddef.h>
#include <stdint.h>

#ifdef __cplusplus
extern "C" {
#endif

enum f5h_status {
  F5H_OK = 0,
  F5H_EINVAL = -1,
  F5H_EHIP = -2,
  F5H_ENOWEIGHT = -3,
  F5H_ENOMEM = -4,
};

enum f5h_backbone { F5H_DIT = 0, F5H_UNETT = 1 };
enum f5h_compute { F5H_FP32 = 0, F5H_BF16 = 1, F5H_FP16 = 2 };

typedef struct f5h_arch {
  int32_t backbone;
  int32_t dim;
  int32_t depth;
// ... 15 lines not shown
  const float* data;
  int64_t numel;
} f5h_weight;

enum f5h_dtype { F5H_DT_F32 = 0, F5H_DT_BF16 = 1, F5H_DT_F16 = 2 };

typedef struct f5h_tensor_view {
  const char* name;
  const void* data;
  int32_t dtype;
  int32_t on_device;
  int64_t numel;
} f5h_tensor_view;

typedef struct f5h_engine f5h_engine;

int f5h_engine_create_views(const f5h_arch* arch, const f5h_tensor_view* weights, int32_t n_weights,
                            int32_t device, f5h_engine** out);
int f5h_engine_create(const f5h_arch* arch, const f5h_weight* weights, int32_t n_weights,
                      int32_t device, f5h_engine** out);
void f5h_engine_destroy(f5h_engine* eng);
int f5h_release_pending(int32_t wait);

typedef struct f5h_sample_args {
  int32_t B, N, nt, nfe;
  const float* cond;
  const uint8_t* cond_mask;
  const int64_t* text;
  const int32_t* duration;
  const float* y0;
  const float* t_grid;
  float cfg_strength;
  int32_t use_batch_mask;
  float* out;
  float* trajectory;
} f5h_sample_args;

size_t f5h_workspace_size(const f5h_engine* eng, int32_t B, int32_t N, int32_t nt, int32_t nfe,
                          int32_t use_cfg);

int f5h_sample(f5h_engine* eng, void* stream, const f5h_sample_args* args, void* workspace,
               size_t workspace_bytes);

enum f5h_ode_method { F5H_EULER = 0, F5H_MIDPOINT = 1, F5H_RK4 = 2 };

size_t f5h_workspace_size_ode(const f5h_engine* eng, int32_t B, int32_t N, int32_t nt, int32_t steps,
                              int32_t use_cfg, int32_t method);
int f5h_sample_ode(f5h_engine* eng, void* stream, const f5h_sample_args* args, int32_t method, void* workspace,
                   size_t workspace_bytes);
int f5h_debug_ode_tableau(int32_t method, int32_t* stages, float* c, float* a, float* b);
int f5h_debug_ode_eval_times(int32_t method, int32_t compute, const float* t_grid, int32_t steps, float* out);

typedef struct f5h_forward_args {
  int32_t B, N, nt;
  const float* x;
  const float* cond;
  const uint8_t* cond_mask;
  const int64_t* text;
  const int32_t* duration;
  float t;
  int32_t use_batch_mask;
  float* pred;
  int32_t cfg_infer;
  int32_t drop_audio_cond;
  int32_t drop_text;
  const float* t_dev;
  int32_t text_cache;
} f5h_forward_args;
int f5h_forward(f5h_engine* eng, void* stream, const f5h_forward_args* args, void* workspace,
                size_t workspace_bytes);

int f5h_probe_enable(f5h_engine* eng, int32_t kclass, int32_t enable);
int f5h_probe_read(f5h_engine* eng, int64_t* launches, double* total_ms);
int f5h_probe_timeline(f5h_engine* eng, uint64_t* stamps, int32_t max_wg, int32_t* n_wg, double* tick_khz);

int f5h_set_graph_mode(f5h_engine* eng, int32_t mode);
int f5h_set_cfg_streams(f5h_engine* eng, int32_t n);
int f5h_graph_stats(f5h_engine* eng, int64_t* captures, int64_t* replays, int32_t* cached);
int f5h_last_call_host_ms(f5h_engine* eng, double* ms, int32_t n);
int f5h_set_pad_skip(f5h_engine* eng, int32_t enable);
int f5h_set_chain(f5h_engine* eng, int32_t enable);
int f5h_set_ln_fold(f5h_engine* eng, int32_t enable);
int f5h_ln_fold_stats(f5h_engine* eng, int32_t* supported, int64_t* passes);
int f5h_chain_stats(f5h_engine* eng, int64_t* launches, int32_t* fault, int64_t* refused);
int f5h_chain_debug_spin_limit(int64_t limit);

int f5h_op_linear(void* stream, int32_t compute, int32_t M, int32_t N, int32_t K, const float* A,
                  const float* W, const float* bias, float* C, void* workspace, size_t workspace_bytes);
int f5h_op_attention(void* stream, int32_t compute, int32_t S, int32_t H, int32_t N, const float* Q,
                     const float* K, const float* V, const int32_t* kv_len, int32_t q_prescaled, float* O,
                     void* workspace, size_t workspace_bytes);
int f5h_op_attention_qlen(void* stream, int32_t compute, int32_t S, int32_t H, int32_t N, const float* Q,
                          const float* K, const float* V, const int32_t* kv_len, const int32_t* q_len,
                          int32_t q_prescaled, float* O, void* workspace, size_t workspace_bytes);

int f5h_op_conv_pos(void* stream, int32_t compute, int32_t S, int32_t L, int32_t d, const float* x, const float* w,
                    const float* bias, const uint8_t* rowkeep, int32_t mode, const float* resid, int32_t x_as_f32,
                    int64_t y_seq_stride, int64_t y_row_off, float* y, void* workspace, size_t workspace_bytes);
int f5h_op_norm(void* stream, int32_t compute, int32_t kind, int32_t h16, int32_t M, int32_t d, const float* h,
                const float* shift_or_g, const float* scale, float* out, void* workspace, size_t workspace_bytes);
int f5h_op_dwconv_ln(void* stream, int32_t compute, int32_t S, int32_t L, int32_t C, const float* x,
                     const float* dw_w, const float* dw_b, const float* ln_w, const float* ln_b, float* out,
                     void* workspace, size_t workspace_bytes);
int f5h_op_grn(void* stream, int32_t compute, int32_t S, int32_t L, int32_t C, const float* x, const float* gamma,
               const float* beta, float* out, void* workspace, size_t workspace_bytes);

typedef struct f5h_op_gemm_args {
  int32_t compute, epi, M, N, K, k_split;
  const float* A;
  const float* A2;
  const float* W;
  const float* bias;
  float* C;
  const float* resid;
  const float* gate;
  const uint8_t* rowkeep;
  const int32_t* live_len;
  int32_t live_seq;
  int32_t seq_len, heads, rope_heads;
  float q_scale;
  const float* add;
  int64_t ld_add;
  int64_t dual_rows;
  float* q;
  float* k;
  float* v;
  float* rope_out;
  const float* hs_scale;
  float* hs_out;
  float* ln_part_out;
  const float* ln_part_in;
  const float* ln_u;
  const float* ln_v;
  int32_t ln_nparts, ln_rms;
  float ln_eps;
  int32_t poison;
} f5h_op_gemm_args;
#define F5H_OP_GUARD_ROWS 4
int f5h_op_gemm_epi(void* stream, const f5h_op_gemm_args* args, void* workspace, size_t workspace_bytes);
int f5h_op_lnfold_uv(void* stream, int32_t compute, int32_t nfe, int32_t depth, int32_t d, int32_t F, float* table,
                     int64_t stride, int64_t out_off, const float* W1, const float* Wqkv, void* workspace,
                     size_t workspace_bytes);
int f5h_op_scale_cols(void* stream, int32_t compute, int64_t rows, int32_t K, const float* W, const float* g,
                      float* out, void* workspace, size_t workspace_bytes);

int f5h_gemm_force_config(int32_t cfg);
int f5h_attn_force_safe(int32_t on);
int f5h_debug_tile_live(const int32_t* live_len, int32_t live_seq, int32_t M, int32_t m0, int32_t BM);

typedef struct f5h_vocos_arch {
  int32_t input_channels;
  int32_t dim;
  int32_t intermediate_dim;
  int32_t num_layers;
  int32_t n_fft;
  int32_t hop_length;
  int32_t compute;
} f5h_vocos_arch;
typedef struct f5h_vocos f5h_vocos;

int f5h_vocos_create(const f5h_vocos_arch* arch, const f5h_weight* weights, int32_t n_weights, int32_t device,
                     f5h_vocos** out);
void f5h_vocos_destroy(f5h_vocos* v);
size_t f5h_vocos_workspace_size(const f5h_vocos* v, int32_t B, int32_t T);
int f5h_vocos_decode(f5h_vocos* v, void* stream, int32_t B, int32_t T, const float* mel, float* audio,
                     void* workspace, size_t workspace_bytes);
// ... 23 lines not shown
```

Measured before the change: 18660 mel-frames/s.

## Add write-through store policy for GEMM and attention epilogues

Adds a per-kernel-class store policy that lets the QKV, out-proj, FFN1/FFN2 GEMM epilogues and the attention output use buffer stores with a write-through cache policy (aux bits). Attention gains an LDS-staged, swizzled output path so each wave writes full rows with 128-bit buffer stores. In auto mode the policy is chosen per launch when the grid fits in one wave of CUs, aiming to cut cache write-back latency for the next dependent kernel. The cost is an extra LDS round trip and barrier in attention, more kernel variants, and possible slowdowns if write-through raises memory traffic.

Result: faster. 19630 mel-frames/s, median of 6 (+5.2%).

```diff
diff --git a/f5-tts_amd/csrc/attention.hip b/f5-tts_amd/csrc/attention.hip
--- a/f5-tts_amd/csrc/attention.hip
+++ b/f5-tts_amd/csrc/attention.hip
@@ -35,7 +35,7 @@
   bh = id / nqb;
 }
 
-template <typename T, bool PRESCALED, int NW, bool RSM>
+template <typename T, bool PRESCALED, int NW, bool RSM, bool WT = false>
 __global__ __launch_bounds__(64 * NW, 8 / NW) void attn16_kernel(AttnArgs a) {
   typedef Op16<T> OP;
   typedef typename OP::v8 v8;
@@ -358,12 +358,15 @@
       dma(2, 2);
       pass(IT{});
       l_tot = row_sum();
+      if constexpr (WT) __syncthreads();
     }
   }
   probe_mark(a.probe, probe_t, 2);
   const float inv = l_tot > 0.f ? 1.f / l_tot : 0.f;
   if (!wave_dead) {
     T* O = reinterpret_cast<T*>(a.o) + (((int64_t)s_idx * L + min(qrow, L - 1)) * a.H + head) * 64;
+    uint4* const stg = lds + 256 + wid * 256;
+    const int srow = lane & 31;
 #pragma unroll
     for (int u = 0; u < 2; ++u)
 #pragma unroll
@@ -376,8 +379,26 @@
         auto sx = __builtin_amdgcn_permlane32_swap(a2.x, b2.x, false, false);
         auto sy = __builtin_amdgcn_permlane32_swap(a2.y, b2.y, false, false);
         const uint4 out = make_uint4(sx[0], sy[0], sx[1], sy[1]);
-        if (qrow < L) *reinterpret_cast<uint4*>(O + 32 * u + 8 * r4 + 8 * h) = out;
-      }
+        if constexpr (WT)
+          stg[srow * 8 + ((4 * u + r4 + h) ^ (srow & 7))] = out;
+        else if (qrow < L)
+          *reinterpret_cast<uint4*>(O + 32 * u + 8 * r4 + 8 * h) = out;
+      }
+    if constexpr (WT) {
+      __builtin_amdgcn_fence(__ATOMIC_RELEASE, "wavefront");
+      __builtin_amdgcn_wave_barrier();
+      __builtin_amdgcn_fence(__ATOMIC_ACQUIRE, "wavefront");
+      const int64_t rstride = (int64_t)a.H * 64 * sizeof(T);
+      const __amdgpu_buffer_rsrc_t ors = rsrc_of(reinterpret_cast<T*>(a.o) + ((int64_t)s_idx * L * a.H + head) * 64,
+                                                 (uint64_t)(L - 1) * rstride + 64 * sizeof(T));
+      const int row0 = qb * (32 * NW) + wid_s * 32;
+#pragma unroll
+      for (int i = 0; i < 4; ++i) {
+        const int r = i * 8 + (lane >> 3), c = lane & 7;
+        const uint4 w = stg[r * 8 + (c ^ (r & 7))];
+        buffer_store16<kAuxWT>(ors, (uint32_t)((row0 + r) * rstride + c * 16), __builtin_bit_cast(u32x4, w));
+      }
+    }
   }
   probe_exit(a.probe, probe_t);
 }
@@ -448,6 +469,8 @@
   probe_exit(a.probe, probe_t);
 }
 
+static bool attn_wt_ok(const AttnArgs& a) { return ((int64_t)a.L + 256) * a.H * 128 < ((int64_t)1 << 31); }
+
 template <typename T>
 static void launch16(const AttnArgs& a, hipStream_t st) {
   constexpr int NW = 8;
@@ -456,6 +479,10 @@
     const char* v = getenv("F5H_ATTN_ROWSUM");
     return v && !strcmp(v, "mfma");
   }();
+  if (a.prescaled && !rsm && a.store_wt && attn_wt_ok(a)) {
+    hipLaunchKernelGGL((attn16_kernel<T, true, NW, false, true>), grid, dim3(64 * NW), 0, st, a);
+    return;
+  }
   if (a.prescaled) {
     if (rsm)
       hipLaunchKernelGGL((attn16_kernel<T, true, NW, true>), grid, dim3(64 * NW), 0, st, a);
@@ -469,10 +496,18 @@
 static int g_force_safe = 0;
 void attention_force_safe(int on) { g_force_safe = on ? 1 : 0; }
 
+int gemm_num_cus();
+int attention_store_wt(int compute, const AttnArgs& a, int want) {
+  if (store_policy_forced() >= 0) want = store_policy_forced();
+  if (want == 0 || compute == F5H_C_FP32 || !a.prescaled || !attn_wt_ok(a)) return 0;
+  return want > 0 || (int64_t)((a.L + 255) / 256) * a.S * a.H <= gemm_num_cus();
+}
+
 hipError_t attention(int compute, const AttnArgs& a0, hipStream_t st) {
   if (a0.S <= 0 || a0.H <= 0 || a0.L <= 0) return hipErrorInvalidValue;
   AttnArgs a = a0;
   a.force_safe = g_force_safe;
+  if (store_policy_forced() >= 0) a.store_wt = attention_store_wt(compute, a0, store_policy_forced());
   switch (compute) {
     case F5H_C_BF16: launch16<bf16>(a, st); break;
     case F5H_C_FP16: launch16<f16>(a, st); break;
diff --git a/f5-tts_amd/csrc/chain.h b/f5-tts_amd/csrc/chain.h
--- a/f5-tts_amd/csrc/chain.h
+++ b/f5-tts_amd/csrc/chain.h
@@ -4,7 +4,6 @@
 
 namespace f5h {
 
-constexpr int kAuxWT = 16;
 constexpr unsigned kChainSpinLimit = 1u << 18;
 constexpr int kChainSleep = 2;
 
diff --git a/f5-tts_amd/csrc/common.h b/f5-tts_amd/csrc/common.h
--- a/f5-tts_amd/csrc/common.h
+++ b/f5-tts_amd/csrc/common.h
@@ -228,6 +228,11 @@
 
 F5H_DEV __amdgpu_buffer_rsrc_t rsrc_of(const void* p, uint64_t bytes) {
   return __builtin_amdgcn_make_buffer_rsrc(const_cast<void*>(p), 0, (int)(uint32_t)bytes, 0x00020000);
+}
+constexpr int kAuxWT = 16;
+template <int AUX>
+F5H_DEV void buffer_store16(__amdgpu_buffer_rsrc_t r, uint32_t off, u32x4 v) {
+  __builtin_amdgcn_raw_buffer_store_b128(v, r, off, 0, AUX);
 }
 F5H_DEV void dma16(__amdgpu_buffer_rsrc_t r, LDS_PTR(void) dst, uint32_t voff, uint32_t soff) {
   __builtin_amdgcn_raw_ptr_buffer_load_lds(r, dst, 16, voff, soff, 0, 0);
diff --git a/f5-tts_amd/csrc/engine.cpp b/f5-tts_amd/csrc/engine.cpp
--- a/f5-tts_amd/csrc/engine.cpp
+++ b/f5-tts_amd/csrc/engine.cpp
@@ -57,14 +57,15 @@
 struct GraphKey {
   const void* ws;
   int kind;
-  int B, N, nt, nfe, use_cfg, batch_mask, probe, split, pad_skip, chain, lnfold;
+  int B, N, nt, nfe, use_cfg, batch_mask, probe, split, pad_skip, chain, lnfold, store;
   int method;
   uint64_t kernel_epoch;
   uint32_t cfg_bits;
   bool operator==(const GraphKey& o) const {
     return ws == o.ws && kind == o.kind && B == o.B && N == o.N && nt == o.nt && nfe == o.nfe && kernel_epoch == o.kernel_epoch &&
            use_cfg == o.use_cfg && batch_mask == o.batch_mask && probe == o.probe && cfg_bits == o.cfg_bits &&
-           split == o.split && pad_skip == o.pad_skip && chain == o.chain && lnfold == o.lnfold && method == o.method;
+           split == o.split && pad_skip == o.pad_skip && chain == o.chain && lnfold == o.lnfold && store == o.store &&
+           method == o.method;
   }
 };
 
@@ -104,6 +105,8 @@
   const void** lnf_w = nullptr;
   int64_t ada_row = 0;
   std::atomic<int64_t> n_lnfold{0};
+  int store_policy = -1;
+  std::atomic<int64_t> n_store_wt{0}, n_store_plain{0};
   unsigned* chain_fault = nullptr;
   volatile unsigned* fault_host = nullptr;
   int fault_slot = -1;
@@ -503,6 +506,15 @@
 }
 
 enum { KC_FFN1 = 0, KC_ATTN = 1, KC_QKV = 2, KC_FFN2 = 3, KC_CONV = 4, KC_OUT = 5, KC_NORM = 6, KC_CHAIN = 7 };
+static constexpr int kStoreBit(int kclass) {
+  return kclass == KC_QKV ? 1 : kclass == KC_ATTN ? 2 : kclass == KC_OUT ? 4 : kclass == KC_FFN1 ? 8 : kclass == KC_FFN2 ? 16 : 0;
+}
+static constexpr int kStoreAutoMask = 1 | 2 | 4 | 8 | 16;
+static int store_want(int policy, int kclass) {
+  if (policy == 0 || policy == 1) return policy;
+  if (policy >= 0x100) return (policy & kStoreBit(kclass)) ? 1 : 0;
+  return (kStoreAutoMask & kStoreBit(kclass)) ? -1 : 0;
+}
 struct ProbeScope {
   f5h_engine* e;
   hipStream_t st;
@@ -539,6 +551,7 @@
   int site;
   int chain;
   int lnfold;
+  int store;
   double* hp;
 };
 enum { HP_TOTAL = 0, HP_PROLOGUE, HP_LOCK, HP_REAP, HP_CAPTURE, HP_INSTANTIATE, HP_LAUNCH, HP_FINAL, kHostPhases };
@@ -784,6 +797,11 @@
     g.ln_nparts = d / 64;
   };
   if (fold_on || rms_on) e->n_lnfold.fetch_add(1, std::memory_order_relaxed);
+  auto count_store = [&](int wt) { (wt ? e->n_store_wt : e->n_store_plain).fetch_add(1, std::memory_order_relaxed); };
+  auto gemm_policy = [&](GemmArgs& g, int epi, int kclass) {
+    g.store_wt = gemm_store_wt(bf, epi, g, store_want(c.store, kclass));
+    count_store(g.store_wt);
+  };
   for (int l = 0; l < a.depth; ++l) {
     Layer& Ly = e->layers[l];
     const float* ad = ada_k ? ada_k + (size_t)l * 6 * d : nullptr;
@@ -815,6 +833,7 @@
         g.W = Ly.qkv_g.w;
         rms_consumer(g);
       }
+      gemm_policy(g, EPI_QKV, KC_QKV);
       ProbeScope ps(e, KC_QKV, st, &c.site, &g.probe);
       KCK(gemm(bf, EPI_QKV, g, st));
     }
@@ -832,6 +851,8 @@
       at.q_len = (c.batch_mask && e->pad_skip) ? b.kvlen + s0 : nullptr;
       at.scale = 0.125f;
       at.prescaled = 1;
+      at.store_wt = attention_store_wt(bf, at, store_want(c.store, KC_ATTN));
+      count_store(at.store_wt);
       ProbeScope ps(e, KC_ATTN, st, &c.site, &at.probe);
       KCK(attention(bf, at, st));
     }
@@ -875,6 +896,7 @@
       }
       if (fold_on) fold_producer(g, ad + 4 * d );
       if (rms_on) rms_producer(g);
+      gemm_policy(g, epi_resid, KC_OUT);
       ProbeScope ps(e, KC_OUT, st, &c.site, &g.probe);
       KCK(gemm(bf, epi_resid, g, st));
     }
@@ -894,6 +916,7 @@
         g.W = Ly.ff1_g.w;
         rms_consumer(g);
       }
+      gemm_policy(g, EPI_GELU_TANH, KC_FFN1);
       ProbeScope ps(e, KC_FFN1, st, &c.site, &g.probe);
       KCK(gemm(bf, EPI_GELU_TANH, g, st));
     }
@@ -902,6 +925,7 @@
       g.gate = ad ? ad + 5 * d : nullptr;
       if (fold_on && l + 1 < a.depth) fold_producer(g, ada_k + (size_t)(l + 1) * 6 * d + d);
       if (rms_on && l + 1 < a.depth / 2) rms_producer(g);
+      gemm_policy(g, epi_resid, KC_FFN2);
       ProbeScope ps(e, KC_FFN2, st, &c.site, &g.probe);
       KCK(gemm(bf, epi_resid, g, st));
     }
@@ -1275,6 +1299,7 @@
   key.use_cfg = c.use_cfg;
   key.batch_mask = c.batch_mask;
   key.lnfold = c.lnfold;
+  key.store = c.store;
   key.method = c.method;
   key.kernel_epoch = g_kernel_epoch.load();
   return key;
@@ -1381,6 +1406,7 @@
   ChainTicket ticket;
   c.chain = chain_for_call(e, c, ticket);
   c.lnfold = e->lnfold && !c.chain && ((e->lnf_ok && !c.batch_mask) || e->rmsf_ok);
+  c.store = e->store_policy;
   double hp[kHostPhases] = {};
   c.hp = hp;
   const double h0 = host_ms();
@@ -1516,6 +1542,7 @@
   key.pad_skip = e->pad_skip;
   key.chain = c.chain;
   key.lnfold = c.lnfold;
+  key.store = c.store;
   key.method = c.method;
   key.kernel_epoch = g_kernel_epoch.load();
   std::memcpy(&key.cfg_bits, &a->cfg_strength, 4);
@@ -1696,6 +1723,7 @@
   ChainTicket ticket;
   c.chain = chain_for_call(e, c, ticket);
   c.lnfold = e->lnfold && !c.chain && ((e->lnf_ok && !c.batch_mask) || e->rmsf_ok);
+  c.store = e->store_policy;
   const bool cached = a->text_cache == 2;
   if (a->t_dev) {
     HIPCK(hipMemcpyAsync(c.b.tgrid, a->t_dev, sizeof(float), hipMemcpyDeviceToDevice, c.st));
@@ -1727,6 +1755,7 @@
     key.pad_skip = e->pad_skip;
     key.chain = c.chain;
     key.lnfold = c.lnfold;
+    key.store = c.store;
     key.kernel_epoch = g_kernel_epoch.load();
     std::shared_ptr<GraphEntry> hold;
     RC(graph_get(c, key, false, body, hold, 1));
@@ -1861,6 +1890,29 @@
   if (!e) return fail(F5H_EINVAL, "null engine");
   if (supported) *supported = (e->lnf_ok || e->rmsf_ok) ? 1 : 0;
   if (passes) *passes = e->n_lnfold.load(std::memory_order_relaxed);
+  return 0;
+}
+
+int f5h_set_store_policy(f5h_engine* e, int32_t mode) {
+  if (!e) return fail(F5H_EINVAL, "null engine");
+  if (mode != -1 && mode != 0 && mode != 1 && (mode < 0x100 || mode > 0x11F))
+    return fail(F5H_EINVAL, "store policy must be -1 (auto), 0 (plain), 1 (write-through) or 0x100 | class mask");
+  std::lock_guard<std::mutex> g(e->gm);
+  e->store_policy = mode;
+  return 0;
+}
+
+int f5h_store_policy_stats(f5h_engine* e, int64_t* write_through, int64_t* plain) {
+  if (!e) return fail(F5H_EINVAL, "null engine");
+  if (write_through) *write_through = e->n_store_wt.load(std::memory_order_relaxed);
+  if (plain) *plain = e->n_store_plain.load(std::memory_order_relaxed);
+  return 0;
+}
+
+int f5h_store_policy_force(int32_t mode) {
+  if (mode < -1 || mode > 1) return fail(F5H_EINVAL, "forced store policy must be -1 (off), 0 (plain) or 1 (write-through)");
+  store_policy_force(mode);
+  g_kernel_epoch.fetch_add(1);
   return 0;
 }
 
diff --git a/f5-tts_amd/csrc/gemm.hip b/f5-tts_amd/csrc/gemm.hip
--- a/f5-tts_amd/csrc/gemm.hip
+++ b/f5-tts_amd/csrc/gemm.hip
@@ -95,7 +95,31 @@
 
 void gemm_force_config(int cfg) { g_force_cfg = cfg; }
 
-hipError_t gemm(int compute, int epi, const GemmArgs& a, hipStream_t st) {
+static int g_store_force = -1;
+void store_policy_force(int mode) { g_store_force = mode; }
+int store_policy_forced() { return g_store_force; }
+
+static bool gemm_wt_variant(int compute, int epi, const GemmArgs& a, int64_t* tiles, int64_t* slots) {
+  if (compute == F5H_C_FP32 || (epi != EPI_QKV && epi != EPI_RESID16 && epi != EPI_GELU_TANH) || a.M <= 0) return false;
+  const int cfg = gemm_select_cfg(a);
+  if (cfg != 0 && cfg != 1 && cfg != 5) return false;
+  const int bm = cfg == 0 ? 64 : (cfg == 1 ? 128 : 192);
+  *tiles = (int64_t)((a.M + bm - 1) / bm) * ((a.N + 127) / 128);
+  *slots = 2 * (int64_t)gemm_num_cus();
+  return epi == EPI_QKV ? fast_epi_ok<EPI_QKV>(a, 128)
+                        : (epi == EPI_RESID16 ? fast_epi_ok<EPI_RESID16>(a, 128) : fast_epi_ok<EPI_GELU_TANH>(a, 128));
+}
+
+int gemm_store_wt(int compute, int epi, const GemmArgs& a, int want) {
+  if (g_store_force >= 0) want = g_store_force;
+  int64_t tiles = 0, slots = 0;
+  if (want == 0 || !gemm_wt_variant(compute, epi, a, &tiles, &slots)) return 0;
+  return want > 0 || tiles <= slots;
+}
+
+hipError_t gemm(int compute, int epi, const GemmArgs& a0, hipStream_t st) {
+  GemmArgs a = a0;
+  if (g_store_force >= 0) a.store_wt = gemm_store_wt(compute, epi, a0, g_store_force);
   const int bke = compute ? 64 : 32;
   if (a.K % bke != 0 || a.M < 0 || a.N <= 0 || a.lda % 8 || a.ldw % 8) return hipErrorInvalidValue;
   if (epi == EPI_INPROJ && (a.ldc % 8 || a.ld_add % 8 || a.N % 8)) return hipErrorInvalidValue;
diff --git a/f5-tts_amd/csrc/gemm_impl.h b/f5-tts_amd/csrc/gemm_impl.h
--- a/f5-tts_amd/csrc/gemm_impl.h
+++ b/f5-tts_amd/csrc/gemm_impl.h
@@ -526,7 +526,7 @@
           }
           const float m2 = sum8(q2.x + q2.y);
           __builtin_amdgcn_raw_buffer_store_b64(u32x2_t{__float_as_uint(mean), __float_as_uint(m2)}, ln_st,
-                                                (uint32_t)((row * ln_np + ln_p) * 8), 0, AUX);
+                                                (uint32_t)((row * ln_np + ln_p) * 8), 0, 0);
         }
       } else if constexpr (EPI == EPI_GELU_TANH || EPI == EPI_GELU_ERF_OP) {
         if constexpr (EPI == EPI_GELU_TANH && is16<TC>()) {
@@ -565,10 +565,11 @@
     __builtin_amdgcn_fence(__ATOMIC_ACQUIRE, "wavefront");
   });
 }
-template <typename TC, int EPI, int MT, int NT, int WN, int EPAD, bool PREF, int AUX = 0, int PD = 1, int PM, int PT>
+template <typename TC, int EPI, int MT, int NT, int WN, int EPAD, bool PREF, int AUX = 0, int PD = 1, bool FOLD = true,
+          int PM, int PT>
 F5H_DEV void epilogue_fast(const GemmArgs& g, const f32x4 (&acc)[MT][NT], float* Cs, int rbase, int cbase,
                            int lane, const V8 (&pre)[PM][PT], const float* ln_rows = nullptr) {
-  if constexpr (WN == 64 && is16<TC>() && AUX == 0) {
+  if constexpr (WN == 64 && is16<TC>() && FOLD) {
     if constexpr (EPI == EPI_RESID16) {
       if (g.ln_part && g.ln_rms) {
         if (g.bias)
@@ -800,7 +801,7 @@
 
 
 template <typename TC, int EPI, int BM, int BN, int WGM, int WGN, int NS, bool FAST, int KB, bool PUB = false,
-          bool CHAIN = false>
+          bool CHAIN = false, int AUX = 0>
 F5H_DEV void gemm_body(const GemmArgs& g, const int b, const int nwg, uint4* lds, const ChainDep& dep) {
   const ProbeT probe_t = probe_enter(g.probe);
   typedef GemmCfg<BM, BN, WGM, WGN, NS, KB> C;
@@ -1005,8 +1006,9 @@
   constexpr bool FAST_EPI = FAST && NT % 2 == 0;
   static_assert(FAST_EPI || !PUB, "the chain publishes after the fast (LDS-strip) epilogue");
   if constexpr (FAST_EPI) {
-    epilogue_fast<TC, EPI, MT, NT, WN, C::EPAD, PREF, PUB ? kAuxWT : 0>(g, acc, Cs, m0 + wm * WM, n0 + wn * WN, lane,
-                                                                         pre, LNC ? ln_rows + 2 * wm * WM : nullptr);
+    static_assert(AUX == 0 || FAST_EPI, "the store policy exists for the strip epilogue only");
+    epilogue_fast<TC, EPI, MT, NT, WN, C::EPAD, PREF, PUB ? kAuxWT : AUX, 1, !PUB>(
+        g, acc, Cs, m0 + wm * WM, n0 + wn * WN, lane, pre, LNC ? ln_rows + 2 * wm * WM : nullptr);
     if constexpr (PUB) chain_publish(dep, g.M, m0, BM);
   }
   if constexpr (!FAST_EPI) {
@@ -1034,10 +1036,10 @@
   probe_exit(g.probe, probe_t);
 }
 
-template <typename TC, int EPI, int BM, int BN, int WGM, int WGN, int NS, bool FAST = false, int KB = 128>
+template <typename TC, int EPI, int BM, int BN, int WGM, int WGN, int NS, bool FAST = false, int KB = 128, int AUX = 0>
 __global__ __launch_bounds__(64 * WGM * WGN, 2) void gemm_kernel(GemmArgs g) {
   __shared__ __attribute__((aligned(16))) uint4 lds[GemmCfg<BM, BN, WGM, WGN, NS, KB>::bytes / 16];
-  gemm_body<TC, EPI, BM, BN, WGM, WGN, NS, FAST, KB>(g, blockIdx.x, gridDim.x, lds, ChainDep{});
+  gemm_body<TC, EPI, BM, BN, WGM, WGN, NS, FAST, KB, false, false, AUX>(g, blockIdx.x, gridDim.x, lds, ChainDep{});
 }
 
 template <int BM, int BN, int WGM2, int WGN2, int KS, int D>
@@ -1623,6 +1625,11 @@
 template <typename TC, int EPI>
 static void launch_8p(const GemmArgs& a, hipStream_t st);
 
+template <typename TC, int EPI>
+constexpr bool store_wt_epi() {
+  return is16<TC>() && (EPI == EPI_QKV || EPI == EPI_RESID16 || EPI == EPI_GELU_TANH);
+}
+
 template <int EPI>
 static bool fast_epi_ok(const GemmArgs& a, int BN) {
   const uint64_t span = (uint64_t)(a.M + a.dual_rows) * (uint64_t)std::max<int64_t>(a.ldc, a.N) * 4;
@@ -1684,6 +1691,13 @@
                        EPI == EPI_GELU_ERF_OP || EPI == EPI_STORE || EPI == EPI_STORE16 || EPI == EPI_INPROJ;
   if constexpr (HOT) {
     if (fast_epi_ok<EPI>(a, BN)) {
+      if constexpr (store_wt_epi<TC, EPI>()) {
+        if (a.store_wt) {
+          hipLaunchKernelGGL((gemm_kernel<TC, EPI, BM, BN, WGM, WGN, NS, true, KB, kAuxWT>), dim3(tiles),
+                             dim3(64 * WGM * WGN), 0, st, a);
+          return;
+        }
+      }
       hipLaunchKernelGGL((gemm_kernel<TC, EPI, BM, BN, WGM, WGN, NS, true, KB>), dim3(tiles), dim3(64 * WGM * WGN), 0,
                          st, a);
       return;
diff --git a/f5-tts_amd/csrc/kernels.h b/f5-tts_amd/csrc/kernels.h
--- a/f5-tts_amd/csrc/kernels.h
+++ b/f5-tts_amd/csrc/kernels.h
@@ -53,6 +53,7 @@
   void* hs; const float* hs_scale; float* ln_part;
   const float* ln_part_in; int ln_nparts; const float* ln_u; const float* ln_v;
   int ln_rms; float ln_eps;
+  int store_wt;
 };
 
 __host__ __device__ inline bool tile_live_rows(const int32_t* live_len, int live_seq, int M, int m0, int BM) {
@@ -70,6 +71,11 @@
 hipError_t gemm(int compute, int epi, const GemmArgs& a, hipStream_t st);
 void gemm_force_config(int cfg);
 
+
+int gemm_store_wt(int compute, int epi, const GemmArgs& a, int want);
+void store_policy_force(int mode);
+int store_policy_forced();
+
 struct AttnArgs {
   const void* q; const void* k; const void* v; void* o;
   int S, H, L;
@@ -79,8 +85,10 @@
   int prescaled;
   DevProbe probe;
   int force_safe;
+  int store_wt;
 };
 hipError_t attention(int compute, const AttnArgs& a, hipStream_t st);
+int attention_store_wt(int compute, const AttnArgs& a, int want);
 void attention_force_safe(int on);
 
 struct ConvArgs {
diff --git a/f5-tts_amd/f5_tts_amd/_lib.py b/f5-tts_amd/f5_tts_amd/_lib.py
--- a/f5-tts_amd/f5_tts_amd/_lib.py
+++ b/f5-tts_amd/f5_tts_amd/_lib.py
@@ -41,6 +41,9 @@
     "f5h_chain_debug_spin_limit",
     "f5h_set_ln_fold",
     "f5h_ln_fold_stats",
+    "f5h_set_store_policy",
+    "f5h_store_policy_stats",
+    "f5h_store_policy_force",
     "f5h_op_linear",
     "f5h_op_attention",
     "f5h_op_attention_qlen",
@@ -231,6 +234,13 @@
         L.f5h_set_ln_fold.restype = ctypes.c_int
         L.f5h_ln_fold_stats.argtypes = [vp, ctypes.POINTER(i32), ctypes.POINTER(i64)]
         L.f5h_ln_fold_stats.restype = ctypes.c_int
+    if hasattr(L, "f5h_set_store_policy"):
+        L.f5h_set_store_policy.argtypes = [vp, i32]
+        L.f5h_set_store_policy.restype = ctypes.c_int
+        L.f5h_store_policy_stats.argtypes = [vp, ctypes.POINTER(i64), ctypes.POINTER(i64)]
+        L.f5h_store_policy_stats.restype = ctypes.c_int
+        L.f5h_store_policy_force.argtypes = [i32]
+        L.f5h_store_policy_force.restype = ctypes.c_int
     if hasattr(L, "f5h_chain_debug_spin_limit"):
         L.f5h_chain_debug_spin_limit.argtypes = [i64]
         L.f5h_chain_debug_spin_limit.restype = ctypes.c_int
diff --git a/f5-tts_amd/f5_tts_amd/engine.py b/f5-tts_amd/f5_tts_amd/engine.py
--- a/f5-tts_amd/f5_tts_amd/engine.py
+++ b/f5-tts_amd/f5_tts_amd/engine.py
@@ -129,6 +129,16 @@
         sup, n = ctypes.c_int32(), ctypes.c_int64()
         _lib.check(_lib.lib().f5h_ln_fold_stats(self._h, ctypes.byref(sup), ctypes.byref(n)), "ln_fold_stats")
         return bool(sup.value), int(n.value)
+
+    STORE_CLASS_BITS = {"qkv": 1, "attn": 2, "out": 4, "ffn1": 8, "ffn2": 16}
+
+    def set_store_policy(self, mode: int):
+        _lib.check(_lib.lib().f5h_set_store_policy(self._h, int(mode)), "set_store_policy")
+
+    def store_policy_stats(self):
+        wt, plain = ctypes.c_int64(), ctypes.c_int64()
+        _lib.check(_lib.lib().f5h_store_policy_stats(self._h, ctypes.byref(wt), ctypes.byref(plain)), "store_policy_stats")
+        return int(wt.value), int(plain.value)
 
     def chain_stats(self):
         n, f, r = ctypes.c_int64(), ctypes.c_int32(), ctypes.c_int64()
@@ -264,7 +274,7 @@
     return C
 
 
-def op_attention(Q, K, V, kv_len=None, compute="bf16", q_prescaled=False, poison=False, q_len=None):
+def op_attention(Q, K, V, kv_len=None, compute="bf16", q_prescaled=False, poison=False, q_len=None, return_ws=False):
     S, H, N, D = Q.shape
     assert D == 64
     O = torch.empty(S, N, H * 64, dtype=torch.float32, device=Q.device)
@@ -277,7 +287,7 @@
                                                Q.contiguous().data_ptr(), K.contiguous().data_ptr(),
                                                V.contiguous().data_ptr(), _lib.ptr(kv), int(bool(q_prescaled)),
                                                O.data_ptr(), ws.data_ptr(), ws.numel()), "f5h_op_attention")
-        return O
+        return (O, ws) if return_ws else O
     if poison:
         O.fill_(float("nan"))
     ql = q_len.to(Q.device, torch.int32).contiguous()
@@ -286,7 +296,7 @@
                                                 V.contiguous().data_ptr(), _lib.ptr(kv), ql.data_ptr(),
                                                 int(bool(q_prescaled)), O.data_ptr(), ws.data_ptr(), ws.numel()),
                "f5h_op_attention_qlen")
-    return O
+    return (O, ws) if return_ws else O
 
 
 def _f32(t, dev=None):
@@ -356,7 +366,7 @@
 def op_gemm_epi(epi, A, W, bias=None, C=None, compute="bf16", A2=None, k_split=0, resid=None, gate=None, rowkeep=None,
                 live_len=None, live_seq=0, add=None, dual_rows=0, seq_len=0, heads=0, rope_heads=0, q_scale=0.0,
                 hs_scale=None, ln_producer=False, ln_part_in=None, ln_u=None, ln_v=None, ln_rms=False, ln_eps=0.0,
-                ln_nparts=None, poison=False):
+                ln_nparts=None, poison=False, ws_fill=None, return_ws=False):
     M, K = A.shape
     N = W.shape[0]
     dev = A.device
@@ -403,9 +413,12 @@
         a.C = C.data_ptr()
         out = C
     ws = torch.empty(ws_bytes, dtype=torch.uint8, device=dev)
+    if ws_fill is not None:
+        ws.fill_(int(ws_fill))
     _lib.check(_lib.lib().f5h_op_gemm_epi(_lib.stream_handle(dev), ctypes.byref(a), ws.data_ptr(), ws.numel()),
                "f5h_op_gemm_epi")
-    return (out, hs, parts) if ln_producer else out
+    res = (out, hs, parts) if ln_producer else out
+    return (res, ws) if return_ws else res
 
 
 def op_lnfold_uv(table, W1, Wqkv, nfe, out_off, compute="bf16"):
@@ -440,5 +453,9 @@
     _lib.check(_lib.lib().f5h_gemm_force_config(int(cfg)), "gemm_force_config")
 
 
+def store_policy_force(mode: int = -1):
+    _lib.check(_lib.lib().f5h_store_policy_force(int(mode)), "store_policy_force")
+
+
 def chain_debug_spin_limit(limit: int = -1):
     _lib.check(_lib.lib().f5h_chain_debug_spin_limit(int(limit)), "chain_debug_spin_limit")
diff --git a/include/f5h.h b/include/f5h.h
--- a/include/f5h.h
+++ b/include/f5h.h
@@ -121,6 +121,9 @@
 int f5h_set_chain(f5h_engine* eng, int32_t enable);
 int f5h_set_ln_fold(f5h_engine* eng, int32_t enable);
 int f5h_ln_fold_stats(f5h_engine* eng, int32_t* supported, int64_t* passes);
+int f5h_set_store_policy(f5h_engine* eng, int32_t mode);
+int f5h_store_policy_stats(f5h_engine* eng, int64_t* write_through, int64_t* plain);
+int f5h_store_policy_force(int32_t mode);
 int f5h_chain_stats(f5h_engine* eng, int64_t* launches, int32_t* fault, int64_t* refused);
 int f5h_chain_debug_spin_limit(int64_t limit);
 
```
